# nextpyp/pyp

Hardware: AMD Instinct MI355X
Metric: particles/sec projection-matching, 256^2 box (higher is better)
Workload: dtype f32

## Files before the change

### include/ppm.h

```cpp
#ifndef PPM_H
#define PPM_H

#include <stddef.h>

#ifdef __cplusplus
extern "C" {
#endif

#define PPM_NCOL 32
enum {
    PPM_POS = 0, PPM_PSI = 1, PPM_THETA = 2, PPM_PHI = 3, PPM_XSHIFT = 4, PPM_YSHIFT = 5,
    PPM_DF1 = 6, PPM_DF2 = 7, PPM_ANGAST = 8, PPM_PSHIFT = 9, PPM_FILM = 10, PPM_OCC = 11,
    PPM_LOGP = 12, PPM_SIGMA = 13, PPM_SCORE = 14, PPM_PIXEL = 15, PPM_VOLTAGE = 16,
    PPM_CS = 17, PPM_AMP = 18, PPM_BTX = 19, PPM_BTY = 20, PPM_PIND = 26, PPM_TIND = 27
};

#define PPM_MAX_SHIFT_STEPS 8
#define PPM_MAX_TOP_HITS 64
#define PPM_MAX_DEFOCUS_STEPS 20

typedef struct ppm_refine_cfg {
    int box;
    float pixel_size;
    float molecular_mass_kda;
    float mask_radius;
    float res_low;
    float res_high;
    float res_signed_cc;
    float search_mask_radius;
    float res_search;
    float angular_step;
    int top_hits;
    float search_range_x;
    float search_range_y;
    int global_search;
    int local_refine;
    int refine_psi, refine_theta, refine_phi, refine_x, refine_y;
    int normalize;
    int invert;
    float mask_falloff;
    int iters_hit;
    int iters_final;
    float local_angle_step;
    float local_shift_step;
    char symmetry[8];
    float band_factor;
    int refine_defocus;
    float defocus_range;
    float defocus_step;
    float focus[4];
    int use_priors;
    float prior_mean[5];
    float prior_var[5];
    float res_classification;
} ppm_refine_cfg;

typedef struct ppm_recon_cfg {
    int box;
    float pixel_size;
    float res_limit;
    float score_weight_bfactor;
    float score_average;
    float score_threshold;
    int normalize;
    int invert;
    int split_by_pind;
    float mask_radius;
    const float *dose_weights; int n_dose_weights;
    float dose_exponent;
    float dose_transition;
} ppm_recon_cfg;

typedef struct ppm_final_cfg {
    float molecular_mass_kda;
    float inner_radius;
    float outer_radius;
    float mask_falloff;
} ppm_final_cfg;

enum { PPM_CSP_PARTICLES = 1, PPM_CSP_MICROGRAPHS = 2 };
#define PPM_NPCOL 12
#define PPM_NTCOL 6
typedef struct ppm_csp_cfg {
    int unit;
    int refine_rotation;
    int refine_translation;
    float tol_angle[3];
    float tol_shift;
    float step_tolerance;
    int max_iterations;
    int tind_min, tind_max;
    int first, last;
    int refine_defocus;
    float defocus_range;
    float defocus_step;
    int search_points;
    int search_candidates;
} ppm_csp_cfg;

typedef struct ppm_csp_search_info {
    int active;
    int shift_grid;
    double step;
    double r_g;
    double h_s;
    double tol_shift;
    int n_angle[3];
    int full_turn[3];
    int n_shift_axis;
    long n_rot, n_shift;
    int n_candidates;
} ppm_csp_search_info;

#define PPM_STATS_COLS 7

typedef struct ppm_ref ppm_ref_t;
typedef struct ppm_accum ppm_accum_t;

enum { PPM_K_PREP = 0, PPM_K_BANK = 1, PPM_K_GLOBAL = 2, PPM_K_TOPK = 3, PPM_K_LOCAL = 4,
       PPM_K_INSERT = 5, PPM_K_FINAL = 6, PPM_K_EXTRACT = 7, PPM_K_NORMS = 8, PPM_K_COUNT = 9 };

int ppm_init(int device);
const char *ppm_last_error(void);
const char *ppm_version(void);
const char *ppm_build_id(void);
int ppm_device_mem_info(size_t *free_bytes, size_t *total_bytes);

ppm_ref_t *ppm_reference_create(const float *vol, int n, float max_band_px);
ppm_ref_t *ppm_reference_create_padded(const float *vol, int n, float max_band_px, int pad);
ppm_ref_t *ppm_reference_create_weighted(const float *vol, int n, float max_band_px, int pad, const float *ring_weight, int n_weight);
void ppm_reference_destroy(ppm_ref_t *ref);

int ppm_refine_batch(ppm_ref_t *ref, const ppm_refine_cfg *cfg, const void *images,
                     int images_on_device, int n_img, const double *rows_in, double *rows_out);
int ppm_refine_last_counts(ppm_ref_t *ref, long *n_global, long *n_local, long *samples_global,
                           long *samples_local);
const char *ppm_refine_note(ppm_ref_t *ref);
int ppm_refine_last_sections(ppm_ref_t *ref);
int ppm_refine_last_overlap(ppm_ref_t *ref);

int ppm_match_projections(ppm_ref_t *ref, const ppm_refine_cfg *cfg, const double *rows, int n_rows, float *out);

int ppm_csp_refine(ppm_ref_t *ref, const ppm_refine_cfg *cfg, const ppm_csp_cfg *csp, const void *images, int images_on_device,
                   int n_proj, double *rows, double *particles, int n_part, double *tilts, int n_tilt);
int ppm_csp_search_plan(const ppm_refine_cfg *cfg, const ppm_csp_cfg *csp, ppm_csp_search_info *out);
int ppm_csp_search_candidates(ppm_ref_t *ref, long unit, int max_k, long *rot_index, long *shift_index, double *score);

#define PPM_FRAME_MAX_STEPS 8
typedef struct ppm_frame_cfg { float range_px, step_px; int half_width, tind_min, tind_max, first, last; } ppm_frame_cfg;
typedef struct ppm_frame_info { long groups, models, rows_refined, rows_scored, rows_skipped; int n_steps; float step_px, range_px; int clipped; } ppm_frame_info;
int ppm_frame_refine(ppm_ref_t *ref, const ppm_refine_cfg *cfg, const ppm_frame_cfg *fcfg, const void *images, int images_on_device,
                     const double *rows, int n_rows, double *rows_out, float *own_maps, float *pooled_maps, ppm_frame_info *info);
int ppm_frame_plan(const ppm_frame_cfg *fcfg, float *step_px, int *n_steps, int *clipped);

typedef struct ppm_sva_cfg {
    int box; float pixel_size;
    float window[3];
    float window_sigma;
    float highpass_cutoff, highpass_decay, lowpass_cutoff, lowpass_decay;
    int use_missing_wedge;
    float tol_angle;
    float tol_shift;
    float step_tolerance;
    int max_iterations;
    float band_factor;
    int search_mode;
    float global_step;
    int n_candidates;
    char symmetry[8];
} ppm_sva_cfg;
int ppm_sva_align(ppm_ref_t *ref, const ppm_sva_cfg *cfg, const void *volumes, int volumes_on_device, int n_vol, const float *wedges,
                  double *poses, double *scores);

size_t ppm_accum_floats(int box);
ppm_accum_t *ppm_accum_create(int box, float pixel_size, const char *symmetry,
                              void *ext_device_buffer);
void ppm_accum_destroy(ppm_accum_t *acc);
int ppm_insert_batch(ppm_accum_t *acc, const ppm_recon_cfg *cfg, const void *images,
                     int images_on_device, int n_img, const double *rows);
int ppm_accum_download(ppm_accum_t *acc, float *host);
int ppm_accum_download_range(ppm_accum_t *acc, float *host, size_t first, size_t count);
int ppm_accum_add(ppm_accum_t *acc, const float *host);
long ppm_accum_count(ppm_accum_t *acc, int half);
void ppm_accum_set_count(ppm_accum_t *acc, int half, long count);

typedef struct ppm_comm_id { char bytes[128]; } ppm_comm_id;
int ppm_comm_unique_id(ppm_comm_id *id);
void *ppm_comm_create(int n_ranks, int rank, const ppm_comm_id *id);
int ppm_comm_count(void *comm);
void ppm_comm_destroy(void *comm);
int ppm_accum_reduce(ppm_accum_t *acc, void *comm, int root);

int ppm_sva_insert(ppm_accum_t *acc, const ppm_sva_cfg *cfg, const void *volumes, int volumes_on_device, int n_vol, const float *wedges,
                   const double *poses, const long *index);

int ppm_sva_align_average(ppm_ref_t *ref, ppm_accum_t *acc, const ppm_sva_cfg *cfg, const void *volumes, int volumes_on_device, int n_vol,
                          const float *wedges, double *poses, double *scores, const long *index);

int ppm_finalize(ppm_accum_t *acc, const ppm_final_cfg *cfg, float *half1, float *half2,
                 float *filtered, double *stats);

typedef struct ppm_mask_cfg { double pixel_size; int edge_width; double outside_weight;
                              int filter; double filter_radius_A; double filter_edge_px; } ppm_mask_cfg;
int ppm_mask_volume(const void *map, const void *mask, int on_device, int n, const ppm_mask_cfg *cfg, void *out);

typedef struct ppm_create_mask_cfg { double pixel_size, outer_radius_A, threshold, lowpass_A, lowpass_edge_px, rebin; } ppm_create_mask_cfg;
typedef struct ppm_create_mask_info { double density_min, density_max; long above, components, largest, mask_voxels; } ppm_create_mask_info;
int ppm_create_mask(const void *map, int on_device, int n, const ppm_create_mask_cfg *cfg, void *mask_out, ppm_create_mask_info *info);

typedef struct ppm_post_cfg {
    double pixel_size;
    int mask_mode;
    double automask_lp;
    int threshold_method;
    double threshold_value;
    int randomize_method;
    double randomize_value;
    unsigned seed;
    int bfactor_method;
    double adhoc_bfac, fit_low, fit_high;
    int lowpass_auto;
    double lowpass, highpass;
    int gaussian, skip_fsc_weighting, apply_fsc2, flip_x, flip_y, flip_z;
} ppm_post_cfg;
typedef struct ppm_post_info { int s_r, res_shell, fit_shells, transforms; double resolution, bfactor, threshold; long mask_voxels; } ppm_post_info;
int ppm_postprocess(const void *half1, const void *half2, const void *mask, int on_device, int n, const ppm_post_cfg *cfg,
                    void *unmasked_out, void *masked_out, void *mask_out, double *curves, long *shell_count, ppm_post_info *info);

#define PPM_LOCRES_MAX_LEVELS 64
#define PPM_LOCRES_UNASSIGNED 100.0f
typedef struct ppm_locres_cfg { double pixel_size, p_value, min_res, max_res, step; int keep_levels; } ppm_locres_cfg;
typedef struct ppm_locres_info {
    int n_levels, transforms;
    long n_inside, unassigned;
    double median;
    float levels[PPM_LOCRES_MAX_LEVELS], tau[PPM_LOCRES_MAX_LEVELS];
    long counts[PPM_LOCRES_MAX_LEVELS];
    char notes[256];
} ppm_locres_info;
int ppm_local_resolution(const ppm_locres_cfg *cfg, const void *half1, const void *half2, const void *mask, int on_device, int n,
                         void *out_res, void *level_maps, ppm_locres_info *info);

int ppm_extract_boxes(const void *image, int image_on_device, int rows, int cols, const double *coords, int m,
                      int box, double coordinate_binning, double radius_px, int normalize, int fix_empty,
                      void *out, int out_on_device);

void ppm_profile_enable(int on);
void ppm_profile_reset(void);
int ppm_profile_get(int kernel_id, double *total_ms, long *launches);

void *ppm_device_alloc(size_t bytes);
void ppm_device_free(void *p);
int ppm_device_upload(void *dst, const void *src, size_t bytes);
int ppm_device_sync(void);
void *ppm_host_alloc(size_t bytes);
void ppm_host_free(void *p);
int ppm_host_read(int fd, long long offset, void *dst, size_t bytes, int n_threads);

#ifdef __cplusplus
}
#endif
#endif
```

### pyp_amd/csrc/host_ctx.h

```cpp
#pragma once

namespace {

thread_local std::string g_err;
int fail(int code, const std::string &msg) { g_err = "ERROR: " + msg; return code; }

#define HIPCHK(call)                                                                          \
    do {                                                                                      \
        hipError_t e_ = (call);                                                               \
        if (e_ != hipSuccess) {                                                               \
            g_err = std::string("ERROR: HIP: ") + hipGetErrorString(e_) + " at " #call;        \
            return -5;                                                                        \
        }                                                                                     \
    } while (0)
#define HIPCHKP(call)                                                                         \
    do {                                                                                      \
        hipError_t e_ = (call);                                                               \
        if (e_ != hipSuccess) {                                                               \
            g_err = std::string("ERROR: HIP: ") + hipGetErrorString(e_) + " at " #call;        \
            return nullptr;                                                                   \
        }                                                                                     \
    } while (0)

struct Ctx {
// ... 26 lines not shown
};

hipEvent_t ev_get() {
    std::lock_guard<std::mutex> lk(g_mu);
    if (!g.pool.empty()) { hipEvent_t e = g.pool.back(); g.pool.pop_back(); return e; }
    hipEvent_t e; (void)hipEventCreate(&e); return e;
}
void prof_flush() {
    std::lock_guard<std::mutex> lk(g_mu);
    for (auto &p : g.pending) {
        (void)hipEventSynchronize(p.b);
        float ms = 0; (void)hipEventElapsedTime(&ms, p.a, p.b);
        g.prof_ms[p.id] += ms; g.prof_n[p.id] += 1;
        g.pool.push_back(p.a); g.pool.push_back(p.b);
    }
    g.pending.clear();
}
struct ProfScope {
    int id; hipEvent_t a = nullptr;
    explicit ProfScope(int id_) : id(id_) { if (g.prof_on) { a = ev_get(); (void)hipEventRecord(a, cur_stream()); } }
    ~ProfScope() { if (a) { hipEvent_t b = ev_get(); (void)hipEventRecord(b, cur_stream()); std::lock_guard<std::mutex> lk(g_mu); g.pending.push_back({ id, a, b }); } }
};

struct Trace {
    const char *who; bool on; std::chrono::steady_clock::time_point t0;
    explicit Trace(const char *w) : who(w), on(getenv("PPM_TRACE") != nullptr), t0(std::chrono::steady_clock::now()) {}
    void mark(const char *what) const {
        if (!on) return;
        const double host_ms = std::chrono::duration<double, std::milli>(std::chrono::steady_clock::now() - t0).count();
        (void)hipStreamSynchronize(cur_stream());
        fprintf(stderr, "%s: %8.2f ms  (host reached this mark)\n", who, host_ms);
        fprintf(stderr, "%s: %8.2f ms  %s\n", who, std::chrono::duration<double, std::milli>(std::chrono::steady_clock::now() - t0).count(), what);
    }
};

int ensure_plan(int n) {
    if (n < 2 || n > 512) return fail(-22, "FFT length out of range");
    std::lock_guard<std::mutex> lk(g_mu);
    if (g.plans[n].ready) return 0;
    std::vector<int> fac; std::vector<unsigned short> perm;
    fft_factors(n, fac, perm);
    int prod = 1; for (int f : fac) prod *= f;
    if (prod != n || fac.size() > 12) return fail(-22, "FFT length must have prime factors 2, 3, 5 and 7 only");
    std::vector<float2> t(n);
    for (int k = 0; k < n; k++) t[k] = make_float2((float)std::cos(2.0 * kPi * k / n), (float)std::sin(2.0 * kPi * k / n));
    float2 *dtw = nullptr; unsigned short *dperm = nullptr;
    HIPCHK(hipMalloc(&dtw, sizeof(float2) * n));
    HIPCHK(hipMalloc(&dperm, sizeof(unsigned short) * n));
    HIPCHK(hipMemcpy(dtw, t.data(), sizeof(float2) * n, hipMemcpyHostToDevice));
    HIPCHK(hipMemcpy(dperm, perm.data(), sizeof(unsigned short) * n, hipMemcpyHostToDevice));
    FftPlan &p = g.plans[n].plan;
    p.n = n; p.nfac = (int)fac.size(); for (size_t i = 0; i < fac.size(); i++) p.fac[i] = fac[i];
    p.tw = dtw; p.perm = dperm;
    g.plans[n].ready = true;
    return 0;
}


int fft_lines_pass(float2 *d, int n, long nlines, long inner, long inner_stride, long outer_stride, long elem_stride, int line_major, bool inverse) {
    if (nlines <= 0) return 0;
    if (int rc = ensure_plan(n)) return rc;
    int L = std::max(1, std::min(16, 7600 / (n + 1)));
    while (nlines % L) L--;
    FftLinesP P;
    P.data = d; P.plan = g.plans[n].plan; P.n = n; P.inverse = inverse ? 1 : 0; P.L = L; P.nlines = nlines;
    P.inner = inner; P.inner_stride = inner_stride; P.outer_stride = outer_stride; P.elem_stride = elem_stride; P.line_major = line_major;
    hipLaunchKernelGGL(k_fft_lines, dim3((unsigned)((nlines + L - 1) / L)), dim3(256), (size_t)L * (n + 1) * sizeof(float2), cur_stream(), P);
    HIPCHK(hipGetLastError());
    return 0;
}

int fft2d_batch(float2 *d, int n, long nimg, bool inverse) {
    const long nlines = nimg * n;
    if (int rc = fft_lines_pass(d, n, nlines, nlines, n, 0, 1, 0, inverse)) return rc;
    return fft_lines_pass(d, n, nlines, n, 1, (long)n * n, n, 1, inverse);
}

int fft3d(float2 *d, int n, bool inverse) {
    const long nlines = (long)n * n;
    if (int rc = fft_lines_pass(d, n, nlines, nlines, n, 0, 1, 0, inverse)) return rc;
    if (int rc = fft_lines_pass(d, n, nlines, n, 1, nlines, n, 1, inverse)) return rc;
    return fft_lines_pass(d, n, nlines, nlines, 1, 0, nlines, 1, inverse);
}

template <typename T>
struct DevBuf {
    T *p = nullptr; size_t cap = 0;
    DevBuf() = default;
    DevBuf(const DevBuf &) = delete;
    DevBuf &operator=(const DevBuf &) = delete;
    ~DevBuf() { if (p) (void)hipFree(p); }
    int ensure(size_t n) {
        if (n <= cap) return 0;
        if (p) (void)hipFree(p);
        p = nullptr; cap = 0;
        HIPCHK(hipMalloc(&p, n * sizeof(T)));
        cap = n;
        return 0;
    }
};

int raise_lds_limit(const void *fn, int bytes) {
    static std::vector<const void *> raised;
    std::lock_guard<std::mutex> lk(g_mu);
    if (std::find(raised.begin(), raised.end(), fn) != raised.end()) return 0;
    HIPCHK(hipFuncSetAttribute(fn, hipFuncAttributeMaxDynamicSharedMemorySize, bytes));
    raised.push_back(fn);
    return 0;
}

template <typename T>
struct DevTmp {
    T *p = nullptr;
    DevTmp() = default;
    DevTmp(const DevTmp &) = delete;
    DevTmp &operator=(const DevTmp &) = delete;
    ~DevTmp() { if (p) (void)hipFree(p); }
    hipError_t alloc(size_t n) { return hipMalloc(&p, n * sizeof(T)); }
};


}

struct Lane { DevBuf<double> rows_in, rows_out; DevBuf<float> wring, cw, ddef; DevBuf<float2> Il; DevBuf<Hit> hits; DevBuf<LState> states, states2; };

struct ppm_ref {
    hipStream_t stream = nullptr, copy = nullptr;
    hipStream_t local = nullptr;
    int N = 0, B = 0, CX = 0, CY = 0, NBX = 0, NBY = 0, pad = 1; unsigned LB = 0;
    float2 *cube = nullptr;
    Lane lane[2];
    DevBuf<double> dir_theta, dir_phi;
    DevBuf<float> images, C2, nP, nI, cc, mats;
    DevBuf<float2> c_Il, c_band; DevBuf<float> c_cw, c_img, c_wring; DevBuf<double> c_rows, c_N, c_p, c_tl, c_delta, c_s0, c_g0, c_out;
    DevBuf<int> c_eval, c_rp, c_rt, c_slot, c_uoff, c_active; DevBuf<LState> c_states; DevBuf<double> c_mean, c_tmean, c_acc, c_dtrial, c_fpm, c_delta_t;
    DevBuf<double> c_rowtab; DevBuf<float> c_gbest, c_cscore; DevBuf<int> c_gshift, c_cshift; DevBuf<long> c_crot;
    std::vector<long> cand_unit, cand_rot; std::vector<int> cand_shift; std::vector<float> cand_score; int cand_K = 0;
    DevBuf<int> f_int; DevBuf<float> f_flt, f_own, f_pool; DevBuf<double> f_dbl; DevBuf<float2> f_store;
    DevBuf<float2> s_f, s_g, s_F; DevBuf<float> s_vols;
    struct { bool valid = false; float key[5] = { 0, 0, 0, 0, 0 }; int S = 0; std::vector<int> shell_off; DevBuf<uint32_t> samples, pos; DevBuf<float> bandw; DevBuf<float2> Fw; bool fw_valid = false; float wkey[4] = { 0, 0, 0, 0 }; } s_plan;
    DevBuf<float2> band, Wp, bank, twN;
    DevBuf<float2> spill;
    DevBuf<float4> rowtw;
    DevBuf<int> sh;
    DevBuf<uint32_t> samples;
    DevBuf<Hit> hits_t;
    DevBuf<int> tile_c;
    DevBuf<Hit> hits_s; DevBuf<int> sec_k;
    DevBuf<float4> bank4; DevBuf<float> part, gtw;
    std::string grid_key, bank_key, bank4_key; int gtw_ns = 0, gtw_rsx = -1;
    long last_counts[4] = { 0, 0, 0, 0 };
    int last_sections = 0;
    int last_overlap = 0;
    std::string note;
};

struct ppm_accum {
    hipStream_t stream = nullptr, copy = nullptr;
    int N = 0; float pixel = 1.f;
    float *acc = nullptr; bool external = false;
    std::vector<double> symops; int nsym = 1;
    float *d_sym = nullptr;
    unsigned long long *d_counts = nullptr;
    unsigned *d_max = nullptr;
    long counts[2] = { 0, 0 };
    DevBuf<double> rows; DevBuf<float> images, dose; DevBuf<float2> band, spill; DevBuf<PartIns> pp; DevBuf<CullEnt> cull; DevBuf<BrickItem> items;
    DevBuf<float2> s_f, s_g; DevBuf<float> s_vols;
    std::vector<float> brick_load; float load_r = -1.f; int n_items = 0, items_cap = -1;
};

static CubeView cube_view(const ppm_ref *ref) {
    CubeView cv;
    cv.cube = ref->cube; cv.NBX = ref->NBX; cv.NBY = ref->NBY; cv.LB = ref->LB; cv.off = ref->B + 1; cv.scale = (float)ref->pad;
    return cv;
}

static bool local_tables_wanted(int tabR) {
    return !(getenv("PPM_LOCAL_TABLES") && atoi(getenv("PPM_LOCAL_TABLES")) == 0) && cube_tab_bytes(tabR) <= 16 * 1024;
}
static bool tables_fit_lds(size_t ring_bytes, int tabR) { return ring_bytes + cube_tab_bytes(tabR) + 2048 <= (size_t)64 * 1024; }

struct ChunkStager {
    const float *src; float *buf; bool on_device; int n_img, chunk; size_t nn;
    int prime() const {
        if (on_device) return 0;
        HIPCHK(hipMemcpyAsync(buf, src, (size_t)std::min(chunk, n_img) * nn * sizeof(float), hipMemcpyHostToDevice, cur_copy()));
        HIPCHK(hipStreamSynchronize(cur_copy()));
        return 0;
    }
    const float *chunk_ptr(int c0, int ci) const { return on_device ? src + (size_t)c0 * nn : buf + (size_t)(ci & 1) * chunk * nn; }
    int prefetch_next(int c0, int ci) const {
        if (on_device || c0 + chunk >= n_img) return 0;
        const int n_next = std::min(chunk, n_img - (c0 + chunk));
        HIPCHK(hipMemcpyAsync(buf + (size_t)((ci + 1) & 1) * chunk * nn, src + (size_t)(c0 + chunk) * nn, (size_t)n_next * nn * sizeof(float), hipMemcpyHostToDevice, cur_copy()));
        return 0;
    }
    int sync() const {
        HIPCHK(hipStreamSynchronize(cur_stream()));
        HIPCHK(hipStreamSynchronize(cur_copy()));
        return 0;
    }
};

static __global__ void k_noop() {}

extern "C" {

const char *ppm_last_error(void) { return g_err.c_str(); }
const char *ppm_version(void) { return "pypmatch 0.1 (gfx950)"; }
const char *ppm_build_id(void) { return "pypmatch " __DATE__ " " __TIME__; }
int ppm_device_mem_info(size_t *free_bytes, size_t *total_bytes) {
    if (!g.inited) return fail(-1, "ppm_init has not been called");
    (void)hipSetDevice(g.device);
    size_t f = 0, t = 0;
    HIPCHK(hipMemGetInfo(&f, &t));
    if (free_bytes) *free_bytes = f;
    if (total_bytes) *total_bytes = t;
    return 0;
}

int ppm_init(int device) {
    static std::mutex init_mu;
    std::lock_guard<std::mutex> lk(init_mu);
    const auto t_init0 = std::chrono::steady_clock::now();
    if (g.inited && g.device == device) { (void)hipSetDevice(device); return 0; }
    if (g.inited) return fail(-16, "libpypmatch is bound to device " + std::to_string(g.device) + " in this process (one process per GPU); start another process for device " + std::to_string(device));
    int count = 0;
    if (hipGetDeviceCount(&count) != hipSuccess || count <= 0) return fail(-19, "no HIP device visible; libpypmatch has no CPU path");
    if (device < 0 || device >= count) return fail(-22, "device index out of range");
    if (const char *e = getenv("PPM_SYNC")) {
        const std::string v(e);
        (void)hipSetDeviceFlags(v == "block" ? hipDeviceScheduleBlockingSync : (v == "yield" ? hipDeviceScheduleYield : (v == "spin" ? hipDeviceScheduleSpin : hipDeviceScheduleAuto)));
    }
    HIPCHK(hipSetDevice(device));
    hipDeviceProp_t prop;
    HIPCHK(hipGetDeviceProperties(&prop, device));
    if (std::string(prop.gcnArchName).find("gfx950") == std::string::npos)
        return fail(-19, std::string("device is ") + prop.gcnArchName + ", libpypmatch is built for gfx950 only");
    g.total_mem = prop.totalGlobalMem;
    g.cu_count = std::max(1, prop.multiProcessorCount);
    g.lds_per_cu = std::max((size_t)prop.maxSharedMemoryPerMultiProcessor, (size_t)160 * 1024);
    if (!g.stream) HIPCHK(hipStreamCreateWithFlags(&g.stream, hipStreamNonBlocking));
    if (!g.copy) HIPCHK(hipStreamCreateWithFlags(&g.copy, hipStreamNonBlocking));
    if (!g.upload) HIPCHK(hipStreamCreateWithFlags(&g.upload, hipStreamNonBlocking));
    const auto t_ctx = std::chrono::steady_clock::now();
    hipLaunchKernelGGL(k_noop, dim3(1), dim3(64), 0, g.stream);
    HIPCHK(hipGetLastError());
    HIPCHK(hipStreamSynchronize(g.stream));
    g.device = device; g.inited = true;
    if (getenv("PPM_TRACE"))
        fprintf(stderr, "ppm_init: context + streams %.1f ms, code object + first launch %.1f ms\n",
                std::chrono::duration<double, std::milli>(t_ctx - t_init0).count(), std::chrono::duration<double, std::milli>(std::chrono::steady_clock::now() - t_ctx).count());
    return 0;
}

void ppm_profile_enable(int on) { g.prof_on = on != 0; }
void ppm_profile_reset(void) { prof_flush(); for (int i = 0; i < PPM_K_COUNT; i++) { g.prof_ms[i] = 0; g.prof_n[i] = 0; } }
int ppm_profile_get(int id, double *ms, long *n) {
    if (id < 0 || id >= PPM_K_COUNT) return fail(-22, "bad kernel id");
    prof_flush();
    if (ms) *ms = g.prof_ms[id];
    if (n) *n = g.prof_n[id];
    return 0;
}

void *ppm_device_alloc(size_t bytes) { if (g.inited) (void)hipSetDevice(g.device); void *p = nullptr; if (hipMalloc(&p, bytes) != hipSuccess) { g_err = "ERROR: device allocation failed"; return nullptr; } return p; }
void ppm_device_free(void *p) { if (p) (void)hipFree(p); }
int ppm_device_upload(void *dst, const void *src, size_t bytes) {
    if (!g.inited) return fail(-1, "ppm_init has not been called");
    HIPCHK(hipSetDevice(g.device));
    HIPCHK(hipMemcpyAsync(dst, src, bytes, hipMemcpyHostToDevice, g.upload));
    HIPCHK(hipStreamSynchronize(g.upload));
    return 0;
}
void *ppm_host_alloc(size_t bytes) { if (g.inited) (void)hipSetDevice(g.device); void *p = nullptr; if (hipHostMalloc(&p, bytes, hipHostMallocDefault) != hipSuccess) { g_err = "ERROR: pinned host allocation failed"; return nullptr; } return p; }
void ppm_host_free(void *p) { if (p) (void)hipHostFree(p); }
extern "C++" {
namespace {
struct ReadPool {
    std::mutex mu;
    std::mutex qmu;
    std::condition_variable wake, done;
    std::vector<std::thread> threads;
    struct Part { int fd; long long off; char *dst; size_t bytes; };
    std::vector<Part> parts;
    size_t next = 0, pending = 0;
    int err = 0;
    bool quit = false;
    void worker() {
        std::unique_lock<std::mutex> lk(qmu);
        for (;;) {
            wake.wait(lk, [&] { return quit || next < parts.size(); });
            if (quit) return;
            Part p = parts[next++];
            lk.unlock();
            int e = 0;
            size_t got = 0;
            while (got < p.bytes) {
                ssize_t r = pread(p.fd, p.dst + got, std::min(p.bytes - got, (size_t)64 << 20), p.off + (long long)got);
                if (r < 0) { if (errno == EINTR) continue; e = -errno; break; }
                if (r == 0) { e = -5; break; }
                got += (size_t)r;
            }
            lk.lock();
            if (e && !err) err = e;
            if (--pending == 0) done.notify_all();
        }
    }
    int run(int fd, long long off, char *dst, size_t bytes, int nt) {
        std::lock_guard<std::mutex> one(mu);
        nt = std::max(1, std::min(nt, 16));
        std::unique_lock<std::mutex> lk(qmu);
        while ((int)threads.size() < nt) threads.emplace_back([this] { worker(); });
        const size_t per = std::max((size_t)1 << 20, ((bytes + nt - 1) / nt + ((size_t)1 << 20) - 1) >> 20 << 20);
        parts.clear(); next = 0; err = 0;
        for (size_t a = 0; a < bytes; a += per) parts.push_back({fd, off + (long long)a, dst + a, std::min(per, bytes - a)});
        pending = parts.size();
        if (!pending) return 0;
        wake.notify_all();
        done.wait(lk, [&] { return pending == 0; });
        parts.clear(); next = 0;
        return err;
    }
    ~ReadPool() {
        { std::lock_guard<std::mutex> lk(qmu); quit = true; }
        wake.notify_all();
        for (auto &t : threads) t.join();
    }
};
// ... 44 lines not shown
```

### pyp_amd/csrc/host_refine.h

```cpp
#pragma once

static int launch_prep(DevBuf<float2> &spill , const float *d_images, const double *d_rows, int n_img, const Geom &gm, double Rm_px, float fall_px,
                       int normalize, int invert, int do_mask, int whiten, float2 *band, float *wring,
                       const uint32_t *samples, int S_pad, float2 *Il, float *cw, float2 *Wp, float *C2, float *nI,
                       unsigned *band_max = nullptr ,
                       const float *focus_px = nullptr ) {
    if (int rc = ensure_plan(gm.N)) return rc;
    PrepP P;
    P.images = d_images; P.rows = d_rows; P.plan = g.plans[gm.N].plan;
    P.N = gm.N; P.B = gm.B; P.W = gm.W; P.H = gm.H;
    P.r_hi2 = (float)(gm.r_hi * gm.r_hi); P.Rm = (float)Rm_px; P.wfall = fall_px; P.a = (float)gm.a;
    P.Rm2_bg = (float)std::min(std::floor(Rm_px * Rm_px), 16777216.0);
    P.normalize = normalize; P.invert = invert; P.do_mask = do_mask; P.whiten = whiten;
    for (int k = 0; k < 4; k++) P.focus[k] = focus_px ? focus_px[k] : 0.f;
    P.band_max = band_max;
    P.band = band; P.wring = wring; P.samples = samples; P.S_pad = S_pad; P.Il = Il; P.cw = cw;
    P.Wp = Wp; P.C2 = C2; P.nI = nI; P.Bs = gm.Bs; P.Hs = gm.Hs;
    P.r_s2 = (float)(gm.r_s * gm.r_s); P.r_lo2 = (float)(gm.r_lo * gm.r_lo);
    const PrepPlan pl = prep_plan(gm.N, gm.B, gm.W);
    if (pl.err) return fail(-12, pl.err);
    P.L = pl.L; P.nc = pl.nc; P.nchunks = pl.nchunks; P.TS = pl.TS; P.WS = pl.WS;
    P.spill = nullptr;
    if (!pl.scratch_free) {
        if (int rc = spill.ensure((size_t)n_img * gm.N * gm.W)) return rc;
        P.spill = spill.p;
    }
    if (int rc = pl.scratch_free ? raise_lds_limit((const void *)k_prep<512, 2>, 160 * 1024) : raise_lds_limit((const void *)k_prep<256, 3>, 80 * 1024)) return rc;
    ProfScope ps(PPM_K_PREP);
    if (pl.scratch_free) hipLaunchKernelGGL((k_prep<512, 2>), dim3(n_img), dim3(512), pl.lds.total, cur_stream(), P);
    else hipLaunchKernelGGL((k_prep<256, 3>), dim3(n_img), dim3(256), pl.lds.total, cur_stream(), P);
    HIPCHK(hipGetLastError());
    return 0;
}

template <int... I>
static const void *global_kernel_at(int i, std::integer_sequence<int, I...>) {
    static const void *const fn[] = { (const void *)k_global<I / 4 + 1, (I & 2) != 0, (I & 1) != 0>... };
    return fn[i];
}
static const void *global_kernel(int R, bool half, int Bs) {
    const bool two = Bs <= 31;
    return global_kernel_at(((R >= 1 && R <= 5 ? R : 6) - 1) * 4 + (half ? 2 : 0) + (two ? 1 : 0), std::make_integer_sequence<int, 24>());
}
static size_t global_lds_bytes(int HsP, int n_orient, int R, int *topk_lds) {
    size_t lds = (size_t)HsP * 64 * sizeof(float2) * global_particles(R);
    if (lds < 1024) lds = 1024;
    const size_t lds_topk = (size_t)(32 + n_orient) * sizeof(float);
    const int fits = lds_topk <= (size_t)160 * 1024 ? 1 : 0;
    if (topk_lds) *topk_lds = fits;
    if (fits && lds_topk > lds) lds = lds_topk;
    return lds;
}
static int launch_global(GlobP &P, int n_img, bool half, int R) {
    P.n = n_img;
    const size_t lds = global_lds_bytes(P.HsP, P.n_orient, R, &P.topk_lds);
    const void *fn = global_kernel(R, half, P.Bs);
    if (int rc = raise_lds_limit(fn, 160 * 1024)) return rc;
    ProfScope ps(PPM_K_GLOBAL);
    const int ngroups = (n_img + global_particles(R) - 1) / global_particles(R);
    void *args[] = { &P };
    HIPCHK(hipLaunchKernel(fn, dim3(std::min(ngroups, g.cu_count)), dim3(global_threads(R)), args, lds, cur_stream()));
    return 0;
}

struct GfftPlan { int LN = 0, L = 0, RC = 0, nchunk = 1; size_t fixed = 0, t_bytes = 0, lds = 0; int topk_lds = 0; };
static bool gfft_plan(const Geom &gm, GfftPlan &pl) {
    int LN = 0; while ((1 << LN) < gm.Ns) LN++;
    if ((1 << LN) != gm.Ns || LN < 4 || LN > 7) return false;
    pl.LN = LN; pl.L = gm.Ns / 2;
    const int L = pl.L, G = gfft_slices_per_pass(L), NR = 2 * gm.RSy + 1;
    const size_t row = (size_t)G * 2 * gfft_row_stride(L) * sizeof(float2), fixed = (size_t)L * L * sizeof(float4) + gfft_small_bytes(L);
    const size_t room = (size_t)160 * 1024 - fixed;
    int RC = NR;
    if (const char *e = getenv("PPM_GFFT_ROWS")) { const int v = atoi(e); if (v > 0 && v < RC) RC = v; }
    if ((size_t)RC * row > room) RC = (int)(room / row);
    if (RC > 2 * L) RC = 2 * L;
    pl.RC = RC; pl.nchunk = (NR + RC - 1) / RC;
    pl.RC = (NR + pl.nchunk - 1) / pl.nchunk;
    pl.t_bytes = std::max((size_t)pl.RC * row, (size_t)G * L * L * sizeof(float4));
    pl.fixed = fixed;
    return true;
}
static void gfft_plan_topk(GfftPlan &pl, int n_orient) {
    const size_t topk = (size_t)n_orient * sizeof(float);
    pl.topk_lds = 0;
    if (topk <= pl.t_bytes) pl.topk_lds = 1;
    else if (pl.fixed + topk <= (size_t)160 * 1024) { pl.topk_lds = 1; pl.t_bytes = (topk + 15) & ~(size_t)15; }
    pl.lds = pl.fixed + pl.t_bytes;
}
static const void *gfft_kernel(int LN, bool chunked) {
    static const void *const fn[] = { (const void *)k_gfft<4, false>, (const void *)k_gfft<4, true>, (const void *)k_gfft<5, false>, (const void *)k_gfft<5, true>,
                                      (const void *)k_gfft<6, false>, (const void *)k_gfft<6, true>, (const void *)k_gfft<7, false>, (const void *)k_gfft<7, true> };
    return fn[((LN >= 4 && LN <= 6 ? LN : 7) - 4) * 2 + (chunked ? 1 : 0)];
}
static int launch_gfft(GfftP &P, int n_img, const GfftPlan &pl) {
    P.n = n_img; P.RC = pl.RC; P.nchunk = pl.nchunk; P.t_bytes = (int)pl.t_bytes; P.topk_lds = pl.topk_lds;
    const void *fn = gfft_kernel(pl.LN, pl.nchunk > 1);
    if (int rc = raise_lds_limit(fn, 160 * 1024)) return rc;
    ProfScope ps(PPM_K_GLOBAL);
    void *args[] = { &P };
    HIPCHK(hipLaunchKernel(fn, dim3(n_img), dim3(256), args, pl.lds, cur_stream()));
#ifdef PPM_GFFT_STAMPS
    {
        float st[4 * 4 * 12];
        HIPCHK(hipStreamSynchronize(cur_stream()));
        HIPCHK(hipMemcpy(st, P.cc, sizeof(st), hipMemcpyDeviceToHost));
        const char *names[12] = { "products", "fft", "stores", "barrier A", "row tail", "barrier B", "twiddles", "loop", "row reads + pairs", "row fft", "row max", "-" };
        const int nsl = P.n_dir * P.npsi_store;
        for (int b = 0; b < 4 && b < n_img; b++) for (int w = 0; w < 4; w++) {
            fprintf(stderr, "k_gfft stamps block %d wave %d (cycles per slice):", b, w);
            for (int i = 0; i < 11; i++) fprintf(stderr, " | %s %.0f", names[i], st[(b * 4 + w) * 12 + i] / nsl);
            fprintf(stderr, "\n");
        }
    }
#endif
    return 0;
}

static void launch_defocus(const CubeView &cv, const Geom &gm, const uint32_t *samples, int S_pad, const float2 *Il, const float *wring, const double *rows,
                           LState *states, int n, int nt, float step, float *ddef, double *all_scores, float rcls2) {
    const int nrings = gm.B + 2;
    DefocusP DP;
    DP.cv = cv; DP.samples = samples; DP.Il = Il; DP.wring = wring; DP.S_pad = S_pad; DP.nrings = nrings; DP.N = gm.N; DP.B = gm.B;
    DP.rlo2 = (float)(gm.r_lo * gm.r_lo); DP.rmax2 = (float)(gm.r_hi * gm.r_hi); DP.ring_signed = (float)std::min(gm.ring_signed, 1e30); DP.a = (float)gm.a;
    DP.rows = rows; DP.states = states; DP.ddef = ddef; DP.nt = nt; DP.step = step; DP.all_scores = all_scores; DP.rcls2 = rcls2;
    long knob = 0;
    if (const char *e = std::getenv("PPM_DEFOCUS_CHUNK")) knob = std::atol(e);
    DP.tchunk = ppm::defocus_chunk(nt, nrings, knob);
    ProfScope ps(PPM_K_LOCAL);
    hipLaunchKernelGGL(k_defocus, dim3(n), dim3(256), ring_lds_bytes(4, DP.tchunk, nrings), cur_stream(), DP);
}

namespace {
struct LocalLaunch { LocalP P = {}; int threads = 0, per_particle = 1; double evals = 0; };
struct RefineRun {
    ppm_ref *ref = nullptr; const ppm_refine_cfg *cfg = nullptr;
    Geom gm; SampleList sl; CubeView cv;
    int S_pad = 0, nrings = 0, CH = 0;
    int K = 0, Tb = 0, Tc = 0;
    double Rm_px = 0; float fall_px = 0;
    bool focus_on = false, sep_search = false; float focus_px[4] = { 0, 0, 0, 0 };
    GfftPlan gpl; bool use_fft = false;
    RowPlan rows = {};
    int Rtx = 0, Rty = 0, Rwin = 0, HsP = 0, nslices = 0; std::vector<int> cxs, cys;
    std::vector<GridSection> secs; std::vector<int> kpre; int sec_dirs = 0;
    LocalP base = {}; bool local_tab = false;
    double bf = 3.0; bool any_ang = false, any_sh = false;
    double ha0 = 0, hs0 = 0;
    int ndef = 0;
    int per_iter = 0; bool cls_on = false;
    LocalLaunch hit, fin;
    double sample_evals = 0;
    bool overlap = false; int tenants = 0;

    int ntiles() const { return (int)(cxs.size() * cys.size()); }
    int nsec() const { return (int)secs.size(); }
    size_t bank_slice() const { return (size_t)HsP * 64; }
    size_t bank4_slice() const { return use_fft ? (size_t)gpl.L * gpl.L : 0; }
    size_t HS() const { return (size_t)gm.Hs * 64; }
    int prefix_of(double rband) const { int rg = (int)std::ceil(rband); if (rg > gm.B + 1) rg = gm.B + 1; return sl.ring_off[rg]; }
    int reach_of(int S) const { int b = gm.B + 2; while (b > 1 && sl.ring_off[b] > S) b--; return std::min(gm.B, b - 1); }
};
constexpr int kTileR = 6;
constexpr int kFinalThreads = 256;
}

static void refine_notes(ppm_ref *ref, const ppm_refine_cfg *cfg, const Geom &gm) {
    ref->note.clear();
    if (gm.r_s_asked > gm.r_s) {
        char b[256];
        std::snprintf(b, sizeof(b), "NOTE: global search band lowered from %.1f to %.1f Fourier pixels (%.2f A instead of %.2f A): the grid-search "
                      "kernel covers 64 pixels; the top hits are refined up to the high-resolution limit as asked", gm.r_s_asked, gm.r_s,
                      gm.N * gm.a / gm.r_s, gm.N * gm.a / gm.r_s_asked);
        ref->note = b;
    }
    if (cfg->global_search && gm.range_capped) {
        char b[320];
        std::snprintf(b, sizeof(b), "%sNOTE: shift window of the grid search: +-%.0f x +-%.0f pixels (%d x %d search-grid steps of %.1f pixels, the most the "
                      "search grid of %d points holds; asked: %.0f pixels); the refinement of the hits is not limited to it", ref->note.empty() ? "" : "\n",
                      gm.RSx * gm.step, gm.RSy * gm.step, gm.RSx, gm.RSy, gm.step, gm.Ns, gm.range_asked_px);
        ref->note += b;
    }
}

static size_t workspace_budget() { return g.total_mem / 4; }
static size_t bank_budget() {
    size_t b = g.total_mem / 4;
    if (const char *e = std::getenv("PPM_BANK_BYTES")) { const long long v = std::atoll(e); if (v > 0 && (size_t)v < b) b = (size_t)v; }
    return b;
}

static int plan_grid_sections(RefineRun &r) {
    ppm_ref *ref = r.ref; const Geom &gm = r.gm;
    std::string err;
    const size_t budget = bank_budget();
    if (!plan_sections(gm.n_dir, gm.npsi_store, r.bank_slice() * sizeof(float2), r.bank4_slice() * sizeof(float4), budget, r.secs, err)) return fail(-22, err);
    if (r.nsec() > 1 && !r.use_fft && r.ntiles() > 1) {
        char b[320];
        std::snprintf(b, sizeof(b), "PPM_GLOBAL_PATH=tiles keeps the slice bank of the whole grid (%.2f GB at an angular step of %.3g degrees), the bank may take "
                      "%.2f GB; use a coarser angular step or the default path, which searches the grid in sections", (double)r.nslices * r.bank_slice() * sizeof(float2) / 1073741824.0,
                      gm.dstep, budget / 1073741824.0);
        return fail(-22, b);
    }
    r.kpre.assign(1, 0); r.sec_dirs = 0;
    for (const GridSection &sc : r.secs) {
        r.kpre.push_back(r.kpre.back() + std::min(r.K, sc.nd * gm.n_psi));
        r.sec_dirs = std::max(r.sec_dirs, sc.nd);
    }
    if (r.use_fft) gfft_plan_topk(r.gpl, r.sec_dirs * gm.n_psi);
    ref->last_sections = r.nsec();
    if (r.nsec() > 1) {
        char b[200];
        std::snprintf(b, sizeof(b), "%sNOTE: grid search in %d sections of the orientation grid (%d directions, angular step %.3g degrees: the slice banks are "
                      "built and searched one section at a time)", ref->note.empty() ? "" : "\n", r.nsec(), gm.n_dir, gm.dstep);
        ref->note += b;
    }
    return 0;
}

static int refine_plan(RefineRun &r, int n_img) {
    ppm_ref *ref = r.ref; const ppm_refine_cfg *cfg = r.cfg; const Geom &gm = r.gm;
    r.K = cfg->top_hits > 0 ? cfg->top_hits : 20;
    if (r.K > PPM_MAX_TOP_HITS) r.K = PPM_MAX_TOP_HITS;
    if (r.K > gm.n_orient) r.K = gm.n_orient;
    r.Tb = cfg->iters_hit > 0 ? cfg->iters_hit : (cfg->iters_hit < 0 ? 0 : 2); r.Tc = cfg->iters_final > 0 ? cfg->iters_final : 7;
    const double fall = cfg->mask_falloff > 0 ? cfg->mask_falloff : 20.0;
    r.fall_px = (float)(fall / gm.a);
    r.Rm_px = cfg->mask_radius / gm.a;
    r.focus_on = cfg->focus[3] > 0.f;
    for (int k = 0; k < 4; k++) r.focus_px[k] = (float)(cfg->focus[k] / gm.a);
    r.sep_search = !r.focus_on && cfg->global_search && cfg->search_mask_radius > 0 && cfg->search_mask_radius != cfg->mask_radius;

    build_samples(gm, r.sl);
    r.S_pad = (int)r.sl.packed.size();
    r.nrings = gm.B + 2;
    if (int rc = ref->samples.ensure(r.S_pad)) return rc;
    HIPCHK(hipMemcpyAsync(ref->samples.p, r.sl.packed.data(), r.S_pad * sizeof(uint32_t), hipMemcpyHostToDevice, cur_stream()));

    r.use_fft = false;
    if (cfg->global_search && gfft_plan(gm, r.gpl)) {
        const char *gp = getenv("PPM_GLOBAL_PATH");
        const bool force_fft = gp && !strcmp(gp, "fft"), force_tiles = gp && !strcmp(gp, "tiles");
        r.use_fft = force_fft || (!force_tiles && std::max(gm.RSx, gm.RSy) > kTileR);
    }
    r.Rtx = std::min(gm.RSx, kTileR); r.Rty = std::min(gm.RSy, kTileR);
    auto tile_centres = [](int RS, int Rt) {
        const int T = (2 * RS + 1 + 2 * Rt) / (2 * Rt + 1);
        std::vector<int> c(T, 0);
        for (int i = 0; i < T && T > 1; i++) c[i] = -RS + Rt + (int)(((long)i * 2 * (RS - Rt)) / (T - 1));
        return c;
    };
    r.cxs = tile_centres(gm.RSx, r.Rtx); r.cys = tile_centres(gm.RSy, r.Rty);
    r.Rwin = std::max(r.Rtx, r.Rty);
    static_assert(global_unroll(1) == 4 && global_unroll(PPM_MAX_SHIFT_STEPS) == 4, "row_plan lays the bank out in steps of U = 4 rows");
    r.rows = row_plan(gm.Ns, gm.Bs, global_fold(gm.Bs));
    r.HsP = r.rows.HsP;
    r.nslices = gm.n_dir * gm.npsi_store;
    if (cfg->global_search) if (int rc = plan_grid_sections(r)) return rc;
    const size_t NN = (size_t)gm.N * gm.N, HW = (size_t)gm.H * gm.W;
    size_t per = NN * 4 + HW * 8 + (size_t)r.S_pad * 12 + 2 * PPM_NCOL * 8 + (gm.B + 2) * 4;
    if (cfg->global_search) per += r.HS() * 12 + (size_t)r.nslices * 4 + (size_t)gm.n_orient * 8 + (size_t)r.K * (sizeof(Hit) + sizeof(LState)) + sizeof(LState);
    size_t fit = ((size_t)4 << 30) / per;
    if (fit < 64) {
        const size_t ws = workspace_budget(), per_all = per + (r.use_fft ? (size_t)gm.n_orient * 8 : 0);
        fit = std::min<size_t>(64, ws / per_all);
        if (fit < 1) {
            char b[320];
            std::snprintf(b, sizeof(b), "angular step of %.3g degrees: the grid search keeps %.1f GB of tables per particle for its %d orientations, "
                          "the workspace holds %.1f GB; use a coarser angular step", gm.dstep, per_all / 1073741824.0, gm.n_orient, ws / 1073741824.0);
            return fail(-22, b);
        }
    }
    int CH = (int)std::min<size_t>((size_t)n_img, fit);
    CH = std::min(CH, 8192);
    if (CH >= 2048) CH &= ~1023;
    if (const char *e = std::getenv("PPM_CHUNK")) { int v = std::atoi(e); if (v > 0) CH = std::min(CH, v); }
    r.CH = CH;
    return 0;
}

static int ensure_chunk_buffers(RefineRun &r, bool images_on_device) {
    ppm_ref *ref = r.ref; const Geom &gm = r.gm;
    if (!images_on_device) if (int rc = ref->images.ensure((size_t)2 * r.CH * gm.N * gm.N)) return rc;
    return ref->band.ensure((size_t)r.CH * gm.H * gm.W);
}
static int ensure_lane(const RefineRun &r, int i) {
    Lane &L = r.ref->lane[i]; const size_t CH = r.CH;
    if (int rc = L.rows_in.ensure(CH * PPM_NCOL)) return rc;
    if (int rc = L.rows_out.ensure(CH * PPM_NCOL)) return rc;
    if (int rc = L.wring.ensure(CH * (r.gm.B + 2))) return rc;
    if (int rc = L.Il.ensure(CH * r.S_pad)) return rc;
    if (int rc = L.cw.ensure(CH * r.S_pad)) return rc;
    if (int rc = L.states2.ensure(CH)) return rc;
    if (r.cfg->global_search) {
        if (int rc = L.hits.ensure(CH * r.K)) return rc;
        if (int rc = L.states.ensure(CH * r.K)) return rc;
    }
    if (r.ndef > 0) if (int rc = L.ddef.ensure(CH)) return rc;
    return 0;
}

static int ensure_bank(const RefineRun &r, const GridSection &sec) {
    ppm_ref *ref = r.ref; const Geom &gm = r.gm;
    const std::string key = ref->grid_key + "/d" + std::to_string(sec.d0) + "+" + std::to_string(sec.nd);
    if (ref->bank_key == key) return 0;
    const int nsl = sec.nd * gm.npsi_store;
    BankP BP; BP.cv = r.cv; BP.mats = ref->mats.p + (size_t)sec.d0 * gm.npsi_store * 6; BP.bank = ref->bank.p; BP.nslices = nsl; BP.Bs = gm.Bs; BP.Hs = r.HsP; BP.rows = r.rows;
    BP.r_s2 = (float)(gm.r_s * gm.r_s);
    {
        ProfScope ps(PPM_K_BANK);
        size_t tot = (size_t)nsl * r.bank_slice();
        hipLaunchKernelGGL(k_bank, dim3((unsigned)((tot + 255) / 256)), dim3(256), 0, cur_stream(), BP);
    }
    HIPCHK(hipGetLastError());
    ref->bank_key = key;
    return 0;
}

static int ensure_bank4(const RefineRun &r, const GridSection &sec) {
    ppm_ref *ref = r.ref; const Geom &gm = r.gm; const int L = r.gpl.L;
    const std::string key = ref->grid_key + "/d" + std::to_string(sec.d0) + "+" + std::to_string(sec.nd) + "/L" + std::to_string(L);
    if (ref->bank4_key == key) return 0;
    const int nsl = sec.nd * gm.npsi_store;
    Bank4P BP; BP.cv = r.cv; BP.mats = ref->mats.p + (size_t)sec.d0 * gm.npsi_store * 6; BP.bank4 = ref->bank4.p; BP.nslices = nsl; BP.Bs = gm.Bs; BP.L = L; BP.r_s2 = (float)(gm.r_s * gm.r_s);
    ProfScope ps(PPM_K_BANK);
    const size_t tot = (size_t)nsl * r.bank4_slice();
    hipLaunchKernelGGL(k_bank4, dim3((unsigned)((tot + 255) / 256)), dim3(256), 0, cur_stream(), BP);
    HIPCHK(hipGetLastError());
    ref->bank4_key = key;
    return 0;
}

static int ensure_search_tables(RefineRun &r) {
    ppm_ref *ref = r.ref; const Geom &gm = r.gm; const int CH = r.CH, nslices = r.nslices, HsP = r.HsP;
    const size_t HS = r.HS(), HSP = (size_t)HsP * 64;
    if (int rc = ref->Wp.ensure((size_t)CH * HS)) return rc;
    if (int rc = ref->C2.ensure((size_t)CH * HS)) return rc;
    if (int rc = ref->nP.ensure((size_t)CH * nslices)) return rc;
    if (int rc = ref->nI.ensure(CH)) return rc;
    if (int rc = ref->cc.ensure((size_t)CH * gm.n_orient)) return rc;
    if (int rc = ref->sh.ensure((size_t)CH * gm.n_orient)) return rc;
    {
        const size_t cap = ref->bank.cap;
        if (int rc = ref->bank.ensure((size_t)r.sec_dirs * gm.npsi_store * HSP)) return rc;
        if (ref->bank.cap != cap) ref->bank_key.clear();
    }
    if (r.nsec() > 1) {
        if (int rc = ref->hits_s.ensure((size_t)CH * r.kpre.back())) return rc;
        if (int rc = ref->sec_k.ensure(r.kpre.size())) return rc;
        HIPCHK(hipMemcpyAsync(ref->sec_k.p, r.kpre.data(), r.kpre.size() * sizeof(int), hipMemcpyHostToDevice, cur_stream()));
    }
    char key[160];
    std::snprintf(key, sizeof(key), "%d/%.6f/%.6f/%d/%d/%d/%.3f/%.3f", gm.N, gm.r_s, gm.dstep, gm.Ns, gm.npsi_store, HsP, gm.phi_max, gm.theta_max);
    if (ref->grid_key == key) return 0;
    ref->bank_key.clear(); ref->bank4_key.clear();
    std::vector<float> mats((size_t)nslices * 6);
    std::vector<double> dth(gm.n_dir), dph(gm.n_dir);
    for (int d = 0; d < gm.n_dir; d++) {
        grid_direction(gm, d, dth[d], dph[d]);
        for (int k = 0; k < gm.npsi_store; k++) {
            double M[9]; euler_matrix(k * gm.dpsi, dth[d], dph[d], M);
            float *m = &mats[((size_t)d * gm.npsi_store + k) * 6];
            m[0] = (float)M[0]; m[1] = (float)M[1]; m[2] = (float)M[3]; m[3] = (float)M[4]; m[4] = (float)M[6]; m[5] = (float)M[7];
        }
    }
    std::vector<float2> tw(gm.Ns);
    for (int t = 0; t < gm.Ns; t++) tw[t] = make_float2((float)std::cos(2.0 * kPi * t / gm.Ns), (float)std::sin(2.0 * kPi * t / gm.Ns));
    if (int rc = ref->mats.ensure(mats.size())) return rc;
    if (int rc = ref->dir_theta.ensure(gm.n_dir)) return rc;
    if (int rc = ref->dir_phi.ensure(gm.n_dir)) return rc;
    if (int rc = ref->twN.ensure(gm.Ns)) return rc;
    HIPCHK(hipMemcpyAsync(ref->mats.p, mats.data(), mats.size() * sizeof(float), hipMemcpyHostToDevice, cur_stream()));
    HIPCHK(hipMemcpyAsync(ref->dir_theta.p, dth.data(), dth.size() * sizeof(double), hipMemcpyHostToDevice, cur_stream()));
    HIPCHK(hipMemcpyAsync(ref->dir_phi.p, dph.data(), dph.size() * sizeof(double), hipMemcpyHostToDevice, cur_stream()));
    HIPCHK(hipMemcpyAsync(ref->twN.p, tw.data(), tw.size() * sizeof(float2), hipMemcpyHostToDevice, cur_stream()));
    {
        std::vector<float4> rt((size_t)kRowTwRows * PPM_MAX_SHIFT_STEPS, make_float4(1.f, 1.f, 0.f, 0.f));
        for (int tp = 0; 2 * tp < HsP && tp < kRowTwRows; tp++) for (int j = 1; j <= PPM_MAX_SHIFT_STEPS; j++) {
            int t = ((row_slot_t(r.rows, tp) * j) % gm.Ns + gm.Ns) % gm.Ns;
            const float c = (float)std::cos(2.0 * kPi * t / gm.Ns), sn = (float)std::sin(2.0 * kPi * t / gm.Ns);
            rt[(size_t)tp * PPM_MAX_SHIFT_STEPS + j - 1] = make_float4(c, c, sn, sn);
        }
        if (int rc = ref->rowtw.ensure(rt.size())) return rc;
        HIPCHK(hipMemcpyAsync(ref->rowtw.p, rt.data(), rt.size() * sizeof(float4), hipMemcpyHostToDevice, cur_stream()));
    }
    HIPCHK(hipStreamSynchronize(cur_stream()));
    ref->grid_key = key;
    return 0;
}

static int ensure_gfft_tables(RefineRun &r) {
    ppm_ref *ref = r.ref; const Geom &gm = r.gm;
    const int L = r.gpl.L;
    if (int rc = ref->part.ensure((size_t)r.CH * gm.n_orient * 2)) return rc;
    {
        const size_t cap = ref->bank4.cap;
        if (int rc = ref->bank4.ensure((size_t)r.sec_dirs * gm.npsi_store * r.bank4_slice())) return rc;
        if (ref->bank4.cap != cap) ref->bank4_key.clear();
    }
    if (ref->gtw_ns != gm.Ns || ref->gtw_rsx != gm.RSx) {
        const int nb = fr::bfly_entries(L);
        std::vector<float> tw((size_t)fr::tw_table_floats(L) + gm.Ns, 0.f);
        auto put = [&](float *d, double ang) { d[0] = (float)std::cos(ang); d[1] = (float)std::sin(ang); };
        for (int M = L; M >= 8; M /= 4)
            for (int k = 1; k < M / 4; k++)
                for (int j = 1; j <= 3; j++) put(&tw[(size_t)fr::bfly_entry(L, M, k) * 8 + (j - 1) * 2], 2.0 * kPi * j * k / M);
        for (int t = 0; t < L; t++) put(&tw[(size_t)nb * 8 + (size_t)t * 2], 2.0 * kPi * t / gm.Ns);
        for (int pp = 0; pp < L; pp++)
            for (int h = 0; h < 2; h++) {
                const int j = 2 * fr::freq_at(L, pp) + h, sx = j < L ? j : j - gm.Ns;
                tw[(size_t)fr::tw_table_floats(L) + 2 * pp + h] = std::abs(sx) <= gm.RSx ? 0.f : -3.0e38f;
            }
        if (int rc = ref->gtw.ensure(tw.size())) return rc;
        HIPCHK(hipMemcpyAsync(ref->gtw.p, tw.data(), tw.size() * sizeof(float), hipMemcpyHostToDevice, cur_stream()));
        HIPCHK(hipStreamSynchronize(cur_stream()));
        ref->gtw_ns = gm.Ns; ref->gtw_rsx = gm.RSx;
    }
    return 0;
}

static int local_setup(RefineRun &r) {
    ppm_ref *ref = r.ref; const ppm_refine_cfg *cfg = r.cfg; const Geom &gm = r.gm; LocalP &LP = r.base;
    r.bf = cfg->band_factor == 0 ? 3.0 : cfg->band_factor;
    r.any_ang = cfg->refine_psi || cfg->refine_theta || cfg->refine_phi; r.any_sh = cfg->refine_x || cfg->refine_y;
    r.ha0 = cfg->local_angle_step > 0 ? cfg->local_angle_step : 2.5; r.hs0 = cfg->local_shift_step > 0 ? cfg->local_shift_step : 2.0;
    r.ndef = cfg->refine_defocus ? ppm::defocus_steps(cfg->defocus_range, cfg->defocus_step, PPM_MAX_DEFOCUS_STEPS) : 0;
    LP.cv = r.cv; LP.samples = ref->samples.p; LP.S_pad = r.S_pad; LP.nrings = r.nrings; LP.N = gm.N;
    LP.tabR = cube_tab_radius(gm.B, r.cv.scale);
    r.local_tab = local_tables_wanted(LP.tabR);
    LP.rlo2 = (float)(gm.r_lo * gm.r_lo); LP.ring_signed = (float)std::min(gm.ring_signed, 1e30);
    LP.en[0] = cfg->refine_psi; LP.en[1] = cfg->refine_theta; LP.en[2] = cfg->refine_phi; LP.en[3] = cfg->refine_x; LP.en[4] = cfg->refine_y;
    LP.use_priors = 0;
    for (int i = 0; i < 5; i++) { LP.pmean[i] = 0; LP.pw[i] = 0; }
    if (cfg->use_priors) {
        const double ns = kPi * (gm.r_hi * gm.r_hi - gm.r_lo * gm.r_lo);
        for (int i = 0; i < 5; i++) {
            double var = cfg->prior_var[i], mean = cfg->prior_mean[i];
            if (i >= 3) { mean /= gm.a; var /= gm.a * gm.a; }
            LP.pmean[i] = mean;
            if (LP.en[i] && var > 0 && ns > 0) { LP.pw[i] = 1.0 / (2.0 * var * ns); LP.use_priors = 1; }
        }
    }
    const int nfree = (cfg->refine_psi != 0) + (cfg->refine_theta != 0) + (cfg->refine_phi != 0) + (cfg->refine_x != 0) + (cfg->refine_y != 0);
    r.per_iter = nfree ? 2 * nfree + 2 : 0;
    if (r.Tb + r.Tc > kMaxIters) return fail(-22, "too many compass iterations requested");
    LP.rmax2_final = (float)(gm.r_hi * gm.r_hi); LP.S_final = r.S_pad;
    r.cls_on = gm.r_cls < gm.r_hi;
    LP.rmax2_class = (float)(gm.r_cls * gm.r_cls); LP.S_class = (r.cls_on && r.ndef == 0) ? r.prefix_of(gm.r_cls) : 0;
    return 0;
}

static LocalLaunch with_schedule(const RefineRun &r, LocalLaunch L, double ha, double hs, double rcap) {
    for (int t = 0; t < L.P.T; t++) {
        double rb = march_band(r.bf, r.gm.N, r.Rm_px, ha, hs, r.any_ang, r.any_sh, rcap);
        L.P.rmax2_it[t] = (float)(rb * rb); L.P.S_it[t] = r.prefix_of(rb);
        L.evals += (double)L.per_particle * r.per_iter * std::floor(kPi * rb * rb / 2);
        ha *= 0.5; hs *= 0.5;
    }
    return L;
}
static LocalLaunch hit_launch(const RefineRun &r) {
    const Geom &gm = r.gm;
    LocalLaunch L; L.P = r.base; L.per_particle = r.K;
    L.P.T = r.Tb; L.P.final_rescore = 0; L.P.nr = std::min(r.nrings, (int)std::ceil(gm.r_s) + 1);
    L = with_schedule(r, L, 0.5 * gm.dstep, gm.step, gm.r_s);
    L.threads = r.Tb > 0 && L.P.S_it[0] > 1024 ? 128 : 64;
    return L;
}
static LocalLaunch full_band_launch(const RefineRun &r, int T, double ha, double hs) {
    LocalLaunch L; L.P = r.base; L.threads = kFinalThreads;
    L.P.T = r.cfg->local_refine ? T : 0; L.P.final_rescore = 1; L.P.nr = r.nrings;
    L = with_schedule(r, L, ha, hs, r.gm.r_hi);
    L.evals += std::floor(kPi * r.gm.r_hi * r.gm.r_hi / 2);
    return L;
}
static LocalLaunch final_launch(const RefineRun &r) { return full_band_launch(r, r.Tc, 0.5 * r.gm.dstep / (double)(1 << r.Tb), r.gm.step / (double)(1 << r.Tb)); }
static LocalLaunch rows_launch(const RefineRun &r) { return full_band_launch(r, r.Tb + r.Tc, r.ha0, r.hs0); }

struct LocalShape { size_t lds; bool tab; int tabR; };
static LocalShape local_shape(const RefineRun &r, const LocalLaunch &L) {
    const LocalP &LP = L.P;
    const size_t ring = ring_lds_bytes8(L.threads / 64, kMaxCand, LP.nr);
    LocalShape s;
    s.tab = r.local_tab && tables_fit_lds(ring, LP.tabR);
    int S = 0;
    for (int t = 0; t < LP.T; t++) S = std::max(S, LP.S_it[t]);
    if (LP.final_rescore) S = std::max(S, std::max(LP.S_final, LP.S_class));
    s.tabR = std::min(LP.tabR, cube_tab_radius(r.reach_of(S), r.cv.scale));
    s.lds = ring + (s.tab ? cube_tab_bytes(s.tabR) : 0);
    return s;
}
static void launch_local(const RefineRun &r, const LocalLaunch &L, const Lane &ln, LState *states, int nb) {
    LocalP LP = L.P;
    LP.Il = ln.Il.p; LP.cw = ln.cw.p; LP.states = states;
    const LocalShape s = local_shape(r, L);
    LP.tabR = s.tabR;
    const dim3 grid((unsigned)(nb * L.per_particle)), block(L.threads);
    ProfScope ps(PPM_K_LOCAL);
    if (s.tab) hipLaunchKernelGGL(k_local<true>, grid, block, s.lds, cur_stream(), LP);
    else hipLaunchKernelGGL(k_local<false>, grid, block, s.lds, cur_stream(), LP);
}

static int search_section(const RefineRun &r, int nb, const GridSection &sec, Hit *hits, int K, hipEvent_t ev_pre) {
    ppm_ref *ref = r.ref; const Geom &gm = r.gm;
    const int HsP = r.HsP, ntiles = r.ntiles(), nsl = sec.nd * gm.npsi_store, sl0 = sec.d0 * gm.npsi_store, o0 = sec.d0 * gm.n_psi;
    if (int rc = ensure_bank(r, sec)) return rc;
    if (r.use_fft) if (int rc = ensure_bank4(r, sec)) return rc;
    GlobP GP;
    GP.bank = ref->bank.p; GP.Wp = ref->Wp.p; GP.nP = ref->nP.p + sl0; GP.nI = ref->nI.p; GP.twN = ref->twN.p; GP.rowtw = ref->rowtw.p;
    GP.cc = ref->cc.p + o0; GP.sh = ref->sh.p + o0; GP.hits = hits;
    GP.Bs = gm.Bs; GP.Hs = gm.Hs; GP.HsP = HsP; GP.rows = r.rows; GP.Ns = gm.Ns; GP.RSx = r.Rtx; GP.RSy = r.Rty;
    GP.n_dir = sec.nd; GP.n_psi = gm.n_psi; GP.npsi_store = gm.npsi_store; GP.n_orient = sec.nd * gm.n_psi; GP.K = K;
    GP.nP_ld = r.nslices; GP.o_ld = gm.n_orient; GP.o_base = o0;
    {
        ProfScope ps(PPM_K_NORMS);
        NormP NP; NP.C2 = ref->C2.p; NP.bank = ref->bank.p; NP.nP = ref->nP.p + sl0; NP.n = nb; NP.nslices = nsl; NP.ldn = r.nslices; NP.Bs = gm.Bs; NP.Hs = gm.Hs; NP.HsP = HsP; NP.rows = r.rows;
        hipLaunchKernelGGL(k_slice_norms, dim3((nb + 127) / 128, (nsl + 127) / 128), dim3(256), 0, cur_stream(), NP);
    }
    if (r.use_fft) {
        GfftP FP;
        FP.bank4 = ref->bank4.p; FP.bank4_bytes = (unsigned)((size_t)nsl * r.bank4_slice() * sizeof(float4)); FP.Wp = ref->Wp.p; FP.nP = ref->nP.p + sl0; FP.nI = ref->nI.p; FP.tw = ref->gtw.p;
        FP.part = ref->part.p + (size_t)o0 * (r.gpl.L == 64 ? 2 : 1); FP.cc = ref->cc.p + o0; FP.hits = hits;
        FP.Bs = gm.Bs; FP.Hs = gm.Hs; FP.RSx = gm.RSx; FP.RSy = gm.RSy;
        FP.n_dir = sec.nd; FP.n_psi = gm.n_psi; FP.npsi_store = gm.npsi_store; FP.n_orient = sec.nd * gm.n_psi; FP.K = K;
        FP.nP_ld = r.nslices; FP.o_ld = gm.n_orient; FP.o_base = o0;
        if (int rc = launch_gfft(FP, nb, r.gpl)) return rc;
    } else if (ntiles == 1) {
        if (ev_pre) HIPCHK(hipEventRecord(ev_pre, cur_stream()));
        if (int rc = launch_global(GP, nb, gm.half != 0, r.Rwin)) return rc;
    } else {
        if (int rc = ref->hits_t.ensure((size_t)ntiles * nb * K)) return rc;
        if (int rc = ref->tile_c.ensure((size_t)2 * ntiles)) return rc;
        std::vector<int> tc(2 * ntiles);
        for (int ty = 0, t = 0; ty < (int)r.cys.size(); ty++) for (int tx = 0; tx < (int)r.cxs.size(); tx++, t++) { tc[t] = r.cxs[tx]; tc[ntiles + t] = r.cys[ty]; }
        HIPCHK(hipMemcpyAsync(ref->tile_c.p, tc.data(), tc.size() * sizeof(int), hipMemcpyHostToDevice, cur_stream()));
        int px = 0, py = 0;
        const size_t tot = (size_t)nb * r.HS();
        for (int t = 0; t < ntiles; t++) {
            const int dcx = tc[t] - px, dcy = tc[ntiles + t] - py;
            if (dcx || dcy) hipLaunchKernelGGL(k_wp_ramp, dim3((unsigned)((tot + 255) / 256)), dim3(256), 0, cur_stream(), ref->Wp.p, tot, gm.Bs, gm.Ns, dcx, dcy, ref->twN.p);
            px = tc[t]; py = tc[ntiles + t];
            GP.hits = ref->hits_t.p + (size_t)t * nb * K;
            if (int rc = launch_global(GP, nb, gm.half != 0, r.Rwin)) return rc;
        }
        hipLaunchKernelGGL(k_merge_hits, dim3((nb + 127) / 128), dim3(128), 0, cur_stream(), ref->hits_t.p, hits, nb, K, ntiles, ref->tile_c.p, ref->tile_c.p + ntiles);
        HIPCHK(hipStreamSynchronize(cur_stream()));
    }
    return 0;
}

static int search_stage(const RefineRun &r, int nb, const Lane &L, hipEvent_t ev_pre) {
    ppm_ref *ref = r.ref; const Geom &gm = r.gm;
    const int K = r.K;
    if (r.nsec() == 1) {
        if (int rc = search_section(r, nb, r.secs[0], L.hits.p, K, ev_pre)) return rc;
    } else {
        for (int s = 0; s < r.nsec(); s++)
            if (int rc = search_section(r, nb, r.secs[s], ref->hits_s.p + (size_t)r.kpre[s] * nb, r.kpre[s + 1] - r.kpre[s], ev_pre)) return rc;
        ProfScope ps(PPM_K_TOPK);
        hipLaunchKernelGGL(k_merge_sections, dim3(nb), dim3(64), 0, cur_stream(), ref->hits_s.p, L.hits.p, nb, K, r.nsec(), ref->sec_k.p);
        HIPCHK(hipGetLastError());
    }
    {
        ProfScope ps(PPM_K_TOPK);
        hipLaunchKernelGGL(k_states_from_hits, dim3((nb * K + 255) / 256), dim3(256), 0, cur_stream(), L.hits.p, L.states.p, nb, K,
                           ref->dir_theta.p, ref->dir_phi.p, gm.n_psi, gm.dpsi, gm.step, 0.5 * gm.dstep, gm.step);
    }
    return 0;
}

static void hits_local_stage(const RefineRun &r, int nb, const Lane &L) {
    if (r.Tb > 0) launch_local(r, r.hit, L, L.states.p, nb);
    {
        ProfScope ps(PPM_K_TOPK);
        hipLaunchKernelGGL(k_select_best, dim3((nb + 255) / 256), dim3(256), 0, cur_stream(), L.states.p, L.states2.p, nb, r.K);
    }
    launch_local(r, r.fin, L, L.states2.p, nb);
}

static void rows_stage(const RefineRun &r, int nb, const Lane &L) {
    hipLaunchKernelGGL(k_states_from_rows, dim3((nb + 255) / 256), dim3(256), 0, cur_stream(), L.rows_in.p, L.states2.p, nb, r.gm.a, r.ha0, r.hs0);
    launch_local(r, r.fin, L, L.states2.p, nb);
}

static int finish_chunk(const RefineRun &r, int nb, const Lane &L) {
    ppm_ref *ref = r.ref; const Geom &gm = r.gm;
    const float *d_ddef = nullptr;
    if (r.ndef > 0) {
        launch_defocus(r.cv, gm, ref->samples.p, r.S_pad, L.Il.p, L.wring.p, L.rows_in.p, L.states2.p, nb, r.ndef, r.cfg->defocus_step,
                       L.ddef.p, nullptr, r.cls_on ? (float)(gm.r_cls * gm.r_cls) : 0.f);
        d_ddef = L.ddef.p;
    }
    hipLaunchKernelGGL(k_rows_out, dim3((nb + 255) / 256), dim3(256), 0, cur_stream(), L.states2.p, L.rows_in.p, L.rows_out.p, nb, gm.a, gm.r_cls, gm.r_lo, d_ddef);
    HIPCHK(hipGetLastError());
    return 0;
}

static int plan_overlap(RefineRun &r, int n_img) {
    ppm_ref *ref = r.ref; const Geom &gm = r.gm;
    r.overlap = false; r.tenants = 0;
    OverlapCall c;
    c.global_search = r.cfg->global_search != 0; c.use_fft = r.use_fft; c.ntiles = r.ntiles(); c.nsections = r.nsec();
    c.nchunks = (n_img + r.CH - 1) / r.CH; c.hit_stage = r.Tb > 0;
    const char *e = std::getenv("PPM_REFINE_OVERLAP");
    c.forced_off = e && std::atoi(e) == 0;
    if (!overlap_on(1, c)) return 0;
    const LocalShape ls = local_shape(r, r.hit);
    hipFuncAttributes ga, la;
    HIPCHK(hipFuncGetAttributes(&ga, global_kernel(r.Rwin, gm.half != 0, gm.Bs)));
    HIPCHK(hipFuncGetAttributes(&la, ls.tab ? (const void *)k_local<true> : (const void *)k_local<false>));
    const OverlapKernel host = { ga.numRegs, global_threads(r.Rwin), (long)ga.sharedSizeBytes + (long)global_lds_bytes(r.HsP, r.secs[0].nd * gm.n_psi, r.Rwin, nullptr) };
    const OverlapKernel tenant = { la.numRegs, r.hit.threads, (long)la.sharedSizeBytes + (long)ls.lds };
    const OverlapDevice dev = { 512, 4, (long)g.lds_per_cu, 8, 1280 };
    r.tenants = overlap_tenants(host, tenant, dev);
    r.overlap = overlap_on(r.tenants, c);
    if (std::getenv("PPM_TRACE"))
        fprintf(stderr, "ppm_refine_batch: k_global %d VGPRs / %ld B LDS, hit stage %d threads, %d VGPRs / %ld B LDS: %d blocks per CU beside the search, overlap %s\n",
                host.vgprs, host.lds_bytes, tenant.threads, tenant.vgprs, tenant.lds_bytes, r.tenants, r.overlap ? "on" : "off");
    if (!r.overlap) return 0;
    if (int rc = ensure_lane(r, 1)) return rc;
    if (!ref->local) {
        int lo = 0, hi = 0;
        HIPCHK(hipDeviceGetStreamPriorityRange(&lo, &hi));
        HIPCHK(hipStreamCreateWithPriority(&ref->local, hipStreamNonBlocking, lo));
    }
    return 0;
}

struct OverlapStreams {
    ppm_ref *ref = nullptr; hipEvent_t ready[2] = { nullptr, nullptr }, pre[2] = { nullptr, nullptr }, done[2] = { nullptr, nullptr };
    int open(ppm_ref *ref_) {
        ref = ref_;
        for (int i = 0; i < 2; i++) { ready[i] = ev_get(); pre[i] = ev_get(); done[i] = ev_get(); if (!ready[i] || !pre[i] || !done[i]) return fail(-12, "out of events"); }
        return 0;
    }
    int drain() {
        HIPCHK(hipStreamSynchronize(ref->local));
        HIPCHK(hipStreamSynchronize(ref->stream));
        return 0;
    }
    ~OverlapStreams() {
        if (!ref) return;
        (void)hipStreamSynchronize(ref->local); (void)hipStreamSynchronize(ref->stream);
        std::lock_guard<std::mutex> lk(g_mu);
        for (int i = 0; i < 2; i++) for (hipEvent_t e : { ready[i], pre[i], done[i] }) if (e) g.pool.push_back(e);
    }
};

static void refine_counts(const RefineRun &r) {
    const ppm_refine_cfg *cfg = r.cfg; const Geom &gm = r.gm;
    long nl;
    if (cfg->global_search) nl = (long)r.K * r.Tb * r.per_iter + (cfg->local_refine ? (long)r.Tc * r.per_iter : 0) + 1;
    else nl = 1 + (cfg->local_refine ? (long)(r.Tb + r.Tc) * r.per_iter : 0);
    nl += 2L * r.ndef + (r.cls_on ? 1 : 0);
    double evals = r.sample_evals + 2.0 * r.ndef * std::floor(kPi * gm.r_hi * gm.r_hi / 2);
    if (r.cls_on) evals += std::floor(kPi * gm.r_cls * gm.r_cls / 2);
    long *c = r.ref->last_counts;
    c[0] = cfg->global_search ? gm.n_orient : 0;
    c[1] = nl;
    c[2] = (long)std::floor(kPi * gm.r_s * gm.r_s / 2);
    c[3] = (long)evals;
}

extern "C" {

ppm_ref_t *ppm_reference_create_weighted(const float *vol, int n, float max_band_px, int pad, const float *ring_weight, int n_weight) {
    if (!g.inited) { fail(-1, "ppm_init has not been called"); return nullptr; }
    if (!vol || !box_ok(n) || !(max_band_px > 0)) { fail(-22, "reference box must be even, 32..512, with prime factors 2, 3, 5, 7, and the band positive"); return nullptr; }
    if ((pad != 1 && pad != 2 && pad != 4) || n * pad > 512) { fail(-22, "padding factor must be 1, 2 or 4 with padded box <= 512"); return nullptr; }
    if (max_band_px > n / 2) max_band_px = (float)(n / 2);
    const int np = n * pad;
    int B = (int)std::ceil((double)max_band_px * pad) - 1;
    if (B > np / 2 - 1) B = np / 2 - 1;
    size_t n3 = (size_t)n * n * n, np3 = (size_t)np * np * np;
    struct Undo { ppm_ref *p; ~Undo() { ppm_reference_destroy(p); } } guard{ new ppm_ref() };
    ppm_ref *r = guard.p;
    HIPCHKP(hipStreamCreateWithFlags(&r->stream, hipStreamNonBlocking));
    HIPCHKP(hipStreamCreateWithFlags(&r->copy, hipStreamNonBlocking));
    StreamScope ss_(r->stream, r->copy);
    DevTmp<float> t_vol, t_w; DevTmp<float2> t_f;
    HIPCHKP(t_vol.alloc(n3));
    HIPCHKP(t_f.alloc(np3));
    float *d_vol = t_vol.p; float2 *d_f = t_f.p;
    HIPCHKP(hipMemcpy(d_vol, vol, n3 * sizeof(float), hipMemcpyHostToDevice));
    if (pad > 1) HIPCHKP(hipMemsetAsync(d_f, 0, np3 * sizeof(float2), cur_stream()));
    float *d_w = nullptr;
    if (ring_weight && n_weight > 0) {
        HIPCHKP(t_w.alloc((size_t)n_weight));
        d_w = t_w.p;
        HIPCHKP(hipMemcpyAsync(d_w, ring_weight, (size_t)n_weight * sizeof(float), hipMemcpyHostToDevice, cur_stream()));
    }
    r->N = n; r->pad = pad; r->B = B; r->CX = B + 2; r->CY = 2 * B + 3;
    size_t cube_n = (size_t)r->CX * r->CY * r->CY;
    r->NBX = (r->CX + 3) / 4; r->NBY = (r->CY + 1) / 2;
    const size_t copy_n = (size_t)r->NBX * r->NBY * r->NBY * 16;
    if (2 * copy_n * sizeof(float2) >= ((size_t)1 << 32)) {
    fail(-22, "reference cube too large"); return nullptr; }
    r->LB = (unsigned)copy_n;
    if (hipMalloc(&r->cube, 2 * copy_n * sizeof(float2)) != hipSuccess) { r->cube = nullptr; fail(-12, "out of device memory for the reference cube"); return nullptr; }
    HIPCHKP(hipMemsetAsync(r->cube, 0, 2 * copy_n * sizeof(float2), cur_stream()));
    {
        ProfScope ps(PPM_K_BANK);
        hipLaunchKernelGGL(k_ref_load, dim3((unsigned)((n3 + 255) / 256)), dim3(256), 0, cur_stream(), d_vol, d_f, n, np);
        if (fft3d(d_f, np, false)) return nullptr;
        hipLaunchKernelGGL(k_ref_crop, dim3((unsigned)((cube_n + 255) / 256)), dim3(256), 0, cur_stream(), d_f, r->cube, np, n, B, r->CX, r->CY, r->NBX, r->NBY, r->LB, d_w, n_weight);
    }
    if (hipStreamSynchronize(cur_stream()) != hipSuccess || hipGetLastError() != hipSuccess) { fail(-5, "reference preparation failed on the device"); return nullptr; }
    return std::exchange(guard.p, nullptr);
}

ppm_ref_t *ppm_reference_create_padded(const float *vol, int n, float max_band_px, int pad) { return ppm_reference_create_weighted(vol, n, max_band_px, pad, nullptr, 0); }
ppm_ref_t *ppm_reference_create(const float *vol, int n, float max_band_px) { return ppm_reference_create_weighted(vol, n, max_band_px, 1, nullptr, 0); }

void ppm_reference_destroy(ppm_ref_t *r) {
    if (!r) return;
    if (r->cube) (void)hipFree(r->cube);
    if (r->local) (void)hipStreamDestroy(r->local);
    if (r->stream) (void)hipStreamDestroy(r->stream);
    if (r->copy) (void)hipStreamDestroy(r->copy);
    delete r;
}

int ppm_match_projections(ppm_ref_t *ref, const ppm_refine_cfg *cfg, const double *rows, int n_rows, float *out) {
    if (!g.inited) return fail(-1, "ppm_init has not been called");
    if (!ref || !cfg || !rows || !out) return fail(-22, "null argument");
    StreamScope ss_(ref->stream, ref->copy);
    if (n_rows <= 0) return 0;
    ppm_refine_cfg c2 = *cfg; c2.global_search = 0;
    Geom gm; std::string err;
    if (!geom_init(gm, c2, err)) return fail(-22, err);
    if (gm.N != ref->N) return fail(-22, "particle box differs from the reference box");
    if (gm.B > (ref->B + 1) / ref->pad - 1) return fail(-22, "high-resolution limit exceeds the band the reference was prepared for");
    const size_t NN = (size_t)gm.N * gm.N;
    const int CH = (int)std::min<size_t>((size_t)n_rows, std::max<size_t>(1, ((size_t)1 << 30) / (NN * 12)));
    DevTmp<float2> d_f; DevTmp<float> d_o; DevTmp<MatchRow> d_rows;
    HIPCHK(d_f.alloc(NN * CH)); HIPCHK(d_o.alloc(NN * CH)); HIPCHK(d_rows.alloc(CH));
    MatchP MP;
    MP.cv = cube_view(ref);
    MP.rows = d_rows.p; MP.f = d_f.p; MP.N = gm.N; MP.B = gm.B; MP.r_hi2 = (float)(gm.r_hi * gm.r_hi);
    std::vector<MatchRow> hr(CH);
    const float scale = (cfg->invert ? -1.f : 1.f) / (float)gm.N;
    for (int c0 = 0; c0 < n_rows; c0 += CH) {
        const int nb = std::min(CH, n_rows - c0);
        for (int i = 0; i < nb; i++) {
            const double *row = rows + (size_t)(c0 + i) * PPM_NCOL;
            double M[9]; euler_matrix(row[PPM_PSI], row[PPM_THETA], row[PPM_PHI], M);
            MatchRow &q = hr[i];
            q.m[0] = (float)M[0]; q.m[1] = (float)M[1]; q.m[2] = (float)M[3]; q.m[3] = (float)M[4]; q.m[4] = (float)M[6]; q.m[5] = (float)M[7];
            q.sx = (float)(row[PPM_XSHIFT] / gm.a); q.sy = (float)(row[PPM_YSHIFT] / gm.a);
            q.ctf = ctf_from_row(row, gm.N, gm.a);
        }
        HIPCHK(hipMemcpyAsync(d_rows.p, hr.data(), (size_t)nb * sizeof(MatchRow), hipMemcpyHostToDevice, cur_stream()));
        MP.n = nb;
        hipLaunchKernelGGL(k_match_fill, dim3((unsigned)((NN * nb + 255) / 256)), dim3(256), 0, cur_stream(), MP);
        if (int rc = fft2d_batch(d_f.p, gm.N, nb, true)) return rc;
        hipLaunchKernelGGL(k_match_real, dim3((unsigned)((NN * nb + 255) / 256)), dim3(256), 0, cur_stream(), d_f.p, d_o.p, NN * nb, scale);
        HIPCHK(hipGetLastError());
        HIPCHK(hipMemcpyAsync(out + (size_t)c0 * NN, d_o.p, NN * nb * sizeof(float), hipMemcpyDeviceToHost, cur_stream()));
        HIPCHK(hipStreamSynchronize(cur_stream()));
    }
    return 0;
}

int ppm_refine_batch(ppm_ref_t *ref, const ppm_refine_cfg *cfg, const void *images, int images_on_device,
                     int n_img, const double *rows_in, double *rows_out) {
    if (!g.inited) return fail(-1, "ppm_init has not been called");
    if (!ref || !cfg || !images || !rows_in || !rows_out) return fail(-22, "null argument");
    StreamScope ss_(ref->stream, ref->copy);
    if (n_img <= 0) return 0;
    ref->last_sections = 0;
    RefineRun r; r.ref = ref; r.cfg = cfg;
    const Geom &gm = r.gm; std::string err;
    if (!geom_init(r.gm, *cfg, err)) return fail(-22, err);
    if (gm.N != ref->N) return fail(-22, "particle box differs from the reference box");
    refine_notes(ref, cfg, gm);
    if (gm.B > (ref->B + 1) / ref->pad - 1) return fail(-22, "high-resolution limit exceeds the band the reference was prepared for");
    if (cfg->global_search && gm.Bs + 1 > 64)
        return fail(-22, "global search band wider than 64 Fourier pixels is not supported; lower the 'resolution limit for search'");
    if (int rc = refine_plan(r, n_img)) return rc;
    if (int rc = ensure_chunk_buffers(r, images_on_device != 0)) return rc;
    r.cv = cube_view(ref);
    if (cfg->global_search) {
        if (int rc = ensure_search_tables(r)) return rc;
        if (int rc = ensure_bank(r, r.secs[0])) return rc;
        if (r.use_fft) { if (int rc = ensure_gfft_tables(r)) return rc; if (int rc = ensure_bank4(r, r.secs[0])) return rc; }
    }
    HIPCHK(hipStreamSynchronize(cur_stream()));
    if (int rc = local_setup(r)) return rc;
    if (cfg->global_search) { r.hit = hit_launch(r); r.fin = final_launch(r); }
    else r.fin = rows_launch(r);
    r.sample_evals = r.hit.evals + r.fin.evals;
    if (int rc = ensure_lane(r, 0)) return rc;
    if (int rc = plan_overlap(r, n_img)) return rc;
    ref->last_overlap = r.overlap ? r.tenants : 0;

    const int CH = r.CH;
    const size_t NN = (size_t)gm.N * gm.N;
    const ChunkStager stage{ (const float *)images, ref->images.p, images_on_device != 0, n_img, CH, NN };
    if (int rc = stage.prime()) return rc;
    auto front = [&](int c0, int ci, int nb, const Lane &L, hipEvent_t ev_pre) -> int {
        HIPCHK(hipMemcpyAsync(L.rows_in.p, rows_in + (size_t)c0 * PPM_NCOL, (size_t)nb * PPM_NCOL * sizeof(double), hipMemcpyHostToDevice, cur_stream()));
        const float *d_img = stage.chunk_ptr(c0, ci);
        if (int rc = launch_prep(ref->spill, d_img, L.rows_in.p, nb, gm, r.Rm_px, r.fall_px, cfg->normalize, cfg->invert, 1, 1, ref->band.p, L.wring.p,
                                 ref->samples.p, r.S_pad, L.Il.p, L.cw.p,
                                 (cfg->global_search && !r.sep_search) ? ref->Wp.p : nullptr, ref->C2.p, ref->nI.p, nullptr, r.focus_on ? r.focus_px : nullptr)) return rc;
        if (r.sep_search)
            if (int rc = launch_prep(ref->spill, d_img, L.rows_in.p, nb, gm, cfg->search_mask_radius / gm.a, r.fall_px, cfg->normalize, cfg->invert, 1, 1,
                                     ref->band.p, nullptr, nullptr, 0, nullptr, nullptr, ref->Wp.p, ref->C2.p, ref->nI.p)) return rc;
        if (cfg->global_search) if (int rc = search_stage(r, nb, L, ev_pre)) return rc;
        return 0;
    };
    auto back = [&](int nb, const Lane &L) -> int {
        if (cfg->global_search) hits_local_stage(r, nb, L);
        else rows_stage(r, nb, L);
        return finish_chunk(r, nb, L);
    };
    auto download = [&](int c0, int nb, const Lane &L) -> int {
        HIPCHK(hipMemcpyAsync(rows_out + (size_t)c0 * PPM_NCOL, L.rows_out.p, (size_t)nb * PPM_NCOL * sizeof(double), hipMemcpyDeviceToHost, cur_stream()));
        return 0;
    };
    if (!r.overlap) {
        const Lane &L = ref->lane[0];
        for (int c0 = 0, ci = 0; c0 < n_img; c0 += CH, ci++) {
            const int nb = std::min(CH, n_img - c0);
            if (int rc = front(c0, ci, nb, L, nullptr)) return rc;
            if (int rc = back(nb, L)) return rc;
            if (int rc = stage.prefetch_next(c0, ci)) return rc;
            if (int rc = download(c0, nb, L)) return rc;
            if (int rc = stage.sync()) return rc;
        }
        refine_counts(r);
        return 0;
    }
    OverlapStreams os;
    if (int rc = os.open(ref)) return rc;
    int prev_c0 = 0, prev_nb = 0;
    for (int c0 = 0, ci = 0; ; c0 += CH, ci++) {
        const bool more = c0 < n_img;
        const int lane = ci & 1, nb = more ? std::min(CH, n_img - c0) : 0;
        if (more) {
            if (ci >= 2) HIPCHK(hipStreamWaitEvent(cur_stream(), os.done[lane], 0));
            if (int rc = front(c0, ci, nb, ref->lane[lane], os.pre[lane])) return rc;
            HIPCHK(hipEventRecord(os.ready[lane], cur_stream()));
        }
        if (ci >= 1) {
            StreamScope sb(ref->local, ref->copy);
            HIPCHK(hipStreamWaitEvent(cur_stream(), os.ready[lane ^ 1], 0));
            if (more) HIPCHK(hipStreamWaitEvent(cur_stream(), os.pre[lane], 0));
            if (int rc = back(prev_nb, ref->lane[lane ^ 1])) return rc;
            if (int rc = download(prev_c0, prev_nb, ref->lane[lane ^ 1])) return rc;
            HIPCHK(hipEventRecord(os.done[lane ^ 1], cur_stream()));
        }
        if (!more) break;
        if (int rc = stage.prefetch_next(c0, ci)) return rc;
        if (int rc = stage.sync()) return rc;
        prev_c0 = c0; prev_nb = nb;
    }
    if (int rc = os.drain()) return rc;
    refine_counts(r);
    return 0;
}


const char *ppm_refine_note(ppm_ref_t *ref) { return ref ? ref->note.c_str() : ""; }

int ppm_refine_last_sections(ppm_ref_t *ref) { return ref ? ref->last_sections : 0; }
int ppm_refine_last_overlap(ppm_ref_t *ref) { return ref ? ref->last_overlap : 0; }

int ppm_refine_last_counts(ppm_ref_t *ref, long *n_global, long *n_local, long *samples_global, long *samples_local) {
    if (!ref) return fail(-22, "null reference");
    if (n_global) *n_global = ref->last_counts[0];
    if (n_local) *n_local = ref->last_counts[1];
    if (samples_global) *samples_global = ref->last_counts[2];
    if (samples_local) *samples_local = ref->last_counts[3];
    return 0;
}

}
```

### pyp_amd/csrc/ppm_dev.h

```cpp
#pragma once
#include <hip/hip_runtime.h>
#include <stdint.h>

namespace ppm {

constexpr float kPiF = 3.14159265358979323846f;

__device__ __forceinline__ float2 cmul(float2 a, float2 b) { return make_float2(a.x * b.x - a.y * b.y, a.x * b.y + a.y * b.x); }
__device__ __forceinline__ float2 cadd(float2 a, float2 b) { return make_float2(a.x + b.x, a.y + b.y); }
__device__ __forceinline__ float2 csub(float2 a, float2 b) { return make_float2(a.x - b.x, a.y - b.y); }


__device__ __forceinline__ void lds_barrier() {
    asm volatile("s_waitcnt lgkmcnt(0)\n\ts_barrier" ::: "memory");
}

constexpr int kDppXor1 = 0xB1, kDppXor2 = 0x4E, kDppHalfMirror = 0x141, kDppMirror = 0x140, kDppRor8 = 0x128;
template <int CTRL> __device__ __forceinline__ float dpp_mov(float x) {
    return __uint_as_float((unsigned)__builtin_amdgcn_update_dpp(0, (int)__float_as_uint(x), CTRL, 0xf, 0xf, false));
}
template <int CTRL> __device__ __forceinline__ int dpp_mov(int x) { return __builtin_amdgcn_update_dpp(0, x, CTRL, 0xf, 0xf, false); }
template <int CTRL, int ROWS> __device__ __forceinline__ int dpp_from(int x) { return __builtin_amdgcn_update_dpp(0, x, CTRL, ROWS, 0xf, false); }
__device__ __forceinline__ int wave_scan_add(int v) {
    v += dpp_from<0x111, 0xf>(v); v += dpp_from<0x112, 0xf>(v); v += dpp_from<0x114, 0xf>(v); v += dpp_from<0x118, 0xf>(v);
// ... 52 lines not shown
    int q = (int)((float)i * inv);
    const int r = i - q * d;
    return r < 0 ? q - 1 : (r >= d ? q + 1 : q);
}

__device__ inline void lds_fft(float2 *buf, const FftPlan &pl, int nlines, int lstride, bool inverse, int tid, int nthr, const float2 *tw) {
    const int n = pl.n;
    const float sgn = inverse ? 1.f : -1.f;
    int Lp = 1;
    for (int st = 0; st < pl.nfac; st++) {
        const int r = pl.fac[st], L = Lp * r, m = n / r, tws = n / L;
        const float inv_m = 1.0f / (float)m, inv_Lp = 1.0f / (float)Lp;
        lds_barrier();
        for (int i = tid; i < nlines * m; i += nthr) {
            const int line = fast_div(i, m, inv_m), t = i - line * m, blk = fast_div(t, Lp, inv_Lp), j = t - blk * Lp;
            float2 *p = buf + line * lstride + blk * L + j;
            float2 x[7];
#pragma unroll
            for (int q = 0; q < 7; q++) {
                if (q < r) {
                    float2 v = p[q * Lp];
                    if (q > 0) { float2 w = tw[q * j * tws]; w.y *= sgn; v = cmul(v, w); }
                    x[q] = v;
                }
            }
            if (r == 2) {
                p[0] = cadd(x[0], x[1]); p[Lp] = csub(x[0], x[1]);
            } else if (r == 4) {
                float2 t0 = cadd(x[0], x[2]), t1 = csub(x[0], x[2]), t2 = cadd(x[1], x[3]), d = csub(x[1], x[3]);
                float2 jd = make_float2(-sgn * d.y, sgn * d.x);
                p[0] = cadd(t0, t2); p[2 * Lp] = csub(t0, t2);
                p[Lp] = cadd(t1, jd); p[3 * Lp] = csub(t1, jd);
            } else if (r == 3) {
                float2 sm = cadd(x[1], x[2]), d = csub(x[1], x[2]);
                float2 h = make_float2(x[0].x - 0.5f * sm.x, x[0].y - 0.5f * sm.y);
                const float c = 0.8660254037844386f * sgn;
                float2 jd = make_float2(-c * d.y, c * d.x);
                p[0] = cadd(x[0], sm); p[Lp] = cadd(h, jd); p[2 * Lp] = csub(h, jd);
            } else if (r == 5) {
                const float c1 = 0.30901699437494745f, c2 = -0.8090169943749475f, s1 = 0.9510565162951535f, s2 = 0.5877852522924731f;
                float2 a1 = cadd(x[1], x[4]), a2 = cadd(x[2], x[3]), b1 = csub(x[1], x[4]), b2 = csub(x[2], x[3]);
                float2 t1 = make_float2(x[0].x + c1 * a1.x + c2 * a2.x, x[0].y + c1 * a1.y + c2 * a2.y);
                float2 t2 = make_float2(x[0].x + c2 * a1.x + c1 * a2.x, x[0].y + c2 * a1.y + c1 * a2.y);
                float2 u1 = make_float2(s1 * b1.x + s2 * b2.x, s1 * b1.y + s2 * b2.y);
                float2 u2 = make_float2(s2 * b1.x - s1 * b2.x, s2 * b1.y - s1 * b2.y);
                float2 j1 = make_float2(-sgn * u1.y, sgn * u1.x), j2 = make_float2(-sgn * u2.y, sgn * u2.x);
                p[0] = make_float2(x[0].x + a1.x + a2.x, x[0].y + a1.y + a2.y);
                p[Lp] = cadd(t1, j1); p[4 * Lp] = csub(t1, j1);
                p[2 * Lp] = cadd(t2, j2); p[3 * Lp] = csub(t2, j2);
            } else {
                const float c1 = 0.6234898018587336f, c2 = -0.2225209339563144f, c3 = -0.9009688679024191f;
                const float s1 = 0.7818314824680298f, s2 = 0.9749279121818236f, s3 = 0.4338837391175581f;
                float2 a1 = cadd(x[1], x[6]), a2 = cadd(x[2], x[5]), a3 = cadd(x[3], x[4]);
                float2 b1 = csub(x[1], x[6]), b2 = csub(x[2], x[5]), b3 = csub(x[3], x[4]);
                float2 t1 = make_float2(x[0].x + c1 * a1.x + c2 * a2.x + c3 * a3.x, x[0].y + c1 * a1.y + c2 * a2.y + c3 * a3.y);
                float2 t2 = make_float2(x[0].x + c2 * a1.x + c3 * a2.x + c1 * a3.x, x[0].y + c2 * a1.y + c3 * a2.y + c1 * a3.y);
                float2 t3 = make_float2(x[0].x + c3 * a1.x + c1 * a2.x + c2 * a3.x, x[0].y + c3 * a1.y + c1 * a2.y + c2 * a3.y);
                float2 u1 = make_float2(s1 * b1.x + s2 * b2.x + s3 * b3.x, s1 * b1.y + s2 * b2.y + s3 * b3.y);
                float2 u2 = make_float2(s2 * b1.x - s3 * b2.x - s1 * b3.x, s2 * b1.y - s3 * b2.y - s1 * b3.y);
                float2 u3 = make_float2(s3 * b1.x - s1 * b2.x + s2 * b3.x, s3 * b1.y - s1 * b2.y + s2 * b3.y);
                float2 j1 = make_float2(-sgn * u1.y, sgn * u1.x), j2 = make_float2(-sgn * u2.y, sgn * u2.x), j3 = make_float2(-sgn * u3.y, sgn * u3.x);
                p[0] = make_float2(x[0].x + a1.x + a2.x + a3.x, x[0].y + a1.y + a2.y + a3.y);
                p[Lp] = cadd(t1, j1); p[6 * Lp] = csub(t1, j1);
                p[2 * Lp] = cadd(t2, j2); p[5 * Lp] = csub(t2, j2);
                p[3 * Lp] = cadd(t3, j3); p[4 * Lp] = csub(t3, j3);
            }
        }
        Lp = L;
    }
    lds_barrier();
}
__device__ inline void lds_fft(float2 *buf, const FftPlan &pl, int nlines, int lstride, bool inverse, int tid, int nthr) {
    lds_fft(buf, pl, nlines, lstride, inverse, tid, nthr, pl.tw);
}

__device__ __forceinline__ void bfly4(float2 &a, float2 &b, float2 &c, float2 &d) {
    const float2 t0 = cadd(a, c), t1 = csub(a, c), t2 = cadd(b, d), e = csub(b, d);
    const float2 t3 = make_float2(e.y, -e.x);
    a = cadd(t0, t2); c = csub(t0, t2); b = cadd(t1, t3); d = csub(t1, t3);
}
__device__ __forceinline__ void dft16(float2 (&x)[16]) {
#pragma unroll
    for (int n1 = 0; n1 < 4; n1++) bfly4(x[n1], x[n1 + 4], x[n1 + 8], x[n1 + 12]);
    constexpr float C1 = 0.9238795325112867f, S1 = 0.3826834323650898f, C2 = 0.7071067811865476f;
    x[1 + 4] = cmul(x[1 + 4], make_float2(C1, -S1));
    x[1 + 8] = cmul(x[1 + 8], make_float2(C2, -C2));
    x[1 + 12] = cmul(x[1 + 12], make_float2(S1, -C1));
    x[2 + 4] = cmul(x[2 + 4], make_float2(C2, -C2));
    x[2 + 8] = make_float2(x[2 + 8].y, -x[2 + 8].x);
    x[2 + 12] = cmul(x[2 + 12], make_float2(-C2, -C2));
    x[3 + 4] = cmul(x[3 + 4], make_float2(S1, -C1));
    x[3 + 8] = cmul(x[3 + 8], make_float2(-C2, -C2));
    x[3 + 12] = cmul(x[3 + 12], make_float2(-C1, S1));
#pragma unroll
    for (int k2 = 0; k2 < 4; k2++) bfly4(x[4 * k2], x[4 * k2 + 1], x[4 * k2 + 2], x[4 * k2 + 3]);
#pragma unroll
    for (int i = 0; i < 4; i++)
#pragma unroll
        for (int j = i + 1; j < 4; j++) { const float2 t = x[4 * i + j]; x[4 * i + j] = x[4 * j + i]; x[4 * j + i] = t; }
}

__device__ inline void lds_fft256(float2 *buf, int nlines, int lstride, int tid, int nthr, const float2 *tw) {
    const int work = nlines * 16;
    lds_barrier();
    for (int base = 0; base < work; base += nthr) {
        const int w = base + tid, line = w >> 4, n1 = w & 15;
        float2 x[16];
        float2 *row = buf + line * lstride;
        if (w < work) {
#pragma unroll
            for (int n2 = 0; n2 < 16; n2++) x[n2] = row[n1 + 16 * n2];
        }
        lds_barrier();
        if (w < work) {
            dft16(x);
#pragma unroll
            for (int k2 = 0; k2 < 16; k2++) {
                float2 v = x[k2];
                if (k2 > 0) { float2 t = tw[n1 * k2]; t.y = -t.y; v = cmul(v, t); }
                row[k2 * 17 + n1] = v;
            }
        }
    }
    lds_barrier();
    for (int base = 0; base < work; base += nthr) {
        const int w = base + tid, line = w >> 4, k2 = w & 15;
        float2 y[16];
        float2 *row = buf + line * lstride;
        if (w < work) {
#pragma unroll
            for (int n1 = 0; n1 < 16; n1++) y[n1] = row[k2 * 17 + n1];
        }
        lds_barrier();
        if (w < work) {
            dft16(y);
#pragma unroll
            for (int k1 = 0; k1 < 16; k1++) row[16 * k1 + k2] = y[k1];
        }
    }
    lds_barrier();
}

struct CubeView { const float2 *cube; int NBX, NBY, off; unsigned LB; float scale; };

__host__ __device__ __forceinline__ size_t cube_element(int NBX, int NBY, unsigned LB, int copy, int x, int y, int z) {
    const int xs = x - 2 * copy;
    return (size_t)copy * LB + ((size_t)((z >> 1) * NBY + (y >> 1)) * NBX + (xs >> 2)) * 16 + ((z & 1) * 2 + (y & 1)) * 4 + (xs & 3);
}

struct CubeTaps { float4 a, b, c, d; float fx, fy, fz; bool cj; };

typedef float cube_v4f __attribute__((ext_vector_type(4)));

__device__ __forceinline__ CubeTaps cube_fetch(const CubeView &cv, float X, float Y, float Z) {
    CubeTaps t;
    X *= cv.scale; Y *= cv.scale; Z *= cv.scale;
    t.cj = X < 0.f;
    if (t.cj) { X = -X; Y = -Y; Z = -Z; }
    const float xf = floorf(X), yf = floorf(Y), zf = floorf(Z);
    t.fx = X - xf; t.fy = Y - yf; t.fz = Z - zf;
    const int x0 = (int)xf, y0 = (int)yf + cv.off, z0 = (int)zf + cv.off;
    const bool second = (x0 & 3) == 3;
    const int xs = second ? x0 - 2 : x0;
    const unsigned rowb = (unsigned)cv.NBX * 128u, planeb = __umul24(rowb, (unsigned)cv.NBY);
    const unsigned xl = (unsigned)(xs >> 2) * 128u + (unsigned)(xs & 3) * 8u + (second ? cv.LB * 8u : 0u);
    const unsigned yl0 = __umul24((unsigned)(y0 >> 1), rowb) + (unsigned)(y0 & 1) * 32u, dy = (y0 & 1) ? rowb - 32u : 32u;
    const unsigned zl0 = __umul24((unsigned)(z0 >> 1), planeb) + (unsigned)(z0 & 1) * 64u, dz = (z0 & 1) ? planeb - 64u : 64u;
    const unsigned oa = xl + yl0 + zl0, ob = oa + dy, oc = oa + dz, od = ob + dz;
    const __amdgpu_buffer_rsrc_t rs = __builtin_amdgcn_make_buffer_rsrc((void *)cv.cube, 0, (int)(2u * cv.LB * 8u), 0x00020000);
    const cube_v4f a = __builtin_amdgcn_raw_buffer_load_b128(rs, (int)oa, 0, 0), b = __builtin_amdgcn_raw_buffer_load_b128(rs, (int)ob, 0, 0);
    const cube_v4f c = __builtin_amdgcn_raw_buffer_load_b128(rs, (int)oc, 0, 0), d = __builtin_amdgcn_raw_buffer_load_b128(rs, (int)od, 0, 0);
    t.a = make_float4(a.x, a.y, a.z, a.w); t.b = make_float4(b.x, b.y, b.z, b.w);
    t.c = make_float4(c.x, c.y, c.z, c.w); t.d = make_float4(d.x, d.y, d.z, d.w);
    return t;
}

struct CubeTab { const uint2 *ty0, *tz0; const unsigned *tx0; };
__host__ __device__ inline int cube_tab_radius(int band_px, float scale) { return (int)ceilf((float)(band_px + 2) * scale) + 2; }
__host__ __device__ inline size_t cube_tab_bytes(int R) { return R > 0 ? (size_t)2 * (2 * R + 2) * 8 + (size_t)(R + 2) * 4 : 0; }
__device__ inline CubeTab cube_tab_fill(const CubeView &cv, void *mem, int R, int tid, int nthr) {
    uint2 *ty = (uint2 *)mem, *tz = ty + (2 * R + 2);
    unsigned *tx = (unsigned *)(tz + (2 * R + 2));
    const unsigned rowb = (unsigned)cv.NBX * 128u, planeb = rowb * (unsigned)cv.NBY;
    for (int i = tid; i < 2 * R + 2; i += nthr) {
        const int y0 = i - (R + 1) + cv.off;
        ty[i] = make_uint2((unsigned)(y0 >> 1) * rowb + (unsigned)(y0 & 1) * 32u, (y0 & 1) ? rowb - 32u : 32u);
        tz[i] = make_uint2((unsigned)(y0 >> 1) * planeb + (unsigned)(y0 & 1) * 64u, (y0 & 1) ? planeb - 64u : 64u);
    }
    for (int x0 = tid; x0 < R + 2; x0 += nthr) {
        const bool second = (x0 & 3) == 3;
        const int xs = second ? x0 - 2 : x0;
        tx[x0] = (unsigned)(xs >> 2) * 128u + (unsigned)(xs & 3) * 8u + (second ? cv.LB * 8u : 0u);
    }
    CubeTab t; t.ty0 = ty + (R + 1); t.tz0 = tz + (R + 1); t.tx0 = tx;
    return t;
}

__device__ __forceinline__ int floor_to_int(float x) { int i; asm("v_cvt_flr_i32_f32 %0, %1" : "=v"(i) : "v"(x)); return i; }

__device__ __forceinline__ CubeTaps cube_fetch_tab(const CubeView &cv, const CubeTab &tb, float X, float Y, float Z) {
    CubeTaps t;
    t.cj = X < 0.f;
    if (t.cj) { X = -X; Y = -Y; Z = -Z; }
    t.fx = __builtin_amdgcn_fractf(X); t.fy = __builtin_amdgcn_fractf(Y); t.fz = __builtin_amdgcn_fractf(Z);
    const unsigned xl = tb.tx0[floor_to_int(X)];
    const uint2 ey = tb.ty0[floor_to_int(Y)], ez = tb.tz0[floor_to_int(Z)];
    const unsigned oa = xl + ey.x + ez.x, ob = oa + ey.y, oc = oa + ez.y, od = ob + ez.y;
    const __amdgpu_buffer_rsrc_t rs = __builtin_amdgcn_make_buffer_rsrc((void *)cv.cube, 0, (int)(2u * cv.LB * 8u), 0x00020000);
    const cube_v4f a = __builtin_amdgcn_raw_buffer_load_b128(rs, (int)oa, 0, 0), b = __builtin_amdgcn_raw_buffer_load_b128(rs, (int)ob, 0, 0);
    const cube_v4f c = __builtin_amdgcn_raw_buffer_load_b128(rs, (int)oc, 0, 0), d = __builtin_amdgcn_raw_buffer_load_b128(rs, (int)od, 0, 0);
    t.a = make_float4(a.x, a.y, a.z, a.w); t.b = make_float4(b.x, b.y, b.z, b.w);
    t.c = make_float4(c.x, c.y, c.z, c.w); t.d = make_float4(d.x, d.y, d.z, d.w);
    return t;
}

__device__ __forceinline__ float2 cube_interp(const CubeTaps &t) {
    const float fx = t.fx, fy = t.fy, fz = t.fz;
    const float ar = t.a.x + fx * (t.a.z - t.a.x), ai = t.a.y + fx * (t.a.w - t.a.y);
    const float br = t.b.x + fx * (t.b.z - t.b.x), bi = t.b.y + fx * (t.b.w - t.b.y);
    const float cr = t.c.x + fx * (t.c.z - t.c.x), ci = t.c.y + fx * (t.c.w - t.c.y);
    const float dr = t.d.x + fx * (t.d.z - t.d.x), di = t.d.y + fx * (t.d.w - t.d.y);
    const float er = ar + fy * (br - ar), ei = ai + fy * (bi - ai);
    const float gr = cr + fy * (dr - cr), gi = ci + fy * (di - ci);
    const float rr = er + fz * (gr - er), ri = ei + fz * (gi - ei);
    return make_float2(rr, t.cj ? -ri : ri);
}

__device__ __forceinline__ float2 sample_cube(const CubeView &cv, float X, float Y, float Z) { return cube_interp(cube_fetch(cv, X, Y, Z)); }

struct CtfP { float lambda, cs, dsum, ddif, c2a, s2a, extra, inv_na2; };

__host__ __device__ __forceinline__ CtfP ctf_from_row(const double *row, int N, double a) {
    CtfP c;
    double v = row[PPM_VOLTAGE] * 1000.0;
    double lam = 12.2639 / sqrt(v + 0.97845e-6 * v * v);
    double w = row[PPM_AMP], ast = row[PPM_ANGAST] * 3.14159265358979323846 / 180.0;
    c.lambda = (float)lam;
    c.cs = (float)(row[PPM_CS] * 1e7);
    c.dsum = (float)(row[PPM_DF1] + row[PPM_DF2]);
    c.ddif = (float)(row[PPM_DF1] - row[PPM_DF2]);
    c.c2a = (float)cos(2.0 * ast);
    c.s2a = (float)sin(2.0 * ast);
    c.extra = (float)(row[PPM_PSHIFT] + atan(w / sqrt(1.0 - w * w)));
    c.inv_na2 = (float)(1.0 / ((double)N * a * N * a));
    return c;
}

__device__ __forceinline__ float ctf_eval(const CtfP &c, int kx, int ky) {
    float k2 = (float)(kx * kx + ky * ky);
    if (k2 == 0.f) return -sinf(c.extra);
    float s2 = k2 * c.inv_na2;
    float ik2 = 1.0f / k2;
    float c2 = (float)(kx * kx - ky * ky) * ik2, s2p = (float)(2 * kx * ky) * ik2;
    float df = 0.5f * (c.dsum + c.ddif * (c2 * c.c2a + s2p * c.s2a));
    float chi = kPiF * c.lambda * s2 * (df - 0.5f * c.cs * c.lambda * c.lambda * s2) + c.extra;
    return -sinf(chi);
}

__device__ __forceinline__ float ctf_eval_fast(const CtfP &c, int kx, int ky) {
    float k2 = (float)(kx * kx + ky * ky);
    float s2 = k2 * c.inv_na2;
    float ik2 = __frcp_rn(fmaxf(k2, 1.f));
    float c2 = (float)(kx * kx - ky * ky) * ik2, s2p = (float)(2 * kx * ky) * ik2;
    float df = 0.5f * (c.dsum + c.ddif * (c2 * c.c2a + s2p * c.s2a));
    float chi = kPiF * c.lambda * s2 * (df - 0.5f * c.cs * c.lambda * c.lambda * s2) + c.extra;
    float rev = chi * 0.15915494309189535f; rev -= floorf(rev);
    return -__sinf(6.283185307179586f * rev);
}

__device__ __forceinline__ void unpack_sample(uint32_t u, int &kx, int &ky, int &alpha, int &ring) {
    kx = (int)(u & 511u);
    ky = (int)((u >> 9) & 1023u) - 256;
    alpha = (int)((u >> 19) & 3u);
    ring = (int)(u >> 21);
}

}
```

### pyp_amd/csrc/ppm_geom.h

```cpp
#pragma once
#include <algorithm>
#include <cmath>
#include <cstdint>
#include <cstring>
#include <string>
#include <vector>

#include "../../include/ppm.h"

namespace ppm {

constexpr double kPi = 3.14159265358979323846;

#ifdef __HIPCC__
#define PPM_HD __host__ __device__
#define PPM_FORCEINLINE __forceinline__
#define PPM_UNROLL _Pragma("unroll")
#else
#define PPM_HD
#define PPM_FORCEINLINE inline
#define PPM_UNROLL
#endif
PPM_HD inline void sincos_rad(double t, double *s, double *c) {
#ifdef __HIP_DEVICE_COMPILE__
// ... 126 lines not shown
}

PPM_HD inline void angles_from_matrix(const double M[9], double &psi, double &theta, double &phi) {
    const double r2d = 180.0 / kPi;
    double ct = M[8] > 1 ? 1 : (M[8] < -1 ? -1 : M[8]);
    double st = std::sqrt(M[2] * M[2] + M[5] * M[5]);
    if (st > 1e-7) { theta = std::atan2(st, ct) * r2d; phi = std::atan2(M[5], M[2]) * r2d; psi = std::atan2(M[7], -M[6]) * r2d; }
    else { theta = ct > 0 ? 0.0 : 180.0; phi = 0.0; psi = (ct > 0 ? std::atan2(M[3], M[0]) : std::atan2(M[3], -M[0])) * r2d; }
    if (psi < 0) psi += 360;
    if (phi < 0) phi += 360;
}

PPM_HD inline void mat_mul3(const double *a, const double *b, double *c) {
    double t[9];
    PPM_UNROLL
    for (int i = 0; i < 3; i++)
        PPM_UNROLL
        for (int j = 0; j < 3; j++) {
            double v = 0;
            PPM_UNROLL
            for (int k = 0; k < 3; k++) v += a[i * 3 + k] * b[k * 3 + j];
            t[i * 3 + j] = v;
        }
    PPM_UNROLL
    for (int i = 0; i < 9; i++) c[i] = t[i];
}
PPM_HD inline void rot_xyz(int k, double deg, double R[9]) {
    double s, c;
    sincos_rad(deg * kPi / 180.0, &s, &c);
    if (k == 0) { R[0] = 1; R[1] = 0; R[2] = 0; R[3] = 0; R[4] = c; R[5] = -s; R[6] = 0; R[7] = s; R[8] = c; }
    else if (k == 1) { R[0] = c; R[1] = 0; R[2] = s; R[3] = 0; R[4] = 1; R[5] = 0; R[6] = -s; R[7] = 0; R[8] = c; }
    else { R[0] = c; R[1] = -s; R[2] = 0; R[3] = s; R[4] = c; R[5] = 0; R[6] = 0; R[7] = 0; R[8] = 1; }
}
inline std::vector<double> sva_rotation_grid(double gstep, const char *sym) {
    std::vector<double> grid_d;
    double phi_max, theta_max;
    sym_limits(sym, phi_max, theta_max);
    int n_theta = (int)std::floor(theta_max / gstep + 0.5) + 1; if (n_theta < 2) n_theta = 2;
    int n_psi = (int)std::floor(360.0 / gstep + 0.5); if (n_psi < 1) n_psi = 1;
    for (int i = 0; i < n_theta; i++) {
        const double th = theta_max * i / (n_theta - 1);
        int np = (int)std::floor(phi_max * std::sin(th * kPi / 180.0) / gstep + 0.5); if (np < 1) np = 1;
        for (int j = 0; j < np; j++) for (int k = 0; k < n_psi; k++) {
            double G[9]; euler_matrix(k * 360.0 / n_psi, th, phi_max * j / np, G);
            grid_d.insert(grid_d.end(), G, G + 9);
        }
    }
    return grid_d;
}

struct TiltRot { double a[9], b[9], ai[9], bi[9]; };
PPM_HD inline void tilt_rotations(double tilt, double axis, TiltRot &r) { rot_xyz(1, -tilt, r.a); rot_xyz(2, axis, r.b); rot_xyz(2, -axis, r.ai); rot_xyz(1, tilt, r.bi); }
PPM_HD inline void csp_row_pose(const double N[9], const double p[3], const TiltRot &r, double tsx, double tsy, double M[9], double g[2]) {
    double t[9];
    mat_mul3(N, r.a, t); mat_mul3(t, r.b, M);
    const double q0 = -p[0], q1 = -p[1], q2 = -p[2];
    double u[3], v[2];
    PPM_UNROLL
    for (int i = 0; i < 3; i++) u[i] = r.bi[i * 3] * q0 + r.bi[i * 3 + 1] * q1 + r.bi[i * 3 + 2] * q2;
    PPM_UNROLL
    for (int i = 0; i < 2; i++) v[i] = r.ai[i * 3] * u[0] + r.ai[i * 3 + 1] * u[1] + r.ai[i * 3 + 2] * u[2];
    g[0] = v[0] + tsx; g[1] = v[1] + tsy;
}
PPM_HD inline void csp_row_pose(const double N[9], const double p[3], double tilt, double axis, double tsx, double tsy, double M[9], double g[2]) {
    TiltRot r; tilt_rotations(tilt, axis, r);
    csp_row_pose(N, p, r, tsx, tsy, M, g);
}
PPM_HD inline void unit_apply_delta(double *N, double *p, const double *d) {
    for (int k = 0; k < 3; k++)
        if (d[k] != 0.0) { double R[9]; rot_xyz(k, d[k], R); mat_mul3(N, R, N); }
    for (int k = 0; k < 3; k++) p[k] += d[3 + k];
}

template <int A, int B, int K>
PPM_HD PPM_FORCEINLINE void col_mix(const double *M, double s, double c, double *out) {
    PPM_UNROLL
    for (int r = 0; r < 3; r++) {
        const double ma = M[r * 3 + A], mb = M[r * 3 + B];
        out[r * 3 + A] = ma * c + mb * s;
        out[r * 3 + B] = mb * c - ma * s;
        out[r * 3 + K] = M[r * 3 + K];
    }
}
PPM_HD inline void rot_step(const double *M, int which, int tilt_frame, double hdeg, double *out) {
    double s, c;
    sincos_rad(hdeg * kPi / 180.0, &s, &c);
    if (which == 0) { col_mix<0, 1, 2>(M, s, c, out); return; }
    if (tilt_frame) {
        if (which == 1) col_mix<1, 2, 0>(M, s, c, out); else col_mix<2, 0, 1>(M, s, c, out);
        return;
    }
    if (which == 2) { double r[9] = { c, -s, 0, s, c, 0, 0, 0, 1 }; mat_mul3(r, M, out); return; }
    double psi, th, ph; angles_from_matrix(M, psi, th, ph);
    double cp = std::cos(ph * kPi / 180.0), sp = std::sin(ph * kPi / 180.0);
    double rz[9] = { cp, -sp, 0, sp, cp, 0, 0, 0, 1 }, rzt[9] = { cp, sp, 0, -sp, cp, 0, 0, 0, 1 }, ry[9] = { c, 0, s, 0, 1, 0, -s, 0, c };
    double T[9], L[9];
    mat_mul3(rz, ry, T); mat_mul3(T, rzt, L); mat_mul3(L, M, out);
}

constexpr double kNoProbe = -1e300;
template <int NP>
PPM_HD inline void compass_trial(double f0, const double *pang, const double *psh, const int *en, double ha, double hs,
                                 const double *acc, const double *tol, double *d, double *fp, double *fm) {
    const double *q = pang;
    for (int i = 0; i < NP; i++) {
        d[i] = 0; fp[i] = fm[i] = kNoProbe;
        if (i == 3 && psh) q = psh;
        if (!en[i]) continue;
        const double h = i < 3 ? ha : hs;
        const bool okp = !tol || std::fabs(acc[i] + h) <= tol[i] + 1e-9, okm = !tol || std::fabs(acc[i] - h) <= tol[i] + 1e-9;
        const double p = okp ? q[0] : kNoProbe, m = okm ? q[1] : kNoProbe;
        q += 2;
        fp[i] = p; fm[i] = m;
        if (okp && okm) {
            const double den = 2.0 * f0 - p - m;
            if (den > 1e-12) { const double t = 0.5 * h * (p - m) / den; d[i] = t > h ? h : (t < -h ? -h : t); }
            else { const double best = p > m ? p : m; d[i] = best > f0 ? (p > m ? h : -h) : 0.0; }
        } else if (okp) d[i] = p > f0 ? h : 0.0;
        else if (okm) d[i] = m > f0 ? -h : 0.0;
        if (tol) {
            if (acc[i] + d[i] > tol[i]) d[i] = tol[i] - acc[i];
            if (acc[i] + d[i] < -tol[i]) d[i] = -tol[i] - acc[i];
        }
    }
}
enum CompassMove { kCompassStay = 0, kCompassTrial, kCompassProbe };
template <int NP>
PPM_HD inline CompassMove compass_accept(double f0, double ft, const double *fp, const double *fm, const int *en, int &bi, int &bs, double &fb) {
    bi = -1; bs = 0; fb = f0;
    for (int i = 0; i < NP; i++) {
        if (!en[i]) continue;
        if (fp[i] > fb) { fb = fp[i]; bi = i; bs = 1; }
        if (fm[i] > fb) { fb = fm[i]; bi = i; bs = -1; }
    }
    if (ft > f0 && ft >= fb) return kCompassTrial;
    return bi >= 0 ? kCompassProbe : kCompassStay;
}

inline double march_band(double bf, int N, double rm_px, double ha, double hs, bool any_ang, bool any_sh, double rcap) {
    if (bf < 0) return rcap;
    double d = 0;
    if (any_ang) d = rm_px * ha * kPi / 180.0;
    if (any_sh && hs > d) d = hs;
    if (!(d > 0)) return rcap;
    double rit = bf * N / (2.0 * kPi * d);
    if (rit < 4.0) rit = 4.0;
    return rit < rcap ? rit : rcap;
}
inline int compass_iterations(double ha, double hs, double steptol, int min_iters) {
    const double m = std::max(ha, hs);
    const int T = m > steptol ? (int)std::ceil(std::log(m / steptol) / std::log(2.0)) : min_iters;
    return std::min(12, std::max(min_iters, T));
}
struct LdsRegion { unsigned off, bytes, elem; };
struct PrepLds {
    LdsRegion T;
    LdsRegion Wk;
    LdsRegion ringq;
    LdsRegion ringc;
    LdsRegion ringpw;
    LdsRegion red;
    LdsRegion stat;
    LdsRegion fmask;
    LdsRegion tw;
    LdsRegion perm;
    LdsRegion iperm;
    unsigned total;
};
constexpr int prep_threads(bool scratch_free) { return scratch_free ? 512 : 256; }
constexpr PrepLds prep_lds_regions(bool scratch_free, int N, int B, int L, int nc, int TS, int WS) {
    const unsigned waves = prep_threads(scratch_free) / 64, nb = (unsigned)(B + 2), n = (unsigned)N;
    const unsigned tb = (unsigned)nc * (unsigned)TS * 8, wb = (unsigned)L * (unsigned)WS * 8;
    PrepLds l = {};
    l.T = { 0, tb, 8 };
    l.Wk = { scratch_free ? 0 : tb, wb, 8 };
    l.ringq = { scratch_free ? (tb > wb ? tb : wb) : tb + wb, nb * 8, 8 };
    l.ringc = { l.ringq.off + l.ringq.bytes, nb * 4, 4 };
    l.ringpw = { l.ringc.off + l.ringc.bytes, nb * 4, 4 };
    l.red = { (l.ringpw.off + l.ringpw.bytes + 15) & ~15u, 5 * waves * 8, 16 };
    l.stat = { l.red.off + l.red.bytes, (4 + waves) * 4, 4 };
    l.fmask = { l.stat.off + l.stat.bytes, 8 * 4, 4 };
    l.tw = { l.fmask.off + l.fmask.bytes, n * 8, 8 };
    l.perm = { l.tw.off + l.tw.bytes, scratch_free ? 0 : n * 2, 2 };
    l.iperm = { l.perm.off + l.perm.bytes, scratch_free ? 0 : n * 2, 2 };
    return l;
}
constexpr unsigned prep_lds_tail(bool scratch_free, int N, int B) {
    const PrepLds l = prep_lds_regions(scratch_free, N, B, 0, 0, 0, 0);
    return l.iperm.off + l.iperm.bytes + 16 + 16;
}
constexpr PrepLds prep_lds(bool scratch_free, int N, int B, int L, int nc, int TS, int WS) {
    PrepLds l = prep_lds_regions(scratch_free, N, B, L, nc, TS, WS);
    l.total = l.ringq.off + prep_lds_tail(scratch_free, N, B);
    return l;
}
struct PrepPlan {
    bool scratch_free;
    int threads, L, nc, nchunks;
    int TS, WS;
    PrepLds lds;
    const char *err;
};
inline PrepPlan prep_plan(int N, int B, int W) {
    PrepPlan p = {};
    p.scratch_free = N == 256; p.threads = prep_threads(p.scratch_free);
    if (p.scratch_free) {
        p.TS = 273; p.WS = 272;
        p.L = 64; p.nc = 64; p.nchunks = (std::min(W, 128) + 63) / 64;
        p.lds = prep_lds(true, N, B, p.L, p.nc, p.TS, p.WS);
        if (p.lds.total > 160u * 1024) p.err = "pre-processing kernel: LDS plan exceeds 160 KB";
        return p;
    }
    constexpr size_t budget = 40 * 1024;
    const size_t tail = prep_lds_tail(false, N, B);
    p.TS = N + 1; p.WS = N;
    p.L = std::max(1, std::min(8 * p.threads / N, N / 2));
    while (p.L >= 1 && ((N / 2) % p.L || (size_t)p.L * p.WS * 8 + tail + (size_t)p.TS * 8 > budget / 2 + 8192)) p.L--;
    if (p.L < 1) { p.err = "pre-processing kernel: row buffer does not fit the LDS"; return p; }
    const size_t wk = (size_t)p.L * p.WS * 8;
    const size_t left = budget - tail > wk ? budget - tail - wk : 0;
    p.nc = std::max(1, std::min(W, (int)(left / ((size_t)p.TS * 8))));
    p.nc = std::max(1, std::min(p.nc, 12 * p.threads / N));
    p.nchunks = (W + p.nc - 1) / p.nc;
    p.nc = (W + p.nchunks - 1) / p.nchunks;
    p.lds = prep_lds(false, N, B, p.L, p.nc, p.TS, p.WS);
    if (p.lds.total > budget) p.err = "pre-processing kernel: LDS plan exceeds its budget";
    return p;
}

PPM_HD inline void score_columns(double cc, double r_lo, double r_hi, double *score, double *sigma, double *logp) {
    double res = 1.0 - cc * cc; if (res < 1e-6) res = 1e-6;
    *score = 100.0 * cc; *sigma = std::sqrt(res);
    *logp = -0.5 * (kPi * (r_hi * r_hi - r_lo * r_lo)) * (std::log(2.0 * kPi * res) + 1.0);
}

struct SampleList {
    std::vector<uint32_t> packed;
    std::vector<int> ring_off;
};

inline uint32_t pack_sample(int kx, int ky, int alpha, int ring) {
    return (uint32_t)kx | ((uint32_t)(ky + 256) << 9) | ((uint32_t)alpha << 19) | ((uint32_t)ring << 21);
}

inline void build_samples(const Geom &g, SampleList &sl) {
    int B = g.B;
    std::vector<std::vector<uint32_t>> rings(B + 2);
    double r2 = g.r_hi * g.r_hi;
    for (int ky = -B; ky <= B; ky++) for (int kx = 0; kx <= B; kx++) {
        double k2 = (double)kx * kx + (double)ky * ky;
        if (k2 >= r2 || k2 == 0) continue;
        int b = (int)std::floor(std::sqrt(k2));
        rings[b].push_back(pack_sample(kx, ky, kx == 0 ? 1 : 2, b));
    }
    constexpr int kRingBand = 4;
    sl.packed.clear(); sl.ring_off.assign(B + 3, 0);
    for (int b0 = 0; b0 <= B + 1; b0 += kRingBand) {
        struct Grp { double key; int ring; int first; };
        std::vector<Grp> grps;
        const int b1 = std::min(b0 + kRingBand - 1, B + 1);
        for (int b = b0; b <= b1; b++) {
            while (rings[b].size() % 16) rings[b].push_back(pack_sample(0, 0, 0, b));
            const int G = (int)rings[b].size() / 16;
            for (int gidx = 0; gidx < G; gidx++) grps.push_back({ (gidx + 0.5) / G, b, gidx * 16 });
        }
        std::stable_sort(grps.begin(), grps.end(), [](const Grp &x, const Grp &y) { return x.key < y.key; });
        for (const Grp &gr : grps) for (int i = 0; i < 16; i++) sl.packed.push_back(rings[gr.ring][gr.first + i]);
        for (int b = b0; b <= b1; b++) sl.ring_off[b + 1] = (int)sl.packed.size();
    }
    sl.ring_off[B + 2] = (int)sl.packed.size();
}

inline void rot_axis(const double ax[3], double deg, double *m) {
    double n = std::sqrt(ax[0] * ax[0] + ax[1] * ax[1] + ax[2] * ax[2]);
    double x = ax[0] / n, y = ax[1] / n, z = ax[2] / n, t = deg * kPi / 180, c = std::cos(t), s = std::sin(t), C = 1 - c;
    double r[9] = { c + x * x * C, x * y * C - z * s, x * z * C + y * s, y * x * C + z * s, c + y * y * C, y * z * C - x * s,
                    z * x * C - y * s, z * y * C + x * s, c + z * z * C };
    std::memcpy(m, r, sizeof(r));
}
inline int symmetry_ops(const char *sym, std::vector<double> &ops) {
    double gens[27]; int ng = 0;
    double z[3] = { 0, 0, 1 }, x[3] = { 1, 0, 0 }, d111[3] = { 1, 1, 1 };
    if (!sym || !sym[0]) sym = "C1";
    char t = sym[0] >= 'a' ? sym[0] - 32 : sym[0];
    int n = std::atoi(sym + 1);
    if (t == 'C' && n >= 1) { rot_axis(z, 360.0 / n, gens); ng = 1; }
    else if (t == 'D' && n >= 1) { rot_axis(z, 360.0 / n, gens); rot_axis(x, 180, gens + 9); ng = 2; }
    else if (t == 'T') { rot_axis(z, 180, gens); rot_axis(d111, 120, gens + 9); ng = 2; }
    else if (t == 'O') { rot_axis(z, 90, gens); rot_axis(d111, 120, gens + 9); ng = 2; }
    else if (t == 'I') {
        double phi = (1 + std::sqrt(5.0)) / 2, a5[3] = { 0, 1, phi };
        rot_axis(z, 180, gens); rot_axis(d111, 120, gens + 9); rot_axis(a5, 72, gens + 18); ng = 3;
    } else return -1;
    ops.assign(9, 0.0); ops[0] = ops[4] = ops[8] = 1.0;
    int cnt = 1;
    for (bool grew = true; grew;) {
        grew = false;
        for (int i = 0; i < cnt && cnt < 60; i++) for (int j = 0; j < ng && cnt < 60; j++) {
            double c[9]; mat_mul3(&ops[i * 9], gens + j * 9, c);
            bool found = false;
            for (int k = 0; k < cnt && !found; k++) {
                double d = 0; for (int q = 0; q < 9; q++) d += std::fabs(ops[k * 9 + q] - c[q]);
                if (d < 1e-6) found = true;
            }
            if (!found) { ops.insert(ops.end(), c, c + 9); cnt++; grew = true; }
        }
// ... 6 lines not shown
```

### pyp_amd/csrc/ppm_kernels2.h

```cpp
#pragma once
#include "ppm_kernels.h"

namespace ppm {

struct LState { double M[9]; double sh[2]; double f, ha, hs; int particle; int pad; double fc; };

constexpr int kMaxIters = 24;
struct LocalP {
    CubeView cv; const uint32_t *samples; const float2 *Il; const float *cw;
    int S_pad, nrings, N;
    int nr;
    int tabR;
    float rlo2, ring_signed;
    LState *states; int T, final_rescore; int en[5];
    float rmax2_it[kMaxIters]; int S_it[kMaxIters];
    float rmax2_final; int S_final;
    float rmax2_class; int S_class;
    int use_priors; double pmean[5], pw[5];
};

__device__ inline double d_prior_pen(const LocalP &P, const double *M, double shx, double shy) {
    double v[5]; angles_from_matrix(M, v[0], v[1], v[2]); v[3] = shx; v[4] = shy;
    double pen = 0;
#pragma unroll
    for (int i = 0; i < 5; i++) {
        if (!(P.pw[i] > 0)) continue;
        double d = v[i] - P.pmean[i];
        if (i < 3) { d = fmod(d, 360.0); if (d > 180.0) d -= 360.0; if (d < -180.0) d += 360.0; }
        pen += P.pw[i] * d * d;
    }
    return pen;
}

constexpr int kMaxCand = 13;
constexpr int kMaxGroup = 7;

__device__ __forceinline__ float group16_sum_dpp(float v) {
    v += __int_as_float(__builtin_amdgcn_mov_dpp(__float_as_int(v), 0xB1, 0xF, 0xF, true));
    v += __int_as_float(__builtin_amdgcn_mov_dpp(__float_as_int(v), 0x4E, 0xF, 0xF, true));
    v += __int_as_float(__builtin_amdgcn_mov_dpp(__float_as_int(v), 0x141, 0xF, 0xF, true));
    v += __int_as_float(__builtin_amdgcn_mov_dpp(__float_as_int(v), 0x140, 0xF, 0xF, true));
    return v;
}

struct SweepPlan {
    float m[kMaxGroup][6]; float sh[kMaxCand][2]; int nv[kMaxGroup]; int slot0[kMaxGroup]; int ng, nslots, S_used, q_same; float rmax2;
    float ms[kMaxGroup][6];
    int bsl[kMaxCand];
};

__device__ __forceinline__ double group8_sum_d(double v) {
    v += __shfl_xor(v, 1, 64); v += __shfl_xor(v, 2, 64); v += __shfl_xor(v, 4, 64);
    return v;
}

__host__ __device__ inline size_t ring_lds_bytes(int nw, int nq, int nr) { return ((size_t)nq * nw * nr + (size_t)nq * nw + nw) * sizeof(float); }
__host__ __device__ inline size_t ring_lds_bytes8(int nw, int nq, int nr) { return (ring_lds_bytes(nw, nq, nr) + 7) & ~(size_t)7; }

struct SweepCtx {
    CubeView cv; const uint32_t *samples; const float2 *Il; const float *cw;
    float invN, rlo2, ring_signed; int nr, nw;
    float *ringA, *sumB, *sumC; double *score;
    CubeTab tab;
};

template <bool TAB>
__device__ __forceinline__ void sweep_plan(SweepPlan &plan, const SweepCtx &C, const int tid, const int nthr) {
    const int lane = tid & 63, wave = tid >> 6, nw = C.nw, nr = C.nr;
    float *const ringA = C.ringA, *const sumB = C.sumB, *const sumC = C.sumC; double *const score = C.score;
    const float2 *const Il = C.Il; const float *const cw = C.cw; const float invN = C.invN;
    const int nslots = plan.nslots, ng = plan.ng, S_used = plan.S_used;
    const float rmax2 = plan.rmax2;
    for (int i = tid; i < nslots * nw * nr; i += nthr) ringA[i] = 0.f;
    if (tid < kMaxCand * nw) sumB[tid] = 0.f;
    if (tid < ng * 6) (&plan.ms[0][0])[tid] = (&plan.m[0][0])[tid] * C.cv.scale;
    { const int g = nthr > 64 ? tid - 64 : tid; if (g >= 0 && g < ng) { const int q0 = plan.slot0[g]; for (int v = 0; v < plan.nv[g]; v++) plan.bsl[q0 + v] = q0; } }
    __syncthreads();
    float *const myA = ringA + wave * nr, *const myB = sumB + wave;
    const int q_same = plan.q_same, strideA = nw * nr;
    const bool head = (lane & 15) == 0;
    float accC = 0.f;
    for (int s0 = 0; s0 < S_used; s0 += nthr) {
        const int s = s0 + tid;
        int kx = 0, ky = 0, al = 0, ring = 0;
        float2 iv = make_float2(0.f, 0.f); float c = 0.f;
        if (s < S_used) {
            unpack_sample(C.samples[s], kx, ky, al, ring);
            float k2 = (float)(kx * kx + ky * ky);
            if (!(k2 < rmax2 && k2 >= C.rlo2)) al = 0;
            iv = Il[s]; c = cw[s];
        }
        const float fal = (float)al, fkx = (float)kx, fky = (float)ky;
        accC += fal * (iv.x * iv.x + iv.y * iv.y);
        const float ac = fal * c, ax = ac * iv.x, ay = ac * iv.y, w = ac * c;
        auto turned = [&](int q, float &bx, float &by) {
            float rev = -(fkx * plan.sh[q][0] + fky * plan.sh[q][1]) * invN;
            rev -= floorf(rev);
            const float sn = __sinf(6.283185307179586f * rev), cs = __cosf(6.283185307179586f * rev);
            bx = ax * cs + ay * sn; by = ay * cs - ax * sn;
        };
        float b0x, b0y;
        turned(0, b0x, b0y);
        auto fetch = [&](int g) {
            const float *m = plan.ms[g];
            const float X = m[0] * fkx + m[1] * fky, Y = m[2] * fkx + m[3] * fky, Z = m[4] * fkx + m[5] * fky;
            if constexpr (TAB) return cube_fetch_tab(C.cv, C.tab, X, Y, Z);
            else { CubeView one = C.cv; one.scale = 1.f; return cube_fetch(one, X, Y, Z); }
        };
        const bool mine = head && ring < nr;
        float *const cellA = myA + ring;
        auto score_group = [&](int g, const CubeTaps &t) {
            const float2 v = cube_interp(t);
            const int nv = __builtin_amdgcn_readfirstlane(plan.nv[g]), q0 = __builtin_amdgcn_readfirstlane(plan.slot0[g]);
            const float n2 = w * (v.x * v.x + v.y * v.y);
            if (nv == 1 && q0 <= q_same) {
                float av = b0x * v.x + b0y * v.y, bv = n2;
                av += __int_as_float(__builtin_amdgcn_mov_dpp(__float_as_int(av), 0xB1, 0xF, 0xF, true));
                bv += __int_as_float(__builtin_amdgcn_mov_dpp(__float_as_int(bv), 0xB1, 0xF, 0xF, true));
                av += __int_as_float(__builtin_amdgcn_mov_dpp(__float_as_int(av), 0x4E, 0xF, 0xF, true));
                bv += __int_as_float(__builtin_amdgcn_mov_dpp(__float_as_int(bv), 0x4E, 0xF, 0xF, true));
                av += __int_as_float(__builtin_amdgcn_mov_dpp(__float_as_int(av), 0x141, 0xF, 0xF, true));
                bv += __int_as_float(__builtin_amdgcn_mov_dpp(__float_as_int(bv), 0x141, 0xF, 0xF, true));
                av += __int_as_float(__builtin_amdgcn_mov_dpp(__float_as_int(av), 0x140, 0xF, 0xF, true));
                bv += __int_as_float(__builtin_amdgcn_mov_dpp(__float_as_int(bv), 0x140, 0xF, 0xF, true));
                if (mine) { atomicAdd(cellA + q0 * strideA, av); atomicAdd(myB + q0 * nw, bv); }
                return;
            }
            const float bv = group16_sum_dpp(n2);
            if (mine) atomicAdd(myB + q0 * nw, bv);
            for (int k = 0; k < nv; k++) {
                const int q = q0 + k;
                float bx = b0x, by = b0y;
                if (q > q_same) turned(q, bx, by);
                const float av = group16_sum_dpp(bx * v.x + by * v.y);
                if (mine) atomicAdd(cellA + q * strideA, av);
            }
        };
        CubeTaps A = fetch(0), B;
        int g = 0;
        for (; g + 2 < ng; g += 2) {
            B = fetch(g + 1); __builtin_amdgcn_sched_barrier(0); score_group(g, A);
            A = fetch(g + 2); __builtin_amdgcn_sched_barrier(0); score_group(g + 1, B);
        }
        if (g + 1 < ng) { B = fetch(g + 1); __builtin_amdgcn_sched_barrier(0); score_group(g, A); score_group(g + 1, B); }
        else score_group(g, A);
    }
    accC = wave_sum(accC);
    if (lane == 0) sumC[wave] = accC;
    __syncthreads();
    {
        const int j = tid & 7;
        for (int slot0_ = 0; slot0_ < nslots; slot0_ += nthr >> 3) {
        const int slot = slot0_ + (tid >> 3);
        double sa = 0;
        if (slot < nslots)
            for (int b = j; b < nr; b += 8) {
                const float *cell = ringA + (size_t)slot * nw * nr + b;
                float a = cell[0];
                for (int w = 1; w < nw; w++) a += cell[w * nr];
                sa += ((float)b <= C.ring_signed) ? (double)a : fabs((double)a);
            }
        sa = group8_sum_d(sa);
        if (slot < nslots && j == 0) {
            const int bs = plan.bsl[slot];
            float fb = sumB[bs * nw], fc = sumC[0];
            for (int w = 1; w < nw; w++) { fb += sumB[bs * nw + w]; fc += sumC[w]; }
            const double sb = fb, sc = fc;
            score[slot] = (sb > 0 && sc > 0) ? sa / sqrt(sb * sc) : 0.0;
        }
        }
    }
    __syncthreads();
}

#ifndef PPM_LOCAL_MINW
#define PPM_LOCAL_MINW 4
#endif
template <bool TAB>
__global__ void __launch_bounds__(256, PPM_LOCAL_MINW) k_local(LocalP P) {
    __shared__ SweepPlan plan;
    extern __shared__ float lsm[];
    __shared__ double score[kMaxCand];
    __shared__ LState st;
    __shared__ double sfp[5], sfm[5], sd[5], sMt[9], sshq[2], sf0;
    __shared__ double spen[kMaxCand];
    const int tid = threadIdx.x, nthr = blockDim.x;
    const int nw = nthr >> 6, nr = P.nr;
    float *const ringA = lsm, *const sumB = lsm + kMaxCand * nw * nr, *const sumC = sumB + kMaxCand * nw;
    if (tid == 0) st = P.states[blockIdx.x];
    __syncthreads();
    const int part = st.particle;
    const float2 *Il = P.Il + (size_t)part * P.S_pad;
    const float *cw = P.cw + (size_t)part * P.S_pad;
    const float invN = 1.0f / (float)P.N;
    const int tilt = P.en[1] && P.en[2];

    SweepCtx SC;
    SC.cv = P.cv; SC.samples = P.samples; SC.Il = Il; SC.cw = cw; SC.invN = invN; SC.rlo2 = P.rlo2; SC.ring_signed = P.ring_signed;
    SC.nr = nr; SC.nw = nw; SC.ringA = ringA; SC.sumB = sumB; SC.sumC = sumC; SC.score = score;
    if constexpr (TAB) SC.tab = cube_tab_fill(P.cv, (char *)lsm + ring_lds_bytes8(nw, kMaxCand, nr), P.tabR, tid, nthr);
    auto set_rot = [&](int g, const double *M) {
        plan.m[g][0] = (float)M[0]; plan.m[g][1] = (float)M[1]; plan.m[g][2] = (float)M[3];
        plan.m[g][3] = (float)M[4]; plan.m[g][4] = (float)M[6]; plan.m[g][5] = (float)M[7];
    };
    auto single = [&](const double *M, const double *sh) {
        set_rot(0, M); plan.sh[0][0] = (float)sh[0]; plan.sh[0][1] = (float)sh[1];
        plan.nv[0] = 1; plan.slot0[0] = 0; plan.ng = 1; plan.nslots = 1; plan.q_same = 0;
    };

    int nfree = 0;
    for (int i = 0; i < 5; i++) nfree += P.en[i] ? 1 : 0;
    enum { PH_COMPASS, PH_TRIAL, PH_FINAL, PH_CLASS, PH_DONE };
    int it = 0, phase = PH_COMPASS;
    if (nfree == 0 || P.T <= 0) {
        if (tid == 0) for (int t = 0; t < P.T; t++) { st.ha *= 0.5; st.hs *= 0.5; }
        phase = P.final_rescore ? PH_FINAL : PH_DONE;
        __syncthreads();
    }
    while (phase != PH_DONE) {
        if (phase == PH_COMPASS) {
            int nang = 0;
            for (int i = 0; i < 3; i++) nang += P.en[i] ? 2 : 0;
            if (tid < 6) {
                const int i = tid >> 1, sg = tid & 1;
                if (P.en[i]) {
                    int g = 0;
                    for (int k = 0; k < i; k++) g += P.en[k] ? 2 : 0;
                    g += sg;
                    double Mq[9];
                    rot_step(st.M, i, tilt, sg ? -st.ha : st.ha, Mq);
                    set_rot(g, Mq); plan.nv[g] = 1; plan.slot0[g] = g;
                    plan.sh[g][0] = (float)st.sh[0]; plan.sh[g][1] = (float)st.sh[1];
                    if (P.use_priors) spen[g] = d_prior_pen(P, Mq, st.sh[0], st.sh[1]);
                }
            } else if (tid == 6) {
                int q = nang, g = nang;
                set_rot(g, st.M); plan.slot0[g] = q;
                plan.sh[q][0] = (float)st.sh[0]; plan.sh[q][1] = (float)st.sh[1];
                if (P.use_priors) spen[q] = d_prior_pen(P, st.M, st.sh[0], st.sh[1]);
                q++;
                int nv = 1;
                for (int i = 3; i < 5; i++) {
                    if (!P.en[i]) continue;
                    for (int sg = 0; sg < 2; sg++) {
                        double shq[2] = { st.sh[0], st.sh[1] };
                        shq[i - 3] += sg ? -st.hs : st.hs;
                        plan.sh[q][0] = (float)shq[0]; plan.sh[q][1] = (float)shq[1];
                        if (P.use_priors) spen[q] = d_prior_pen(P, st.M, shq[0], shq[1]);
                        q++; nv++;
                    }
                }
                plan.nv[g] = nv;
                plan.ng = g + 1; plan.nslots = q; plan.q_same = nang; plan.S_used = P.S_it[it]; plan.rmax2 = P.rmax2_it[it];
            }
        } else if (phase == PH_FINAL) {
            if (tid == 0) { single(st.M, st.sh); plan.S_used = P.S_final; plan.rmax2 = P.rmax2_final; }
        } else if (phase == PH_CLASS) {
            if (tid == 0) { plan.S_used = P.S_class; plan.rmax2 = P.rmax2_class; }
        }
        __syncthreads();
        sweep_plan<TAB>(plan, SC, tid, nthr);
        if (tid == 0) {
            if (phase == PH_COMPASS) {
                int qc = 0;
                for (int i = 0; i < 3; i++) qc += P.en[i] ? 2 : 0;
                if (P.use_priors) for (int k = 0; k < plan.nslots; k++) score[k] -= spen[k];
                const double f0 = score[qc];
                sf0 = f0;
                compass_trial<5>(f0, score, score + qc + 1, P.en, st.ha, st.hs, nullptr, nullptr, sd, sfp, sfm);
                double T9[9];
                for (int k = 0; k < 9; k++) sMt[k] = st.M[k];
                for (int i = 0; i < 3; i++) if (P.en[i] && sd[i] != 0) { rot_step(sMt, i, tilt, sd[i], T9); for (int k = 0; k < 9; k++) sMt[k] = T9[k]; }
                sshq[0] = st.sh[0] + sd[3]; sshq[1] = st.sh[1] + sd[4];
                single(sMt, sshq);
            } else if (phase == PH_TRIAL) {
                const double ft = score[0] - (P.use_priors ? d_prior_pen(P, sMt, sshq[0], sshq[1]) : 0.0), f0 = sf0;
                int bi, bs; double fb;
                const CompassMove mv = compass_accept<5>(f0, ft, sfp, sfm, P.en, bi, bs, fb);
                st.f = f0;
                if (mv == kCompassTrial) {
                    for (int k = 0; k < 9; k++) st.M[k] = sMt[k];
                    st.sh[0] = sshq[0]; st.sh[1] = sshq[1]; st.f = ft;
                } else if (mv == kCompassProbe) {
                    if (bi < 3) { double T9[9]; rot_step(st.M, bi, tilt, bs * st.ha, T9); for (int k = 0; k < 9; k++) st.M[k] = T9[k]; }
                    else st.sh[bi - 3] += bs * st.hs;
                    st.f = fb;
                }
                st.ha *= 0.5; st.hs *= 0.5;
            } else if (phase == PH_FINAL) st.f = st.fc = score[0];
            else st.fc = score[0];
        }
        if (phase == PH_COMPASS) phase = PH_TRIAL;
        else if (phase == PH_TRIAL) { it++; phase = it < P.T ? PH_COMPASS : (P.final_rescore ? PH_FINAL : PH_DONE); }
        else if (phase == PH_FINAL) phase = P.S_class > 0 ? PH_CLASS : PH_DONE;
        else phase = PH_DONE;
        __syncthreads();
    }
    if (tid == 0) P.states[blockIdx.x] = st;
}

__global__ void k_states_from_hits(const Hit *hits, LState *states, int n, int K, const double *dir_theta,
                                   const double *dir_phi, int n_psi, double dpsi, double step, double ha0, double hs0) {
    int i = blockIdx.x * blockDim.x + threadIdx.x;
    if (i >= n * K) return;
    Hit h = hits[i];
    LState s;
    int dir = h.orient / n_psi, k = h.orient - dir * n_psi;
    euler_matrix(k * dpsi, dir_theta[dir], dir_phi[dir], s.M);
    s.sh[0] = h.sx * step; s.sh[1] = h.sy * step;
    s.f = h.cc; s.fc = h.cc; s.ha = ha0; s.hs = hs0; s.particle = i / K; s.pad = 0;
    states[i] = s;
}

__global__ void k_states_from_rows(const double *rows, LState *states, int n, double a, double ha0, double hs0) {
    int i = blockIdx.x * blockDim.x + threadIdx.x;
    if (i >= n) return;
    const double *r = rows + (size_t)i * PPM_NCOL;
    LState s;
    euler_matrix(r[PPM_PSI], r[PPM_THETA], r[PPM_PHI], s.M);
    s.sh[0] = r[PPM_XSHIFT] / a; s.sh[1] = r[PPM_YSHIFT] / a;
    s.f = 0; s.fc = 0; s.ha = ha0; s.hs = hs0; s.particle = i; s.pad = 0;
    states[i] = s;
}

__global__ void k_select_best(const LState *in, LState *out, int n, int K) {
    int i = blockIdx.x * blockDim.x + threadIdx.x;
    if (i >= n) return;
    int b = 0;
    for (int k = 1; k < K; k++) if (in[(size_t)i * K + k].f > in[(size_t)i * K + b].f) b = k;
    out[i] = in[(size_t)i * K + b];
}

struct DefocusP {
    CubeView cv; const uint32_t *samples; const float2 *Il; const float *wring; int S_pad, nrings, N, B;
    float rlo2, rmax2, ring_signed, a;
    const double *rows; LState *states; float *ddef;
    int nt; float step;
    int tchunk;
    double *all_scores;
    float rcls2;
};

__global__ void __launch_bounds__(256) k_defocus(DefocusP P) {
    constexpr int MAXT = 2 * PPM_MAX_DEFOCUS_STEPS + 1, NW = 4;
    extern __shared__ float dsm[];
    __shared__ double score[MAXT];
    __shared__ CtfP ctf0;
    __shared__ float m_s[6], sh_s[2];
    const int p = blockIdx.x, tid = threadIdx.x, lane = tid & 63, wave = tid >> 6, T = 2 * P.nt + 1, TC = P.tchunk, nr = P.nrings;
    float *const ringA = dsm, *const sumB = dsm + (size_t)TC * NW * nr, *const sumC = sumB + TC * NW;
    if (tid == 0) {
        const LState &st = P.states[p];
        ctf0 = ctf_from_row(P.rows + (size_t)p * PPM_NCOL, P.N, (double)P.a);
        m_s[0] = (float)st.M[0]; m_s[1] = (float)st.M[1]; m_s[2] = (float)st.M[3]; m_s[3] = (float)st.M[4]; m_s[4] = (float)st.M[6]; m_s[5] = (float)st.M[7];
        sh_s[0] = (float)st.sh[0]; sh_s[1] = (float)st.sh[1];
    }
    __syncthreads();
    const float2 *Il = P.Il + (size_t)p * P.S_pad;
    const float *wr = P.wring + (size_t)p * (P.B + 2);
    const float invN = 1.0f / (float)P.N;
    auto score_offsets = [&](const int t0, const int tn, const float rmax2) {
        for (int i = tid; i < tn * NW * nr + TC * NW; i += 256) { if (i < tn * NW * nr) ringA[i] = 0.f; else sumB[i - tn * NW * nr] = 0.f; }
        __syncthreads();
        float *const myA = ringA + wave * nr, *const myB = sumB + wave;
        float accC = 0.f;
        for (int s0 = 0; s0 < P.S_pad; s0 += 256) {
            const int s = s0 + tid;
            int kx = 0, ky = 0, al = 0, ring = 0;
            float2 iv = make_float2(0.f, 0.f);
            if (s < P.S_pad) {
                unpack_sample(P.samples[s], kx, ky, al, ring);
                const float k2 = (float)(kx * kx + ky * ky);
                if (!(k2 < rmax2 && k2 >= P.rlo2)) al = 0;
                iv = Il[s];
            }
            const float fal = (float)al, fkx = (float)kx, fky = (float)ky;
            accC += fal * (iv.x * iv.x + iv.y * iv.y);
            float2 pv = sample_cube(P.cv, m_s[0] * fkx + m_s[1] * fky, m_s[2] * fkx + m_s[3] * fky, m_s[4] * fkx + m_s[5] * fky);
            float rev = -(fkx * sh_s[0] + fky * sh_s[1]) * invN;
            rev -= floorf(rev);
            const float sn = __sinf(6.283185307179586f * rev), cs = __cosf(6.283185307179586f * rev);
            const float mr = pv.x * cs - pv.y * sn, mi = pv.x * sn + pv.y * cs;
            const float a0 = fal * (iv.x * mr + iv.y * mi), b0 = fal * (pv.x * pv.x + pv.y * pv.y), wgt = al ? wr[ring] : 0.f;
            for (int t = 0; t < tn; t++) {
                CtfP c = ctf0;
                c.dsum += 2.f * (float)(t0 + t - P.nt) * P.step;
                const float ct = ctf_eval(c, kx, ky) * wgt;
                const float av = group16_sum_dpp(a0 * ct), bv = group16_sum_dpp(b0 * ct * ct);
                if ((lane & 15) == 0 && ring < nr) { atomicAdd(&myA[(size_t)t * NW * nr + ring], av); atomicAdd(&myB[t * NW], bv); }
            }
        }
        accC = wave_sum(accC);
        if (lane == 0) sumC[wave] = accC;
        __syncthreads();
        for (int tb = 0; tb < tn; tb += 32) {
            const int t = tb + (tid >> 3), j = tid & 7;
            double sa = 0;
            if (t < tn)
                for (int b = j; b < nr; b += 8) {
                    const float *cell = ringA + (size_t)t * NW * nr + b;
                    const float a = ((cell[0] + cell[nr]) + cell[2 * nr]) + cell[3 * nr];
                    sa += ((float)b <= P.ring_signed) ? (double)a : fabs((double)a);
                }
            sa = group8_sum_d(sa);
            if (t < tn && j == 0) {
                const double sb = ((sumB[t * NW] + sumB[t * NW + 1]) + sumB[t * NW + 2]) + sumB[t * NW + 3];
                const double sc = ((sumC[0] + sumC[1]) + sumC[2]) + sumC[3];
                score[t0 + t] = (sb > 0 && sc > 0) ? sa / sqrt(sb * sc) : 0.0;
            }
        }
        __syncthreads();
    };
    for (int t0 = 0; t0 < T; t0 += TC) score_offsets(t0, min(TC, T - t0), P.rmax2);
    if (P.all_scores) {
        if (tid < T) P.all_scores[(size_t)p * T + tid] = score[tid];
        return;
    }
    __shared__ int s_bt;
    if (tid == 0) {
        int bt = P.nt; double bf = score[P.nt];
        for (int t = 0; t < T; t++) if (t != P.nt && score[t] > bf) { bf = score[t]; bt = t; }
        P.states[p].f = P.states[p].fc = bf;
        P.ddef[p] = (float)(bt - P.nt) * P.step;
        s_bt = bt;
    }
    if (P.rcls2 > 0.f) {
        __syncthreads();
        const int bt = s_bt;
        score_offsets(bt, 1, P.rcls2);
        if (tid == 0) P.states[p].fc = score[bt];
    }
}

__global__ void k_rows_out(const LState *states, const double *rows_in, double *rows_out, int n, double a,
                           double r_cls, double r_lo, const float *ddef) {
    int i = blockIdx.x * blockDim.x + threadIdx.x;
    if (i >= n) return;
    const LState &s = states[i];
    double *o = rows_out + (size_t)i * PPM_NCOL;
    const double *r = rows_in + (size_t)i * PPM_NCOL;
    for (int c = 0; c < PPM_NCOL; c++) o[c] = r[c];
    double psi, th, ph; angles_from_matrix(s.M, psi, th, ph);
    o[PPM_PSI] = psi; o[PPM_THETA] = th; o[PPM_PHI] = ph;
    o[PPM_XSHIFT] = s.sh[0] * a; o[PPM_YSHIFT] = s.sh[1] * a;
    if (ddef) { o[PPM_DF1] = r[PPM_DF1] + (double)ddef[i]; o[PPM_DF2] = r[PPM_DF2] + (double)ddef[i]; }
    double score_cls;
    score_columns(s.fc, r_lo, r_cls, &score_cls, &o[PPM_SIGMA], &o[PPM_LOGP]);
    o[PPM_SCORE] = 100.0 * s.f;
}

struct PartIns {
// ... 516 lines not shown
```

### pyp_amd/host.py

```python
import ctypes as C

import numpy as np

from . import lib
from .abi import NCOL, STATS_COLS, K_NAMES, CreateMaskCfg, CreateMaskInfo, FinalCfg, FrameCfg, FrameInfo, LocresCfg, LocresInfo, MaskCfg, PostCfg, PostInfo, ReconCfg, RefineCfg


def _sync_producer(t):
    import torch
    torch.cuda.current_stream(t.device).synchronize()


def _images_arg(images, n_img, box):
    if hasattr(images, "data_ptr") and hasattr(images, "is_cuda"):
        if not images.is_cuda:
            images = images.numpy()
        else:
            if not getattr(images, "ready", False):
                _sync_producer(images)
            if str(images.dtype) != "torch.float32" or not images.is_contiguous():
                raise ValueError("ERROR: device image stack must be contiguous float32")
            if images.numel() != n_img * box * box:
                raise ValueError("ERROR: image stack size does not match the rows")
            return C.c_void_p(images.data_ptr()), 1, images
    a = np.ascontiguousarray(images, dtype=np.float32)
    if a.size != n_img * box * box:
        raise ValueError("ERROR: image stack size does not match the rows")
    return lib.ptr(a), 0, a


def _volumes_arg(volumes, n_vol, box):
    if hasattr(volumes, "is_cuda") and volumes.is_cuda:
        if str(volumes.dtype) != "torch.float32" or not volumes.is_contiguous() or volumes.numel() != n_vol * box ** 3:
            raise ValueError("ERROR: device volumes must be contiguous float32 of V * box^3 elements")
        if not getattr(volumes, "ready", False):
            _sync_producer(volumes)
        return C.c_void_p(volumes.data_ptr()), 1, volumes
    a = np.ascontiguousarray(volumes.numpy() if hasattr(volumes, "numpy") else volumes, dtype=np.float32)
    if a.size != n_vol * box ** 3:
        raise ValueError("ERROR: volumes do not match the poses")
    return lib.ptr(a), 0, a


class Reference:

    def __init__(self, vol, max_band_px=None, device=0, pad=1, ring_weight=None):
        lib.init(device)
        vol = np.ascontiguousarray(vol, dtype=np.float32)
        if vol.ndim != 3 or len(set(vol.shape)) != 1:
            raise ValueError("ERROR: reference must be a cubic volume")
        self.n = vol.shape[0]
        band = self.n / 2 if max_band_px is None else float(max_band_px)
        w = None if ring_weight is None else np.ascontiguousarray(ring_weight, dtype=np.float32)
        self.h = lib.load().ppm_reference_create_weighted(lib.ptr(vol), self.n, band, int(pad), None if w is None else lib.ptr(w),
                                                          0 if w is None else int(w.size))
        if not self.h:
            raise lib.PpmError(lib.last_error())

    def refine(self, cfg, images, rows):
        rows = np.ascontiguousarray(rows, dtype=np.float64)
        if rows.ndim != 2 or rows.shape[1] != NCOL:
            raise ValueError("ERROR: rows must be (M, 32)")
        out = np.empty_like(rows)
        p, on_dev, keep = _images_arg(images, len(rows), cfg.box)
        lib.check(lib.load().ppm_refine_batch(self.h, C.byref(cfg), p, on_dev, len(rows), lib.ptr(rows), lib.ptr(out)))
        del keep
        return out

    def match_projections(self, cfg, rows):
        rows = np.ascontiguousarray(rows, dtype=np.float64)
        if rows.ndim != 2 or rows.shape[1] != NCOL:
            raise ValueError("ERROR: rows must be (M, 32)")
        out = np.empty((len(rows), cfg.box, cfg.box), dtype=np.float32)
        lib.check(lib.load().ppm_match_projections(self.h, C.byref(cfg), lib.ptr(rows), len(rows), lib.ptr(out)))
        return out

    def csp_refine(self, cfg, csp_cfg, images, rows, particles, tilts):
        rows = np.array(rows, dtype=np.float64, order="C")
        particles = np.array(particles, dtype=np.float64, order="C")
        tilts = np.array(tilts, dtype=np.float64, order="C")
        if rows.ndim != 2 or rows.shape[1] != NCOL or particles.ndim != 2 or particles.shape[1] != 12 or tilts.ndim != 2 or tilts.shape[1] != 6:
            raise ValueError("ERROR: rows must be (M, 32), particles (P, 12), tilts (T, 6)")
        p, on_dev, keep = _images_arg(images, len(rows), cfg.box)
        lib.check(lib.load().ppm_csp_refine(self.h, C.byref(cfg), C.byref(csp_cfg), p, on_dev, len(rows), lib.ptr(rows), lib.ptr(particles),
                                            len(particles), lib.ptr(tilts), len(tilts)))
        del keep
        return rows, particles, tilts

    def frame_refine(self, cfg, fcfg, images, rows, maps=False):
        rows = np.ascontiguousarray(rows, dtype=np.float64)
        if rows.ndim != 2 or rows.shape[1] != NCOL:
            raise ValueError("ERROR: rows must be (M, 32)")
        L = lib.load()
        nst = C.c_int()
        lib.check(L.ppm_frame_plan(C.byref(fcfg), None, C.byref(nst), None))
        side = 2 * nst.value + 1
        out = np.empty_like(rows)
        info = FrameInfo()
        own = np.zeros((len(rows), side, side), dtype=np.float32) if maps else None
        pooled = np.zeros((len(rows), side, side), dtype=np.float32) if maps else None
        p, on_dev, keep = _images_arg(images, len(rows), cfg.box)
        lib.check(L.ppm_frame_refine(self.h, C.byref(cfg), C.byref(fcfg), p, on_dev, lib.ptr(rows), len(rows), lib.ptr(out),
                                     lib.ptr(own) if maps else None, lib.ptr(pooled) if maps else None, C.byref(info)))
        del keep
        return (out, info.as_dict(), own, pooled) if maps else (out, info.as_dict())

    def sva_align(self, cfg, volumes, wedges, poses, accumulator=None, index=None):
        poses = np.array(poses, dtype=np.float64, order="C")
        if poses.ndim != 2 or poses.shape[1] != 12:
            raise ValueError("ERROR: poses must be (V, 12)")
        w = np.ascontiguousarray(wedges, dtype=np.float32).reshape(len(poses), 2)
        scores = np.zeros(len(poses), dtype=np.float64)
        p, on_dev, keep = _volumes_arg(volumes, len(poses), cfg.box)
        if accumulator is None:
            lib.check(lib.load().ppm_sva_align(self.h, C.byref(cfg), p, on_dev, len(poses), lib.ptr(w), lib.ptr(poses), lib.ptr(scores)))
        else:
            idx = None if index is None else np.ascontiguousarray(index, dtype=np.int64)
            if idx is not None and idx.shape != (len(poses),):
                raise ValueError("ERROR: index must be (V,)")
            if accumulator._ext is not None:
                _sync_producer(accumulator._ext)
            lib.check(lib.load().ppm_sva_align_average(self.h, accumulator.h, C.byref(cfg), p, on_dev, len(poses), lib.ptr(w), lib.ptr(poses), lib.ptr(scores),
                                                       None if idx is None else lib.ptr(idx)))
        del keep
        return poses, scores

    def note(self):
        return (lib.load().ppm_refine_note(self.h) or b"").decode(errors="replace")

    def last_counts(self):
        v = [C.c_long() for _ in range(4)]
        lib.check(lib.load().ppm_refine_last_counts(self.h, *[C.byref(x) for x in v]))
        return dict(zip(("n_global", "n_local", "samples_global", "samples_local"), [x.value for x in v]))

    def last_sections(self):
        return int(lib.load().ppm_refine_last_sections(self.h))

    def last_overlap(self):
        return int(lib.load().ppm_refine_last_overlap(self.h))

    def close(self):
        if getattr(self, "h", None):
            lib.load().ppm_reference_destroy(self.h)
            self.h = None

    def __del__(self):
        try:
            self.close()
        except Exception:
            pass


class Accumulator:

    def __init__(self, box, pixel_size, symmetry="C1", device=0, ext_tensor=None):
        lib.init(device)
        self.box, self.pixel = int(box), float(pixel_size)
        self.nfloats = int(lib.load().ppm_accum_floats(self.box))
        self._ext = ext_tensor
        ext = None
        if ext_tensor is not None:
            if ext_tensor.numel() != self.nfloats or not ext_tensor.is_cuda or not ext_tensor.is_contiguous():
                raise ValueError("ERROR: external accumulator tensor has the wrong size or is not on the GPU")
            ext = C.c_void_p(ext_tensor.data_ptr())
        self.h = lib.load().ppm_accum_create(self.box, self.pixel, symmetry.encode(), ext)
        if not self.h:
            raise lib.PpmError(lib.last_error())

    def insert(self, cfg, images, rows):
        rows = np.ascontiguousarray(rows, dtype=np.float64)
        p, on_dev, keep = _images_arg(images, len(rows), self.box)
        if self._ext is not None:
            _sync_producer(self._ext)
        lib.check(lib.load().ppm_insert_batch(self.h, C.byref(cfg), p, on_dev, len(rows), lib.ptr(rows)))
        del keep

    def sva_insert(self, cfg, volumes, wedges, poses, index=None):
        poses = np.ascontiguousarray(poses, dtype=np.float64)
        if poses.ndim != 2 or poses.shape[1] != 12:
            raise ValueError("ERROR: poses must be (V, 12)")
        w = np.ascontiguousarray(wedges, dtype=np.float32).reshape(len(poses), 2)
        idx = None if index is None else np.ascontiguousarray(index, dtype=np.int64)
        if idx is not None and idx.shape != (len(poses),):
            raise ValueError("ERROR: index must be (V,)")
        p, on_dev, keep = _volumes_arg(volumes, len(poses), self.box)
        if self._ext is not None:
            _sync_producer(self._ext)
        lib.check(lib.load().ppm_sva_insert(self.h, C.byref(cfg), p, on_dev, len(poses), lib.ptr(w), lib.ptr(poses), None if idx is None else lib.ptr(idx)))
        del keep

    def counts(self):
        return [int(lib.load().ppm_accum_count(self.h, 0)), int(lib.load().ppm_accum_count(self.h, 1))]

    def set_counts(self, c0, c1):
        lib.load().ppm_accum_set_count(self.h, 0, int(c0))
        lib.load().ppm_accum_set_count(self.h, 1, int(c1))

    def reduce(self, comm, root=-1):
        if self._ext is not None:
            _sync_producer(self._ext)
        lib.check(lib.load().ppm_accum_reduce(self.h, C.c_void_p(comm), int(root)))

    def download(self):
        a = np.empty(self.nfloats, dtype=np.float32)
        if self._ext is not None:
            _sync_producer(self._ext)
        lib.check(lib.load().ppm_accum_download(self.h, lib.ptr(a)))
        return a

    def add(self, host):
        a = np.ascontiguousarray(host, dtype=np.float32)
        if a.size != self.nfloats:
            raise ValueError("ERROR: dump has the wrong size for this box")
        if self._ext is not None:
            _sync_producer(self._ext)
        lib.check(lib.load().ppm_accum_add(self.h, lib.ptr(a)))

    def finalize(self, fcfg):
        n = self.box
        h1 = np.empty((n, n, n), dtype=np.float32)
        h2 = np.empty_like(h1)
        fl = np.empty_like(h1)
        stats = np.zeros((n // 2 - 1, STATS_COLS), dtype=np.float64)
        if self._ext is not None:
            _sync_producer(self._ext)
        lib.check(lib.load().ppm_finalize(self.h, C.byref(fcfg), lib.ptr(h1), lib.ptr(h2), lib.ptr(fl), lib.ptr(stats)))
        return h1, h2, fl, stats

    def close(self):
        if getattr(self, "h", None):
            lib.load().ppm_accum_destroy(self.h)
            self.h = None

    def __del__(self):
        try:
            self.close()
        except Exception:
            pass


def comm_unique_id():
    buf = (C.c_char * 128)()
    lib.check(lib.load().ppm_comm_unique_id(buf))
    return bytes(buf)


def make_comm(n_ranks, rank, unique_id, device=0):
    lib.init(device)
    if len(unique_id) != 128:
        raise ValueError("ERROR: the communicator id must be 128 bytes")
    buf = (C.c_char * 128).from_buffer_copy(unique_id)
    h = lib.load().ppm_comm_create(int(n_ranks), int(rank), buf)
    if not h:
        raise lib.PpmError(lib.last_error())
    return h


def comm_count(comm):
    n = lib.load().ppm_comm_count(comm)
    if n < 0:
        raise lib.PpmError(lib.last_error())
    return int(n)


def destroy_comm(comm):
    if comm:
        lib.load().ppm_comm_destroy(C.c_void_p(comm))


def extract_boxes(micrograph, coords, box, radius_A, pixel_size, coordinate_binning=1, normalize=True, fix_empty=True,
                  out=None, device=0):
    lib.init(device)
    coords = np.ascontiguousarray(coords, dtype=np.float64).reshape(-1, 2)
    m = len(coords)
    radius_px = float(radius_A) / (float(pixel_size) * float(coordinate_binning))
    if hasattr(micrograph, "is_cuda") and micrograph.is_cuda:
        if str(micrograph.dtype) != "torch.float32" or not micrograph.is_contiguous() or micrograph.dim() != 2:
            raise ValueError("ERROR: device micrograph must be a contiguous 2-D float32 tensor")
        _sync_producer(micrograph)
        ip, idev, rows, cols, keep = C.c_void_p(micrograph.data_ptr()), 1, micrograph.shape[0], micrograph.shape[1], micrograph
    else:
        a = np.ascontiguousarray(micrograph, dtype=np.float32)
        if a.ndim != 2:
            raise ValueError("ERROR: micrograph must be 2-D")
        ip, idev, rows, cols, keep = lib.ptr(a), 0, a.shape[0], a.shape[1], a
    if out is not None:
        if not out.is_cuda or out.numel() != m * box * box or not out.is_contiguous():
            raise ValueError("ERROR: output stack tensor has the wrong size or is not on the GPU")
        _sync_producer(out)
        op, odev, res = C.c_void_p(out.data_ptr()), 1, out
    else:
        res = np.empty((m, box, box), dtype=np.float32)
# ... 181 lines not shown
```

### pyp_amd/lib.py

```python
import ctypes as C
import os

import numpy as np

from .abi import NCOL, STATS_COLS, K_NAMES, RefineCfg, ReconCfg, FinalCfg

_HERE = os.path.dirname(os.path.abspath(__file__))
SO_PATH = os.path.join(_HERE, "libpypmatch.so")

EXPORTS = [
    "ppm_init", "ppm_last_error", "ppm_version", "ppm_build_id", "ppm_device_mem_info", "ppm_reference_create", "ppm_reference_create_padded", "ppm_reference_create_weighted", "ppm_reference_destroy",
    "ppm_refine_batch", "ppm_refine_last_counts", "ppm_refine_last_sections", "ppm_refine_last_overlap", "ppm_refine_note", "ppm_match_projections", "ppm_csp_refine", "ppm_csp_search_plan", "ppm_csp_search_candidates", "ppm_frame_refine", "ppm_frame_plan", "ppm_sva_align", "ppm_accum_floats", "ppm_accum_create", "ppm_accum_destroy",
    "ppm_insert_batch", "ppm_accum_download", "ppm_accum_download_range", "ppm_accum_add", "ppm_accum_count", "ppm_accum_set_count",
    "ppm_finalize", "ppm_profile_enable", "ppm_profile_reset", "ppm_profile_get", "ppm_device_alloc",
    "ppm_device_free", "ppm_device_upload", "ppm_device_sync", "ppm_extract_boxes", "ppm_host_alloc", "ppm_host_free", "ppm_host_read",
    "ppm_comm_unique_id", "ppm_comm_create", "ppm_comm_count", "ppm_comm_destroy", "ppm_accum_reduce", "ppm_sva_insert", "ppm_sva_align_average", "ppm_mask_volume",
    "ppm_create_mask", "ppm_postprocess", "ppm_local_resolution",
]


class PpmError(RuntimeError):
    pass


_lib = None


def load():
    global _lib
    if _lib is not None:
        return _lib
    if not os.path.exists(SO_PATH):
        raise PpmError(f"ERROR: {SO_PATH} is missing - build it with `python -c 'import __graft_entry__ as g; g.build()'` "
                       "(there is no CPU fallback)")
    L = C.CDLL(SO_PATH)
    vp, ci, cf, cl = C.c_void_p, C.c_int, C.c_float, C.c_long
    L.ppm_init.argtypes = [ci]; L.ppm_init.restype = ci
    L.ppm_last_error.restype = C.c_char_p
    L.ppm_version.restype = C.c_char_p
    L.ppm_build_id.restype = C.c_char_p
    L.ppm_device_mem_info.argtypes = [vp, vp]; L.ppm_device_mem_info.restype = ci
    L.ppm_reference_create.argtypes = [vp, ci, cf]; L.ppm_reference_create.restype = vp
    L.ppm_reference_create_padded.argtypes = [vp, ci, cf, ci]; L.ppm_reference_create_padded.restype = vp
    L.ppm_reference_create_weighted.argtypes = [vp, ci, cf, ci, vp, ci]; L.ppm_reference_create_weighted.restype = vp
    L.ppm_reference_destroy.argtypes = [vp]; L.ppm_reference_destroy.restype = None
    L.ppm_refine_batch.argtypes = [vp, vp, vp, ci, ci, vp, vp]; L.ppm_refine_batch.restype = ci
    L.ppm_refine_last_counts.argtypes = [vp, vp, vp, vp, vp]; L.ppm_refine_last_counts.restype = ci
    L.ppm_refine_last_sections.argtypes = [vp]; L.ppm_refine_last_sections.restype = ci
    L.ppm_refine_last_overlap.argtypes = [vp]; L.ppm_refine_last_overlap.restype = ci
    L.ppm_refine_note.argtypes = [vp]; L.ppm_refine_note.restype = C.c_char_p
    L.ppm_match_projections.argtypes = [vp, vp, vp, ci, vp]; L.ppm_match_projections.restype = ci
    L.ppm_csp_refine.argtypes = [vp, vp, vp, vp, ci, ci, vp, vp, ci, vp, ci]; L.ppm_csp_refine.restype = ci
    L.ppm_csp_search_plan.argtypes = [vp, vp, vp]; L.ppm_csp_search_plan.restype = ci
    L.ppm_csp_search_candidates.argtypes = [vp, cl, ci, vp, vp, vp]; L.ppm_csp_search_candidates.restype = ci
    L.ppm_frame_refine.argtypes = [vp, vp, vp, vp, ci, vp, ci, vp, vp, vp, vp]; L.ppm_frame_refine.restype = ci
    L.ppm_frame_plan.argtypes = [vp, vp, vp, vp]; L.ppm_frame_plan.restype = ci
    L.ppm_sva_align.argtypes = [vp, vp, vp, ci, ci, vp, vp, vp]; L.ppm_sva_align.restype = ci
    L.ppm_sva_insert.argtypes = [vp, vp, vp, ci, ci, vp, vp, vp]; L.ppm_sva_insert.restype = ci
    L.ppm_sva_align_average.argtypes = [vp, vp, vp, vp, ci, ci, vp, vp, vp, vp]; L.ppm_sva_align_average.restype = ci
    L.ppm_accum_floats.argtypes = [ci]; L.ppm_accum_floats.restype = C.c_size_t
    L.ppm_accum_create.argtypes = [ci, cf, C.c_char_p, vp]; L.ppm_accum_create.restype = vp
    L.ppm_accum_destroy.argtypes = [vp]; L.ppm_accum_destroy.restype = None
    L.ppm_insert_batch.argtypes = [vp, vp, vp, ci, ci, vp]; L.ppm_insert_batch.restype = ci
    L.ppm_accum_download.argtypes = [vp, vp]; L.ppm_accum_download.restype = ci
    L.ppm_accum_download_range.argtypes = [vp, vp, C.c_size_t, C.c_size_t]; L.ppm_accum_download_range.restype = ci
    L.ppm_accum_add.argtypes = [vp, vp]; L.ppm_accum_add.restype = ci
    L.ppm_accum_count.argtypes = [vp, ci]; L.ppm_accum_count.restype = cl
    L.ppm_accum_set_count.argtypes = [vp, ci, cl]; L.ppm_accum_set_count.restype = None
    L.ppm_finalize.argtypes = [vp, vp, vp, vp, vp, vp]; L.ppm_finalize.restype = ci
    L.ppm_profile_enable.argtypes = [ci]; L.ppm_profile_enable.restype = None
    L.ppm_profile_reset.argtypes = []; L.ppm_profile_reset.restype = None
    L.ppm_profile_get.argtypes = [ci, vp, vp]; L.ppm_profile_get.restype = ci
    L.ppm_device_alloc.argtypes = [C.c_size_t]; L.ppm_device_alloc.restype = vp
    L.ppm_device_free.argtypes = [vp]; L.ppm_device_free.restype = None
    L.ppm_device_upload.argtypes = [vp, vp, C.c_size_t]; L.ppm_device_upload.restype = ci
    L.ppm_device_sync.argtypes = []; L.ppm_device_sync.restype = ci
    L.ppm_host_alloc.argtypes = [C.c_size_t]; L.ppm_host_alloc.restype = vp
    L.ppm_host_free.argtypes = [vp]; L.ppm_host_free.restype = None
    L.ppm_host_read.argtypes = [ci, C.c_longlong, vp, C.c_size_t, ci]; L.ppm_host_read.restype = ci
    L.ppm_extract_boxes.argtypes = [vp, ci, ci, ci, vp, ci, ci, C.c_double, C.c_double, ci, ci, vp, ci]; L.ppm_extract_boxes.restype = ci
    L.ppm_comm_unique_id.argtypes = [vp]; L.ppm_comm_unique_id.restype = ci
    L.ppm_comm_create.argtypes = [ci, ci, vp]; L.ppm_comm_create.restype = vp
    L.ppm_comm_count.argtypes = [vp]; L.ppm_comm_count.restype = ci
    L.ppm_comm_destroy.argtypes = [vp]; L.ppm_comm_destroy.restype = None
    L.ppm_accum_reduce.argtypes = [vp, vp, ci]; L.ppm_accum_reduce.restype = ci
    L.ppm_mask_volume.argtypes = [vp, vp, ci, ci, vp, vp]; L.ppm_mask_volume.restype = ci
    L.ppm_create_mask.argtypes = [vp, ci, ci, vp, vp, vp]; L.ppm_create_mask.restype = ci
    L.ppm_postprocess.argtypes = [vp, vp, vp, ci, ci, vp, vp, vp, vp, vp, vp, vp]; L.ppm_postprocess.restype = ci
    L.ppm_local_resolution.argtypes = [vp, vp, vp, vp, ci, ci, vp, vp, vp]; L.ppm_local_resolution.restype = ci
    _lib = L
    return L


def last_error():
    return load().ppm_last_error().decode(errors="replace")


def check(rc):
    if rc != 0:
        raise PpmError(last_error() or f"ERROR: libpypmatch call failed ({rc})")


_inited = None


def init(device=0):
    global _inited
    if _inited != device:
        import sys
        w = sys.modules.get("pyp_amd.surface.warm")
        if w is not None:
            w.join_init()
        check(load().ppm_init(int(device)))
        _inited = device


def ptr(a):
    return a.ctypes.data_as(C.c_void_p)
```

Before: 86490.

## Reuse neighbour trilinear taps in full-band local refinement sweeps

Adds a NEAR variant of the local refinement kernel. In late compass iterations, when the angular step moves samples less than about 1.6 voxels, each lane computes the cell address for every neighbour orientation. If that cell matches the centre orientation's cell, the lane reuses the centre's taps instead of issuing buffer loads. Skipped lanes load from an out-of-range offset that the buffer bounds check discards, which aims to cut gather traffic on the reference cube. It costs extra address arithmetic, a ballot per group, register pressure from the held centre taps, and a separate kernel instantiation. Optional counters report the reuse rate.

```diff
diff --git a/include/ppm.h b/include/ppm.h
--- a/include/ppm.h
+++ b/include/ppm.h
@@ -138,6 +138,7 @@
 const char *ppm_refine_note(ppm_ref_t *ref);
 int ppm_refine_last_sections(ppm_ref_t *ref);
 int ppm_refine_last_overlap(ppm_ref_t *ref);
+int ppm_refine_last_reuse(ppm_ref_t *ref, long *gathers, long *reused);
 
 int ppm_match_projections(ppm_ref_t *ref, const ppm_refine_cfg *cfg, const double *rows, int n_rows, float *out);
 
diff --git a/pyp_amd/csrc/host_ctx.h b/pyp_amd/csrc/host_ctx.h
--- a/pyp_amd/csrc/host_ctx.h
+++ b/pyp_amd/csrc/host_ctx.h
@@ -202,6 +202,7 @@
     long last_counts[4] = { 0, 0, 0, 0 };
     int last_sections = 0;
     int last_overlap = 0;
+    DevBuf<unsigned long long> reuse; long last_reuse[2] = { 0, 0 };
     std::string note;
 };
 
@@ -225,6 +226,7 @@
     return cv;
 }
 
+static bool local_reuse_wanted() { return !(getenv("PPM_LOCAL_REUSE") && atoi(getenv("PPM_LOCAL_REUSE")) == 0); }
 static bool local_tables_wanted(int tabR) {
     return !(getenv("PPM_LOCAL_TABLES") && atoi(getenv("PPM_LOCAL_TABLES")) == 0) && cube_tab_bytes(tabR) <= 16 * 1024;
 }
diff --git a/pyp_amd/csrc/host_refine.h b/pyp_amd/csrc/host_refine.h
--- a/pyp_amd/csrc/host_refine.h
+++ b/pyp_amd/csrc/host_refine.h
@@ -132,7 +132,7 @@
 }
 
 namespace {
-struct LocalLaunch { LocalP P = {}; int threads = 0, per_particle = 1; double evals = 0; };
+struct LocalLaunch { LocalP P = {}; int threads = 0, per_particle = 1; double evals = 0; bool near = false; };
 struct RefineRun {
     ppm_ref *ref = nullptr; const ppm_refine_cfg *cfg = nullptr;
     Geom gm; SampleList sl; CubeView cv;
@@ -152,6 +152,7 @@
     LocalLaunch hit, fin;
     double sample_evals = 0;
     bool overlap = false; int tenants = 0;
+    unsigned long long *reuse = nullptr;
 
     int ntiles() const { return (int)(cxs.size() * cys.size()); }
     int nsec() const { return (int)secs.size(); }
@@ -455,6 +456,7 @@
         double rb = march_band(r.bf, r.gm.N, r.Rm_px, ha, hs, r.any_ang, r.any_sh, rcap);
         L.P.rmax2_it[t] = (float)(rb * rb); L.P.S_it[t] = r.prefix_of(rb);
         L.evals += (double)L.per_particle * r.per_iter * std::floor(kPi * rb * rb / 2);
+        if (L.near && near_reuse_pays(r.any_ang, ha, r.cv.scale, rb)) L.P.near_it |= 1u << t;
         ha *= 0.5; hs *= 0.5;
     }
     return L;
@@ -468,7 +470,7 @@
     return L;
 }
 static LocalLaunch full_band_launch(const RefineRun &r, int T, double ha, double hs) {
-    LocalLaunch L; L.P = r.base; L.threads = kFinalThreads;
+    LocalLaunch L; L.P = r.base; L.threads = kFinalThreads; L.near = local_reuse_wanted();
     L.P.T = r.cfg->local_refine ? T : 0; L.P.final_rescore = 1; L.P.nr = r.nrings;
     L = with_schedule(r, L, ha, hs, r.gm.r_hi);
     L.evals += std::floor(kPi * r.gm.r_hi * r.gm.r_hi / 2);
@@ -478,6 +480,11 @@
 static LocalLaunch rows_launch(const RefineRun &r) { return full_band_launch(r, r.Tb + r.Tc, r.ha0, r.hs0); }
 
 struct LocalShape { size_t lds; bool tab; int tabR; };
+typedef void (*LocalKernel)(LocalP);
+static LocalKernel local_kernel(bool tab, bool near) {
+    if (near) return tab ? k_local<true, true> : k_local<false, true>;
+    return tab ? k_local<true, false> : k_local<false, false>;
+}
 static LocalShape local_shape(const RefineRun &r, const LocalLaunch &L) {
     const LocalP &LP = L.P;
     const size_t ring = ring_lds_bytes8(L.threads / 64, kMaxCand, LP.nr);
@@ -492,13 +499,12 @@
 }
 static void launch_local(const RefineRun &r, const LocalLaunch &L, const Lane &ln, LState *states, int nb) {
     LocalP LP = L.P;
-    LP.Il = ln.Il.p; LP.cw = ln.cw.p; LP.states = states;
+    LP.Il = ln.Il.p; LP.cw = ln.cw.p; LP.states = states; LP.reuse = L.near ? r.reuse : nullptr;
     const LocalShape s = local_shape(r, L);
     LP.tabR = s.tabR;
     const dim3 grid((unsigned)(nb * L.per_particle)), block(L.threads);
     ProfScope ps(PPM_K_LOCAL);
-    if (s.tab) hipLaunchKernelGGL(k_local<true>, grid, block, s.lds, cur_stream(), LP);
-    else hipLaunchKernelGGL(k_local<false>, grid, block, s.lds, cur_stream(), LP);
+    hipLaunchKernelGGL(local_kernel(s.tab, L.near), grid, block, s.lds, cur_stream(), LP);
 }
 
 static int search_section(const RefineRun &r, int nb, const GridSection &sec, Hit *hits, int K, hipEvent_t ev_pre) {
@@ -608,7 +614,7 @@
     const LocalShape ls = local_shape(r, r.hit);
     hipFuncAttributes ga, la;
     HIPCHK(hipFuncGetAttributes(&ga, global_kernel(r.Rwin, gm.half != 0, gm.Bs)));
-    HIPCHK(hipFuncGetAttributes(&la, ls.tab ? (const void *)k_local<true> : (const void *)k_local<false>));
+    HIPCHK(hipFuncGetAttributes(&la, (const void *)local_kernel(ls.tab, r.hit.near)));
     const OverlapKernel host = { ga.numRegs, global_threads(r.Rwin), (long)ga.sharedSizeBytes + (long)global_lds_bytes(r.HsP, r.secs[0].nd * gm.n_psi, r.Rwin, nullptr) };
     const OverlapKernel tenant = { la.numRegs, r.hit.threads, (long)la.sharedSizeBytes + (long)ls.lds };
     const OverlapDevice dev = { 512, 4, (long)g.lds_per_cu, 8, 1280 };
@@ -660,6 +666,17 @@
     c[1] = nl;
     c[2] = (long)std::floor(kPi * gm.r_s * gm.r_s / 2);
     c[3] = (long)evals;
+}
+
+static int read_reuse(const RefineRun &r) {
+    if (!r.reuse) return 0;
+    unsigned long long h[2] = { 0, 0 };
+    HIPCHK(hipMemcpyAsync(h, r.reuse, sizeof(h), hipMemcpyDeviceToHost, cur_stream()));
+    HIPCHK(hipStreamSynchronize(cur_stream()));
+    r.ref->last_reuse[0] = (long)h[0]; r.ref->last_reuse[1] = (long)h[1];
+    if (std::getenv("PPM_TRACE"))
+        fprintf(stderr, "ppm_refine_batch: tap reuse in the full-band stage: %llu of %llu neighbour lane-gathers (iterations 0x%x)\n", h[1], h[0], r.fin.P.near_it);
+    return 0;
 }
 
 extern "C" {
@@ -787,6 +804,13 @@
     }
     HIPCHK(hipStreamSynchronize(cur_stream()));
     if (int rc = local_setup(r)) return rc;
+    ref->last_reuse[0] = ref->last_reuse[1] = 0;
+    if (const char *e = std::getenv("PPM_LOCAL_REUSE_COUNT")) if (std::atoi(e) != 0) {
+        if (int rc = ref->reuse.ensure(2)) return rc;
+        HIPCHK(hipMemsetAsync(ref->reuse.p, 0, 2 * sizeof(unsigned long long), cur_stream()));
+        HIPCHK(hipStreamSynchronize(cur_stream()));
+        r.reuse = ref->reuse.p;
+    }
     if (cfg->global_search) { r.hit = hit_launch(r); r.fin = final_launch(r); }
     else r.fin = rows_launch(r);
     r.sample_evals = r.hit.evals + r.fin.evals;
@@ -830,7 +854,7 @@
             if (int rc = stage.sync()) return rc;
         }
         refine_counts(r);
-        return 0;
+        return read_reuse(r);
     }
     OverlapStreams os;
     if (int rc = os.open(ref)) return rc;
@@ -858,7 +882,7 @@
     }
     if (int rc = os.drain()) return rc;
     refine_counts(r);
-    return 0;
+    return read_reuse(r);
 }
 
 
@@ -866,6 +890,12 @@
 
 int ppm_refine_last_sections(ppm_ref_t *ref) { return ref ? ref->last_sections : 0; }
 int ppm_refine_last_overlap(ppm_ref_t *ref) { return ref ? ref->last_overlap : 0; }
+int ppm_refine_last_reuse(ppm_ref_t *ref, long *gathers, long *reused) {
+    if (!ref) return fail(-22, "null reference");
+    if (gathers) *gathers = ref->last_reuse[0];
+    if (reused) *reused = ref->last_reuse[1];
+    return 0;
+}
 
 int ppm_refine_last_counts(ppm_ref_t *ref, long *n_global, long *n_local, long *samples_global, long *samples_local) {
     if (!ref) return fail(-22, "null reference");
diff --git a/pyp_amd/csrc/ppm_dev.h b/pyp_amd/csrc/ppm_dev.h
--- a/pyp_amd/csrc/ppm_dev.h
+++ b/pyp_amd/csrc/ppm_dev.h
@@ -228,6 +228,33 @@
 
 typedef float cube_v4f __attribute__((ext_vector_type(4)));
 
+struct CubeAddr { unsigned oa, ob, oc, od; int x0, y0, z0; };
+
+__device__ __forceinline__ void cube_load(const CubeView &cv, const CubeAddr &o, CubeTaps &t) {
+    const __amdgpu_buffer_rsrc_t rs = __builtin_amdgcn_make_buffer_rsrc((void *)cv.cube, 0, (int)(2u * cv.LB * 8u), 0x00020000);
+    const cube_v4f a = __builtin_amdgcn_raw_buffer_load_b128(rs, (int)o.oa, 0, 0), b = __builtin_amdgcn_raw_buffer_load_b128(rs, (int)o.ob, 0, 0);
+    const cube_v4f c = __builtin_amdgcn_raw_buffer_load_b128(rs, (int)o.oc, 0, 0), d = __builtin_amdgcn_raw_buffer_load_b128(rs, (int)o.od, 0, 0);
+    t.a = make_float4(a.x, a.y, a.z, a.w); t.b = make_float4(b.x, b.y, b.z, b.w);
+    t.c = make_float4(c.x, c.y, c.z, c.w); t.d = make_float4(d.x, d.y, d.z, d.w);
+}
+__device__ __forceinline__ CubeAddr cube_addr(const CubeView &cv, CubeTaps &t, float X, float Y, float Z) {
+    X *= cv.scale; Y *= cv.scale; Z *= cv.scale;
+    t.cj = X < 0.f;
+    if (t.cj) { X = -X; Y = -Y; Z = -Z; }
+    const float xf = floorf(X), yf = floorf(Y), zf = floorf(Z);
+    t.fx = X - xf; t.fy = Y - yf; t.fz = Z - zf;
+    const int x0 = (int)xf, y0 = (int)yf + cv.off, z0 = (int)zf + cv.off;
+    const bool second = (x0 & 3) == 3;
+    const int xs = second ? x0 - 2 : x0;
+    const unsigned rowb = (unsigned)cv.NBX * 128u, planeb = __umul24(rowb, (unsigned)cv.NBY);
+    const unsigned xl = (unsigned)(xs >> 2) * 128u + (unsigned)(xs & 3) * 8u + (second ? cv.LB * 8u : 0u);
+    const unsigned yl0 = __umul24((unsigned)(y0 >> 1), rowb) + (unsigned)(y0 & 1) * 32u, dy = (y0 & 1) ? rowb - 32u : 32u;
+    const unsigned zl0 = __umul24((unsigned)(z0 >> 1), planeb) + (unsigned)(z0 & 1) * 64u, dz = (z0 & 1) ? planeb - 64u : 64u;
+    CubeAddr o;
+    o.oa = xl + yl0 + zl0; o.ob = o.oa + dy; o.oc = o.oa + dz; o.od = o.ob + dz;
+    o.x0 = x0; o.y0 = y0; o.z0 = z0;
+    return o;
+}
 __device__ __forceinline__ CubeTaps cube_fetch(const CubeView &cv, float X, float Y, float Z) {
     CubeTaps t;
     X *= cv.scale; Y *= cv.scale; Z *= cv.scale;
@@ -274,6 +301,17 @@
 
 __device__ __forceinline__ int floor_to_int(float x) { int i; asm("v_cvt_flr_i32_f32 %0, %1" : "=v"(i) : "v"(x)); return i; }
 
+__device__ __forceinline__ CubeAddr cube_addr_tab(const CubeTab &tb, CubeTaps &t, float X, float Y, float Z) {
+    t.cj = X < 0.f;
+    if (t.cj) { X = -X; Y = -Y; Z = -Z; }
+    t.fx = __builtin_amdgcn_fractf(X); t.fy = __builtin_amdgcn_fractf(Y); t.fz = __builtin_amdgcn_fractf(Z);
+    CubeAddr o;
+    o.x0 = floor_to_int(X); o.y0 = floor_to_int(Y); o.z0 = floor_to_int(Z);
+    const unsigned xl = tb.tx0[o.x0];
+    const uint2 ey = tb.ty0[o.y0], ez = tb.tz0[o.z0];
+    o.oa = xl + ey.x + ez.x; o.ob = o.oa + ey.y; o.oc = o.oa + ez.y; o.od = o.ob + ez.y;
+    return o;
+}
 __device__ __forceinline__ CubeTaps cube_fetch_tab(const CubeView &cv, const CubeTab &tb, float X, float Y, float Z) {
     CubeTaps t;
     t.cj = X < 0.f;
@@ -290,6 +328,19 @@
     return t;
 }
 
+__device__ __forceinline__ bool cube_same_cell(const CubeAddr &o, const CubeAddr &c) { return o.x0 == c.x0 && o.y0 == c.y0 && o.z0 == c.z0; }
+__device__ __forceinline__ void cube_load_unless(const CubeView &cv, CubeAddr o, bool same, CubeTaps &t) {
+    constexpr unsigned kNoTap = 0xFFFFFFF0u;
+    if (same) { o.oa = kNoTap; o.ob = kNoTap; o.oc = kNoTap; o.od = kNoTap; }
+    cube_load(cv, o, t);
+}
+__device__ __forceinline__ float4 cube_pick(bool same, const float4 &c, const float4 &own) {
+    return make_float4(same ? c.x : own.x, same ? c.y : own.y, same ? c.z : own.z, same ? c.w : own.w);
+}
+__device__ __forceinline__ void cube_take(CubeTaps &t, bool same, const CubeTaps &c) {
+    t.a = cube_pick(same, c.a, t.a); t.b = cube_pick(same, c.b, t.b); t.c = cube_pick(same, c.c, t.c); t.d = cube_pick(same, c.d, t.d);
+}
+
 __device__ __forceinline__ float2 cube_interp(const CubeTaps &t) {
     const float fx = t.fx, fy = t.fy, fz = t.fz;
     const float ar = t.a.x + fx * (t.a.z - t.a.x), ai = t.a.y + fx * (t.a.w - t.a.y);
diff --git a/pyp_amd/csrc/ppm_geom.h b/pyp_amd/csrc/ppm_geom.h
--- a/pyp_amd/csrc/ppm_geom.h
+++ b/pyp_amd/csrc/ppm_geom.h
@@ -302,6 +302,10 @@
     const int T = m > steptol ? (int)std::ceil(std::log(m / steptol) / std::log(2.0)) : min_iters;
     return std::min(12, std::max(min_iters, T));
 }
+constexpr double kNearMove = 1.6;
+inline double near_move(double ha, double pad, double rband) { return ha * kPi / 180.0 * pad * rband; }
+inline bool near_reuse_pays(bool any_ang, double ha, double pad, double rband) { return any_ang && near_move(ha, pad, rband) <= kNearMove; }
+
 struct LdsRegion { unsigned off, bytes, elem; };
 struct PrepLds {
     LdsRegion T;
diff --git a/pyp_amd/csrc/ppm_kernels2.h b/pyp_amd/csrc/ppm_kernels2.h
--- a/pyp_amd/csrc/ppm_kernels2.h
+++ b/pyp_amd/csrc/ppm_kernels2.h
@@ -17,6 +17,7 @@
     float rmax2_final; int S_final;
     float rmax2_class; int S_class;
     int use_priors; double pmean[5], pw[5];
+    unsigned near_it; unsigned long long *reuse;
 };
 
 __device__ inline double d_prior_pen(const LocalP &P, const double *M, double shx, double shy) {
@@ -64,8 +65,9 @@
     CubeTab tab;
 };
 
-template <bool TAB>
-__device__ __forceinline__ void sweep_plan(SweepPlan &plan, const SweepCtx &C, const int tid, const int nthr) {
+struct ReuseCount { unsigned all, same; };
+template <bool TAB, bool NEAR = false>
+__device__ __forceinline__ void sweep_plan(SweepPlan &plan, const SweepCtx &C, const int tid, const int nthr, const bool near = false, ReuseCount *cnt = nullptr) {
     const int lane = tid & 63, wave = tid >> 6, nw = C.nw, nr = C.nr;
     float *const ringA = C.ringA, *const sumB = C.sumB, *const sumC = C.sumC; double *const score = C.score;
     const float2 *const Il = C.Il; const float *const cw = C.cw; const float invN = C.invN;
@@ -101,11 +103,18 @@
         };
         float b0x, b0y;
         turned(0, b0x, b0y);
+        auto coord = [&](float m0, float m1) { return __fmaf_rn(fkx, m0, __fmul_rn(fky, m1)); };
         auto fetch = [&](int g) {
             const float *m = plan.ms[g];
-            const float X = m[0] * fkx + m[1] * fky, Y = m[2] * fkx + m[3] * fky, Z = m[4] * fkx + m[5] * fky;
+            const float X = coord(m[0], m[1]), Y = coord(m[2], m[3]), Z = coord(m[4], m[5]);
             if constexpr (TAB) return cube_fetch_tab(C.cv, C.tab, X, Y, Z);
             else { CubeView one = C.cv; one.scale = 1.f; return cube_fetch(one, X, Y, Z); }
+        };
+        auto where = [&](int g, CubeTaps &t) {
+            const float *m = plan.ms[g];
+            const float X = coord(m[0], m[1]), Y = coord(m[2], m[3]), Z = coord(m[4], m[5]);
+            if constexpr (TAB) return cube_addr_tab(C.tab, t, X, Y, Z);
+            else { CubeView one = C.cv; one.scale = 1.f; return cube_addr(one, t, X, Y, Z); }
         };
         const bool mine = head && ring < nr;
         float *const cellA = myA + ring;
@@ -136,6 +145,36 @@
                 if (mine) atomicAdd(cellA + q * strideA, av);
             }
         };
+        if constexpr (NEAR) {
+            const unsigned long long act = __ballot(s < S_used);
+            cnt->all += (unsigned)__builtin_popcountll(act) * (unsigned)(ng - 1);
+            if (near && ng > 1) {
+                struct Near { CubeTaps t; bool same; };
+                CubeTaps C0;
+                const CubeAddr c0 = where(ng - 1, C0);
+                cube_load(C.cv, c0, C0);
+                auto fetch_near = [&](int g) {
+                    Near n;
+                    const CubeAddr o = where(g, n.t);
+                    n.same = cube_same_cell(o, c0);
+                    cnt->same += (unsigned)__builtin_popcountll(__ballot(n.same) & act);
+                    cube_load_unless(C.cv, o, n.same, n.t);
+                    return n;
+                };
+                auto score_near = [&](int g, Near &n) { cube_take(n.t, n.same, C0); score_group(g, n.t); };
+                const int nn = ng - 1;
+                Near A = fetch_near(0), B;
+                __builtin_amdgcn_sched_barrier(0); score_group(nn, C0);
+                int g = 0;
+                for (; g + 2 < nn; g += 2) {
+                    B = fetch_near(g + 1); __builtin_amdgcn_sched_barrier(0); score_near(g, A);
+                    A = fetch_near(g + 2); __builtin_amdgcn_sched_barrier(0); score_near(g + 1, B);
+                }
+                if (g + 1 < nn) { B = fetch_near(g + 1); __builtin_amdgcn_sched_barrier(0); score_near(g, A); score_near(g + 1, B); }
+                else score_near(g, A);
+                continue;
+            }
+        }
         CubeTaps A = fetch(0), B;
         int g = 0;
         for (; g + 2 < ng; g += 2) {
@@ -176,7 +215,7 @@
 #ifndef PPM_LOCAL_MINW
 #define PPM_LOCAL_MINW 4
 #endif
-template <bool TAB>
+template <bool TAB, bool NEAR>
 __global__ void __launch_bounds__(256, PPM_LOCAL_MINW) k_local(LocalP P) {
     __shared__ SweepPlan plan;
     extern __shared__ float lsm[];
@@ -184,6 +223,7 @@
     __shared__ LState st;
     __shared__ double sfp[5], sfm[5], sd[5], sMt[9], sshq[2], sf0;
     __shared__ double spen[kMaxCand];
+    ReuseCount cnt = { 0u, 0u };
     const int tid = threadIdx.x, nthr = blockDim.x;
     const int nw = nthr >> 6, nr = P.nr;
     float *const ringA = lsm, *const sumB = lsm + kMaxCand * nw * nr, *const sumC = sumB + kMaxCand * nw;
@@ -259,7 +299,8 @@
             if (tid == 0) { plan.S_used = P.S_class; plan.rmax2 = P.rmax2_class; }
         }
         __syncthreads();
-        sweep_plan<TAB>(plan, SC, tid, nthr);
+        if constexpr (NEAR) sweep_plan<TAB, true>(plan, SC, tid, nthr, phase == PH_COMPASS && ((P.near_it >> it) & 1u), &cnt);
+        else sweep_plan<TAB>(plan, SC, tid, nthr);
         if (tid == 0) {
             if (phase == PH_COMPASS) {
                 int qc = 0;
@@ -297,6 +338,16 @@
         __syncthreads();
     }
     if (tid == 0) P.states[blockIdx.x] = st;
+    if constexpr (NEAR) {
+        if (P.reuse) {
+            __shared__ unsigned sreuse[2];
+            if (tid == 0) sreuse[0] = sreuse[1] = 0u;
+            __syncthreads();
+            if ((tid & 63) == 0) { atomicAdd(&sreuse[0], cnt.all); atomicAdd(&sreuse[1], cnt.same); }
+            __syncthreads();
+            if (tid == 0) { atomicAdd(P.reuse, (unsigned long long)sreuse[0]); atomicAdd(P.reuse + 1, (unsigned long long)sreuse[1]); }
+        }
+    }
 }
 
 __global__ void k_states_from_hits(const Hit *hits, LState *states, int n, int K, const double *dir_theta,
diff --git a/pyp_amd/host.py b/pyp_amd/host.py
--- a/pyp_amd/host.py
+++ b/pyp_amd/host.py
@@ -138,6 +138,11 @@
 
     def last_overlap(self):
         return int(lib.load().ppm_refine_last_overlap(self.h))
+
+    def last_reuse(self):
+        v = [C.c_long(), C.c_long()]
+        lib.check(lib.load().ppm_refine_last_reuse(self.h, C.byref(v[0]), C.byref(v[1])))
+        return v[0].value, v[1].value
 
     def close(self):
         if getattr(self, "h", None):
diff --git a/pyp_amd/lib.py b/pyp_amd/lib.py
--- a/pyp_amd/lib.py
+++ b/pyp_amd/lib.py
@@ -10,7 +10,7 @@
 
 EXPORTS = [
     "ppm_init", "ppm_last_error", "ppm_version", "ppm_build_id", "ppm_device_mem_info", "ppm_reference_create", "ppm_reference_create_padded", "ppm_reference_create_weighted", "ppm_reference_destroy",
-    "ppm_refine_batch", "ppm_refine_last_counts", "ppm_refine_last_sections", "ppm_refine_last_overlap", "ppm_refine_note", "ppm_match_projections", "ppm_csp_refine", "ppm_csp_search_plan", "ppm_csp_search_candidates", "ppm_frame_refine", "ppm_frame_plan", "ppm_sva_align", "ppm_accum_floats", "ppm_accum_create", "ppm_accum_destroy",
+    "ppm_refine_batch", "ppm_refine_last_counts", "ppm_refine_last_sections", "ppm_refine_last_overlap", "ppm_refine_last_reuse", "ppm_refine_note", "ppm_match_projections", "ppm_csp_refine", "ppm_csp_search_plan", "ppm_csp_search_candidates", "ppm_frame_refine", "ppm_frame_plan", "ppm_sva_align", "ppm_accum_floats", "ppm_accum_create", "ppm_accum_destroy",
     "ppm_insert_batch", "ppm_accum_download", "ppm_accum_download_range", "ppm_accum_add", "ppm_accum_count", "ppm_accum_set_count",
     "ppm_finalize", "ppm_profile_enable", "ppm_profile_reset", "ppm_profile_get", "ppm_device_alloc",
     "ppm_device_free", "ppm_device_upload", "ppm_device_sync", "ppm_extract_boxes", "ppm_host_alloc", "ppm_host_free", "ppm_host_read",
@@ -48,6 +48,7 @@
     L.ppm_refine_last_counts.argtypes = [vp, vp, vp, vp, vp]; L.ppm_refine_last_counts.restype = ci
     L.ppm_refine_last_sections.argtypes = [vp]; L.ppm_refine_last_sections.restype = ci
     L.ppm_refine_last_overlap.argtypes = [vp]; L.ppm_refine_last_overlap.restype = ci
+    L.ppm_refine_last_reuse.argtypes = [vp, vp, vp]; L.ppm_refine_last_reuse.restype = ci
     L.ppm_refine_note.argtypes = [vp]; L.ppm_refine_note.restype = C.c_char_p
     L.ppm_match_projections.argtypes = [vp, vp, vp, ci, vp]; L.ppm_match_projections.restype = ci
     L.ppm_csp_refine.argtypes = [vp, vp, vp, vp, ci, ci, vp, vp, ci, vp, ci]; L.ppm_csp_refine.restype = ci
```

New measurement: 90130 (median of 6 runs). 1.04x the previous value.
